# OFA-Sys/ONE-PEACE

Hardware: AMD Instinct MI355X
Metric: pretrain samples/s (tri-modal global batch) ONE-PEACE-4B (higher is better)
Workload: dtype bf16

## Files before the change

include/onepeace_hip.h:

```cpp
#ifndef ONEPEACE_HIP_H
#define ONEPEACE_HIP_H

#include <stdint.h>

#ifdef __cplusplus
extern "C" {
#endif

int op_abi_version(void);
const char* op_last_error(void);

int op_prof_enable(int on);
int op_prof_reserve(int events);
int op_prof_collect(double* ms, int64_t* count, double* work, int n_families);

int op_layernorm_fwd(const void* x, const void* w, const void* b, void* y, float* mean, float* rstd, int64_t rows,
                     int64_t cols, float eps, int act_gelu, int dtype, const int* x_rows, void* stream);
int64_t op_layernorm_bwd_workspace_bytes(int64_t rows, int64_t cols);
int op_layernorm_bwd(const void* dy, const void* x, const void* w, const void* b, const float* mean, const float* rstd,
                     const void* add, void* dx, void* dw, void* db, void* workspace, int64_t rows, int64_t cols,
                     int act_gelu, int accumulate, int dtype, const int* x_rows, void* stream);

int op_gemm_nt(const void* A, int64_t lda, const void* B0, const void* B1, const void* B2, int64_t ldb, int64_t n_seg,
               const void* bias0, const void* bias1, const void* bias2, void* C, int64_t ldc, void* h0, void* h1,
// ... 22 lines not shown
int op_gemm_tn_grouped(int64_t nprob, const void* const* A, const int64_t* lda, const void* const* B, const int64_t* ldb, void* const* C,
                       const int64_t* ldc, const int64_t* M, const int64_t* N, const int64_t* K, const int32_t* accumulate,
                       const void* const* W, const int64_t* ldw, float* const* rowdot, const void* const* rscale, void* counters,
                       int64_t tune, void* stream);
int op_gemm_tn_grouped_lists(int64_t nprob, const void* const* A, const int64_t* lda, const void* const* B, const int64_t* ldb, void* const* C,
                             const int64_t* ldc, const int64_t* M, const int64_t* N, const int64_t* K, const int32_t* accumulate,
                             const void* const* W, const int64_t* ldw, float* const* rowdot, const void* const* rscale,
                             const int32_t* const* ktiles, const int32_t* const* n_ktiles, void* counters, int64_t tune, void* stream);
int op_live_ktiles(int64_t nseg, const float* const* ps, const int64_t* row0, const int64_t* S, const int64_t* B, int64_t nprob,
                   const int64_t* prob_row0, const int64_t* prob_rows, int32_t* const* ktiles, int32_t* const* n_ktiles, void* stream);
int op_live_mwindows(int64_t nseg, const float* const* ps, const int64_t* ps_stride, const int64_t* row0, const int64_t* S, const int64_t* B,
                     const int64_t* wps, const int64_t* odd, const int64_t* seg_list, const int64_t* seg_prob, const int64_t* seg_base, int64_t nlist,
                     int32_t* const* windows,
                     int32_t* const* n_windows, const int64_t* max_windows, int64_t nout, void* const* out, const int64_t* out_ld,
                     const int64_t* out_cols, const int64_t* out_rows, void* stream);
int op_gemm_nt_grouped_windows(int64_t nprob, const void* const* A, const int64_t* M, int64_t lda, const void* const* B, int64_t ldb,
                               void* const* C, int64_t ldc, int64_t N, int64_t K, const int32_t* windows, const int32_t* n_windows,
                               int64_t max_windows, int64_t max_row_stride, int64_t tune, void* stream);
int op_live_mwindows_fwd(int64_t nseg, const float* const* ps, const int64_t* ps_stride, const int64_t* row0, const int64_t* S, const int64_t* B,
                         const int64_t* wps, const int64_t* odd, const int64_t* seg_list, const int64_t* seg_prob, const int64_t* seg_base,
                         int64_t nlist, int32_t* const* windows, int32_t* const* n_windows, const int64_t* max_windows, int64_t nout,
                         void* const* out, const int64_t* out_ld, const int64_t* out_cols, const int64_t* out_rows,
                         const void* const* out_src, const int64_t* out_src_ld, void* stream);
int op_gemm_nt_grouped_windows_fwd(int64_t nprob, const void* const* A, const int64_t* M, int64_t lda, const void* const* B, int64_t ldb,
                                   int64_t n_seg, const void* const* bias, void* const* C, int64_t ldc, const void* const* resid, int64_t ldr,
                                   const void* const* gamma, const float* const* rowscale, const int64_t* rows_per_sample, int64_t N,
                                   int64_t K, int epilogue, const int32_t* windows, const int32_t* n_windows, int64_t max_windows,
                                   int64_t max_row_stride, int64_t tune, void* stream);
int op_gemm_plan(int64_t M, int64_t N, int64_t K, int epilogue, int has_bias, int64_t workspace_bytes, int64_t tune, int* plan);

int op_quant_fp8_rows(const void* x, int64_t ldx, void* q, int64_t ldq, float* scale, int64_t rows, int64_t cols, void* stream);
int op_layernorm_fwd_q8(const void* x, const void* w, const void* b, void* y, float* mean, float* rstd, void* q8, float* q8_scale,
                        int64_t rows, int64_t cols, float eps, void* stream);
int op_ln_geglu_fwd_q8(const void* h0, const void* h1, int64_t ldh, const void* w, const void* b, void* y, float* mean, float* rstd, void* q8,
                       float* q8_scale, int64_t rows, int64_t cols, float eps, void* stream);
int op_gemm_nt_fp8(const void* A8, int64_t lda, const float* sa, const void* B0, const void* B1, int64_t ldb, const float* sb0,
                   const float* sb1, const void* bias, void* C, int64_t ldc, void* h0, void* h1, const void* resid, int64_t ldr,
                   const void* gamma, const float* rowscale, int64_t rows_per_sample, int64_t M, int64_t N, int64_t K, int epilogue,
                   int64_t tune, void* stream);

int op_attn_fwd(const void* q, const void* k, const void* v, int64_t ld, const void* bias, int64_t bias_batch_stride,
                const void* bias_frag, const void* key_pad, void* out, int64_t ldo, float* lse, int64_t lse_ld, int64_t B,
                int64_t S, int64_t Spad, int64_t heads, int64_t head_dim, float scale, int64_t tune, void* stream);
int64_t op_attn_bias_frag_elems(int64_t n_img, int64_t S);
int op_attn_bias_pack(const void* src, void* dst, int64_t n_img, int64_t S, int64_t Spad, void* stream);
int op_attn_bwd_delta(const void* dout, const void* out, int64_t ldo, float* delta, int64_t B, int64_t S, int64_t Spad,
                      int64_t heads, void* stream);
int64_t op_attn_bwd_dbias_slabs(int64_t B, int64_t S, int64_t heads, int64_t tune);
int op_attn_bwd(const void* q, const void* k, const void* v, int64_t ld, const void* dout, const void* out, int64_t ldo,
                const void* bias, const void* biasT, const void* bias_frag, int64_t bias_batch_stride, const void* key_pad,
                const float* lse, float* delta, void* dq,
                void* dk, void* dv, int64_t ldg, float* dbias, int64_t B, int64_t S, int64_t Spad, int64_t heads,
                int64_t head_dim, float scale, int64_t tune, void* stream);

int op_relpos_bias_build(const void* table, const int* bucket, int64_t bucket_ld, void* out, int64_t heads, int64_t S,
                         int64_t Spad, int transposed, void* stream);
int op_relpos_bias_bwd(const float* dbias, int64_t S, int64_t Spad, const int* pos, const int* seg, int64_t nseg, const int* bucket_seg,
                       int64_t num_rel, float* partial_ws, float* dtable, int64_t heads, void* stream);
int op_relpos_bias_build_ids(const void* table, const int* bucket, int64_t bucket_ld, const int* ids, void* out, int64_t B,
                             int64_t heads, int64_t K, int64_t Kpad, int transposed, void* stream);
int op_relpos_bias_fold_ids(const float* dbias, const int* ids, float* dense_ws, int64_t Sfull, int64_t B, int64_t heads, int64_t K,
                            int64_t Kpad, void* stream);

int op_transpose(const void* in, void* out, int64_t rows, int64_t cols, int64_t ld_in, int64_t ld_out, void* stream);
int op_transpose_scaled(const void* in, void* out, int64_t rows, int64_t cols, int64_t ld_in, int64_t ld_out, const void* scale,
                        void* stream);
int op_transpose_batched(const void* table, int64_t n, int64_t total_tiles, void* stream);
int64_t op_transpose_desc_bytes(void);
int64_t op_colsum_workspace_bytes(int64_t N);
int op_colsum_segments(const void* x, void* out0, void* out1, void* out2, void* workspace, int64_t M, int64_t n_seg,
                       int64_t seg_cols, int accumulate, void* stream);
int64_t op_resid_bwd_workspace_bytes(int64_t N);
int op_resid_bwd(const void* dout, const void* y, const void* gamma, const float* rowscale, int64_t rows_per_sample,
                 void* dbranch, void* dgamma, void* dbias, float* g0, void* workspace, int64_t M, int64_t N, int accumulate,
                 const int* dout_rows, void* stream);
int op_gamma_grad_finish(const float* rowdot, int64_t slots, const void* b0, const float* g00, const void* b1, const float* g01,
                         const void* b2, const float* g02, void* dgamma, int64_t N, int accumulate, void* stream);
int op_ln_geglu_bwd(const void* dy, const void* h0, const void* h1, const void* w, const float* mean, const float* rstd,
                    void* dh0, void* dh1, int64_t ldd, int64_t ldh, void* dw, void* db, void* workspace, int64_t rows,
                    int64_t cols, int accumulate, void* stream);
int op_ln_geglu_fwd(const void* h0, const void* h1, int64_t ldh, const void* w, const void* b, void* y, float* mean, float* rstd,
                    int64_t rows, int64_t cols, float eps, void* stream);
int op_colsum(const void* x, const void* y, const float* rowscale, int64_t rows_per_sample, const void* mul, void* out,
              void* workspace, int64_t M, int64_t N, int accumulate, int out_dtype, void* stream);
int op_geglu_bwd(const void* dg, const void* h0, const void* h1, void* dh0, void* dh1, int64_t numel, void* stream);
int op_scale_rows(const void* dout, const void* gamma, const float* rowscale, int64_t rows_per_sample, void* dbranch,
                  int64_t M, int64_t N, void* stream);

int op_l2norm_fwd(const void* x, void* y, float* inv_norm, int64_t rows, int64_t cols, float eps, int out_dtype, void* stream);
int op_l2norm_bwd(const void* dy, const void* y, const float* inv_norm, void* dx, int64_t rows, int64_t cols, int y_dtype,
                  void* stream);
int op_infonce_rows(float* sim, int64_t rows, int64_t n, int64_t ld, int64_t target0, float label_smoothing, float gscale,
                    float* row_loss, float* row_hit, float* row_dot, int write_grad, void* stream);

int op_adamw_step(void* p, const void* g, float* m, float* v, int64_t numel, float lr, float beta1, float beta2, float eps,
                  float weight_decay, int64_t step, float grad_scale, const float* grad_sqnorm, float clip_norm,
                  void* stream);
int op_adamw_step_groups(void* p, const void* g, float* m, float* v, int64_t numel, const int64_t* group_end8,
                         const float* group_lr_scale, const float* group_weight_decay, int64_t n_groups, float lr, float beta1,
                         float beta2, float eps, int64_t step, float grad_scale, const float* grad_sqnorm, float clip_norm,
                         void* stream);
int op_adamw_step_groups_master(void* p, float* master, const void* g, float* m, float* v, int64_t numel,
                                const int64_t* group_end8, const float* group_lr_scale, const float* group_weight_decay,
                                int64_t n_groups, float lr, float beta1, float beta2, float eps, int64_t step, float grad_scale,
                                const float* grad_sqnorm, float clip_norm, void* stream);
int op_ema_step(float* ema, const void* p, int64_t numel, float keep, float take, void* stream);
// ... 55 lines not shown
```

one-peace_amd/csrc/attention.hip:

```cpp
#include <type_traits>

#include "common.h"

namespace {

constexpr int HD = 64;
constexpr int BQ = 128;
constexpr int BKV = 64;
constexpr int VSTRIDE = 160;

struct AttnArgs {
  const bf16_t* q; const bf16_t* k; const bf16_t* v; int64_t ld;
  const bf16_t* bias;
  int64_t bias_bs;
  const uint8_t* key_pad;
  bf16_t* out; int64_t ldo;
  float* lse;
  int64_t lse_ld;
  int B, S, Spad, heads;
  float scale;
};

__device__ __forceinline__ bf16x8 pack8(const float* a, const float* b) {
  bf16x8 r;
#pragma unroll
  for (int i = 0; i < 4; ++i) { r[i] = (bf16_t)a[i]; r[4 + i] = (bf16_t)b[i]; }
  return r;
}

__device__ __forceinline__ s16x4 tr_read(const char* p) {
  return __builtin_amdgcn_ds_read_tr16_b64_v4i16((__attribute__((address_space(3))) s16x4*)(p));
}

__device__ __forceinline__ bf16x8 join_tr(s16x4 a, s16x4 b) {
  typedef __attribute__((ext_vector_type(8))) short s16x8;
  s16x8 r = {a[0], a[1], a[2], a[3], b[0], b[1], b[2], b[3]};
  return __builtin_bit_cast(bf16x8, r);
}

__device__ __forceinline__ int tr_off_swz(int rowblk, int db, int g, int t) {
  const int row = rowblk * 16 + g * 4 + (t >> 2);
  const int c = db * 2 + ((t >> 1) & 1);
  return row * 128 + ((c ^ (row & 7)) << 4) + (t & 1) * 8;
}

__device__ __forceinline__ void xcd_work_item(int& bx, int& by, int& bz) {
  const int nx = gridDim.x, ny = gridDim.y;
  const int total = nx * ny * (int)gridDim.z;
  int lin = blockIdx.x + nx * (blockIdx.y + ny * blockIdx.z);
  if ((total & 7) == 0) lin = (lin & 7) * (total >> 3) + (lin >> 3);
  bx = lin % nx;
  by = (lin / nx) % ny;
  bz = lin / (nx * ny);
}

template <bool HAS_BIAS, bool HAS_PAD>
__global__ __launch_bounds__(256, 2) void attn_fwd_kernel(AttnArgs p) {
  __shared__ __attribute__((aligned(16))) char smem[BKV * 128 + BKV * VSTRIDE];
  char* ldsK = smem;
  char* ldsV = smem + BKV * 128;
  const int tid = threadIdx.x, lane = tid & 63, wid = tid >> 6;
  const int g = lane >> 4, t = lane & 15;
  int bx, h, b;
  xcd_work_item(bx, h, b);
  const int q0 = bx * BQ + wid * 32;
  const bool wave_active = q0 < p.S;
  const int64_t row_base = (int64_t)b * p.S;

  bf16x8 qf[2][2];
#pragma unroll
  for (int qb = 0; qb < 2; ++qb) {
    const int qi = min(q0 + qb * 16 + t, p.S - 1);
    const bf16_t* qp = p.q + (row_base + qi) * p.ld + h * HD;
#pragma unroll
// ... 346 lines not shown
  };

  const int ntiles = (p.S + BKV - 1) / BKV;
  for (int kt = 0; kt < ntiles; ++kt) {
    const int k0 = kt * BKV;
    if (k0 + BKV <= p.S) tile(k0, std::true_type{});
    else tile(k0, std::false_type{});
  }

  float l = l_run;
  l += __shfl_xor(l, 16);
  l += __shfl_xor(l, 32);
  if (q0 + t >= p.S) continue;
  const float inv = 1.f / l;
  bf16_t* op = p.out + (row_base + q0 + t) * p.ldo + h * HD;
#pragma unroll
  for (int db = 0; db < 4; ++db) {
    bf16x4 o;
#pragma unroll
    for (int r = 0; r < 4; ++r) o[r] = (bf16_t)(ot[db][r] * inv);
    *reinterpret_cast<bf16x4*>(op + db * 16 + g * 4) = o;
  }
  if (g == 0 && p.lse) p.lse[((int64_t)b * p.heads + h) * p.lse_ld + q0 + t] = m2_run * (1.0f / LOG2E) + logf(l);
  }
}

constexpr int PERS_NW = 8;
constexpr int PERS_MAX_ROWS = 288;
constexpr int PERS_SCR = 68;
constexpr int PERS_PPT = 2;

__device__ __forceinline__ s16x4 tr_read_a(const char* p) {
  s16x4 r;
  asm volatile("ds_read_b64_tr_b16 %0, %1" : "=v"(r) : "v"((unsigned)(uintptr_t)((__attribute__((address_space(3))) const char*)p)));
  return r;
}
#define ATTN_WAIT_LGKM0()                         \
  do {                                            \
    __builtin_amdgcn_s_waitcnt(0xC07F);           \
    __builtin_amdgcn_sched_barrier(0);            \
  } while (0)

__device__ __forceinline__ void gload16_asm(bf16x8& d, const void* p) { asm volatile("global_load_dwordx4 %0, %1, off" : "=v"(d) : "v"(p)); }
__device__ __forceinline__ void gload4_asm(unsigned& d, const void* p) { asm volatile("global_load_dword %0, %1, off" : "=v"(d) : "v"(p)); }
template <int OFF>
__device__ __forceinline__ void gload16_s(bf16x8& d, const void* sbase, unsigned voff) {
  asm volatile("s_nop 4\n\tglobal_load_dwordx4 %0, %1, %2 offset:%3" : "=v"(d) : "v"(voff), "s"(sbase), "n"(OFF));
}
template <int OFF>
__device__ __forceinline__ void gload4_s(unsigned& d, const void* sbase, unsigned voff) {
  asm volatile("s_nop 4\n\tglobal_load_dword %0, %1, %2 offset:%3" : "=v"(d) : "v"(voff), "s"(sbase), "n"(OFF));
}

template <bool HAS_BIAS, bool HAS_PAD>
__global__ __launch_bounds__(PERS_NW * 64, 2) void attn_fwd_pers_kernel(AttnArgs p, const bf16_t* __restrict__ bias_frag, int rows_pad,
                                                                         int nitems) {
  extern __shared__ __attribute__((aligned(16))) char smem[];
  const int tid = threadIdx.x, lane = tid & 63;
  const int wid = __builtin_amdgcn_readfirstlane(tid >> 6);
  const int g = lane >> 4, t = lane & 15;
  const int KVB = 2 * rows_pad * 128;
  float* scratch = reinterpret_cast<float*>(smem + 2 * KVB);
  const int nqb = (p.S + 15) >> 4, nkp = (p.S + 31) >> 5;
  const bool has_left = nqb > 2 * PERS_NW;
  const int q0 = wid * 32;
  const int nact = min(2, max(0, nqb - 2 * wid));
  const int64_t per_head = (int64_t)nqb * nkp * FRAG_BLOCK;
  const int ntiles = (p.S + BKV - 1) / BKV;
  const float c1 = p.scale * LOG2E;

  bf16x8 sel_lo, sel_hi;
  {
    const bf16_t inv = (bf16_t)(1.0f / p.scale), zero = (bf16_t)0.f;
#pragma unroll
    for (int i = 0; i < 8; ++i) {
      sel_lo[i] = (g * 8 + i == t) ? inv : zero;
      sel_hi[i] = (g * 8 + i == 16 + t) ? inv : zero;
    }
  }
  int trsw[4];
#pragma unroll
  for (int db = 0; db < 4; ++db) trsw[db] = tr_off_swz(0, db, g, t);
  const int kswz[2] = {((0 * 4 + g) ^ (t & 7)) << 4, ((1 * 4 + g) ^ (t & 7)) << 4};

  const int ngrp = rows_pad >> 3;
  const int r_in = lane >> 3, slot = lane & 7;
  const int npiece = (2 * ngrp - wid + PERS_NW - 1) / PERS_NW;
  auto piece = [&](int it, int buf, int j) {
    const int b = it / p.heads, h = it - b * p.heads;
    const int grp = wid + j * PERS_NW;
    const bool isv = grp >= ngrp;
    const int gi = isv ? grp - ngrp : grp;
    const int r = gi * 8 + r_in;
    const int kr = min(r, p.S - 1);
    const bf16_t* src = (isv ? p.v : p.k) + ((int64_t)b * p.S + kr) * p.ld + h * HD + ((slot ^ (r & 7)) << 3);
    char* dst = smem + buf * KVB + (isv ? rows_pad * 128 : 0) + gi * 1024;
    __builtin_amdgcn_global_load_lds((const __attribute__((address_space(1))) void*)src,
                                     (__attribute__((address_space(3))) void*)dst, 16, 0, 0);
  };
  auto load_q = [&](int it, int qrow, bf16x8 (&q)[2]) {
    const int b = it / p.heads, h = it - b * p.heads;
    const bf16_t* qp = p.q + ((int64_t)b * p.S + qrow) * p.ld + h * HD;
#pragma unroll
    for (int kk = 0; kk < 2; ++kk) q[kk] = *reinterpret_cast<const bf16x8*>(qp + kk * 32 + g * 8);
  };
  const int qi_main[2] = {min(q0 + t, p.S - 1), min(q0 + 16 + t, p.S - 1)};

  bf16x8 bn[2][2];
  unsigned padn[4] = {0u, 0u, 0u, 0u};
  auto small_loads = [&](int it, int kt) {
    const int b = it / p.heads, h = it - b * p.heads;
    if constexpr (HAS_BIAS) {
      const bf16_t* fhead = bias_frag + ((p.bias_bs != 0 ? (int64_t)b * p.heads : 0) + h) * per_head + lane * 8;
#pragma unroll
      for (int qb = 0; qb < 2; ++qb) {
        const bf16_t* fb = fhead + (int64_t)min(2 * wid + qb, nqb - 1) * nkp * FRAG_BLOCK;
#pragma unroll
        for (int m = 0; m < 2; ++m) gload16_asm(bn[qb][m], fb + min(2 * kt + m, nkp - 1) * FRAG_BLOCK);
      }
    }
    if constexpr (HAS_PAD) {
      const uint8_t* pr = p.key_pad + (int64_t)b * p.Spad + g * 4 + kt * BKV;
#pragma unroll
      for (int kb = 0; kb < 4; ++kb) gload4_asm(padn[kb], pr + kb * 16);
    }
  };

  constexpr int NSMALL = (HAS_BIAS ? 4 : 0) + (HAS_PAD ? 4 : 0);
  bf16x8 qn[2][2], ql[2], bfl[2];
  unsigned padl[2][2] = {{0u, 0u}, {0u, 0u}};
  auto late_loads = [&](int it_next, int it) {
    {
      const int b = it_next / p.heads, h = it_next - b * p.heads;
#pragma unroll
      for (int qb = 0; qb < 2; ++qb) {
        const bf16_t* qp = p.q + ((int64_t)b * p.S + qi_main[qb]) * p.ld + h * HD;
#pragma unroll
        for (int kk = 0; kk < 2; ++kk) gload16_asm(qn[qb][kk], qp + kk * 32 + g * 8);
      }
    }
    if (has_left) {
      const int b = it / p.heads, h = it - b * p.heads;
      const bf16_t* qp = p.q + ((int64_t)b * p.S + p.S - 1) * p.ld + h * HD;
#pragma unroll
      for (int kk = 0; kk < 2; ++kk) gload16_asm(ql[kk], qp + kk * 32 + g * 8);
      if constexpr (HAS_BIAS) {
        const bf16_t* fleft = bias_frag + ((p.bias_bs != 0 ? (int64_t)b * p.heads : 0) + h) * per_head + lane * 8 + (int64_t)(nqb - 1) * nkp * FRAG_BLOCK;
        gload16_asm(bfl[0], fleft + wid * FRAG_BLOCK);
        gload16_asm(bfl[1], fleft + min(PERS_NW, nkp - 1) * FRAG_BLOCK);
      }
      if constexpr (HAS_PAD) {
        const uint8_t* pr = p.key_pad + (int64_t)b * p.Spad + g * 4;
#pragma unroll
        for (int j = 0; j < 2; ++j) {
          gload4_asm(padl[0][j], pr + (2 * wid + j) * 16);
          gload4_asm(padl[1][j], pr + min((2 * PERS_NW + j) * 16, p.Spad - 16));
        }
      }
    }
  };

  int item = blockIdx.x;
  const int step = gridDim.x;
  if (item < nitems) {
    for (int j = 0; j < npiece; ++j) piece(item, 0, j);
    load_q(item, qi_main[0], qn[0]);
    load_q(item, qi_main[1], qn[1]);
    small_loads(item, 0);
  }
  int buf = 0, prev_item = -1;
  auto wait_all = [&]() {
    asm volatile("s_waitcnt vmcnt(0)" : "+v"(qn[0][0]), "+v"(qn[0][1]), "+v"(qn[1][0]), "+v"(qn[1][1]), "+v"(bn[0][0]), "+v"(bn[0][1]), "+v"(bn[1][0]), "+v"(bn[1][1]),
                 "+v"(padn[0]), "+v"(padn[1]), "+v"(padn[2]), "+v"(padn[3]) : : "memory");
  };
  wait_all();

  auto merge_left = [&](int it, int sb) {
    const float* sc = scratch + sb * (PERS_NW * PERS_SCR);
    float M = -INFINITY;
#pragma unroll
    for (int w = 0; w < PERS_NW; ++w) M = fmaxf(M, sc[w * PERS_SCR + 64]);
    float L = 0.f, o = 0.f;
#pragma unroll
    for (int w = 0; w < PERS_NW; ++w) {
      const float f = __builtin_amdgcn_exp2f(sc[w * PERS_SCR + 64] - M);
      L = __builtin_fmaf(sc[w * PERS_SCR + 65], f, L);
      o = __builtin_fmaf(sc[w * PERS_SCR + lane], f, o);
    }
    const int b = it / p.heads, h = it - b * p.heads;
    const int qrow = p.S - 1;
    p.out[((int64_t)b * p.S + qrow) * p.ldo + h * HD + lane] = (bf16_t)(o / L);
    if (lane == 0 && p.lse) p.lse[((int64_t)b * p.heads + h) * p.lse_ld + qrow] = M * (1.0f / LOG2E) + logf(L);
  };

  for (; item < nitems; item += step, buf ^= 1) {
    const int b = item / p.heads, h = item - b * p.heads;
    const int64_t row_base = (int64_t)b * p.S;
    __syncthreads();
    bf16x8 qf[2][2] = {{qn[0][0], qn[0][1]}, {qn[1][0], qn[1][1]}};
    const bool more = item + step < nitems;
    const int nxt = more ? item + step : item;
    if (has_left && prev_item >= 0 && wid == ((prev_item / step) & (PERS_NW - 1))) merge_left(prev_item, buf ^ 1);
    prev_item = item;

    const char* ldsK = smem + buf * KVB;
    const char* ldsV = ldsK + rows_pad * 128;

    f32x4 ot[2][4];
    float m2_run[2] = {-INFINITY, -INFINITY}, l_run[2] = {0.f, 0.f};
#pragma unroll
    for (int qb = 0; qb < 2; ++qb)
#pragma unroll
      for (int db = 0; db < 4; ++db) ot[qb][db] = (f32x4){0.f, 0.f, 0.f, 0.f};

    auto tile = [&](const int kt, auto full_c) {
      constexpr bool FULL = decltype(full_c)::value;
      const int k0 = kt * BKV;
      const int nkb = FULL ? 4 : ((p.S - k0 + 15) >> 4);
      bf16x8 bf[2][2];
      unsigned padw[4] = {0u, 0u, 0u, 0u};
      if constexpr (HAS_BIAS) {
#pragma unroll
        for (int qb = 0; qb < 2; ++qb)
#pragma unroll
          for (int m = 0; m < 2; ++m) bf[qb][m] = bn[qb][m];
      }
      if constexpr (HAS_PAD) {
#pragma unroll
        for (int kb = 0; kb < 4; ++kb) padw[kb] = padn[kb];
      }
      __builtin_amdgcn_sched_barrier(0);
      if constexpr (FULL) {
        small_loads(item, kt + 1);
      } else {
        late_loads(nxt, item);
        small_loads(nxt, 0);
      }
      __builtin_amdgcn_sched_barrier(0);
#pragma unroll
      for (int jj = 0; jj < PERS_PPT; ++jj) piece(nxt, buf ^ 1, min(kt * PERS_PPT + jj, npiece - 1));
      __builtin_amdgcn_sched_barrier(0);
      if (nact == 0) return;

      const char* kt_ = ldsK + k0 * 128;
      const char* vt = ldsV + k0 * 128;
      f32x4 st[2][4];
#pragma unroll
      for (int qb = 0; qb < 2; ++qb)
#pragma unroll
        for (int kb = 0; kb < 4; ++kb) st[qb][kb] = (f32x4){0.f, 0.f, 0.f, 0.f};
#pragma unroll
      for (int kb = 0; kb < 4; ++kb) {
        if (!FULL && kb >= nkb) break;
#pragma unroll
        for (int kk = 0; kk < 2; ++kk) {
          const bf16x8 kf = *reinterpret_cast<const bf16x8*>(kt_ + (kb * 16 + t) * 128 + kswz[kk]);
#pragma unroll
          for (int qb = 0; qb < 2; ++qb) st[qb][kb] = __builtin_amdgcn_mfma_f32_16x16x32_bf16(kf, qf[qb][kk], st[qb][kb], 0, 0, 0);
        }
        if constexpr (HAS_BIAS) {
#pragma unroll
          for (int qb = 0; qb < 2; ++qb)
            st[qb][kb] = __builtin_amdgcn_mfma_f32_16x16x32_bf16(bf[qb][kb >> 1], (kb & 1) ? sel_hi : sel_lo, st[qb][kb], 0, 0, 0);
        }
      }
      s16x4 va0[4], va1[4];
#pragma unroll
      for (int db = 0; db < 4; ++db) {
        va0[db] = tr_read_a(vt + trsw[db]);
        va1[db] = tr_read_a(vt + trsw[db] + 2048);
      }
      bf16x8 pf[2][2];
#pragma unroll
      for (int qb = 0; qb < 2; ++qb) {
        float mx = -INFINITY;
#pragma unroll
        for (int kb = 0; kb < 4; ++kb) {
          if (!FULL && kb >= nkb) break;
          const int key = k0 + kb * 16 + g * 4;
#pragma unroll
          for (int r = 0; r < 4; ++r) {
            if constexpr (!FULL || HAS_PAD) {
              bool masked = false;
              if constexpr (!FULL) masked = key + r >= p.S;
              if constexpr (HAS_PAD) masked = masked || ((padw[kb] >> (8 * r)) & 0xffu);
              st[qb][kb][r] = masked ? -INFINITY : st[qb][kb][r];
            }
            mx = fmaxf(mx, st[qb][kb][r]);
// ... 110 lines not shown
        float psum = 0.f;
#pragma unroll
        for (int j = 0; j < 2; ++j)
#pragma unroll
          for (int r = 0; r < 4; ++r) {
            pv[j][r] = __builtin_amdgcn_exp2f(__builtin_fmaf(s4[j][r], c1, -m2_use));
            psum += pv[j][r];
          }
        lsum = lsum * alpha + psum;
        const bf16x8 pf = pack8(pv[0], pv[1]);
        s16x4 v0[4], v1[4];
#pragma unroll
        for (int db = 0; db < 4; ++db) {
          v0[db] = tr_read_a(ldsV + trsw[db] + (2 * kp) * 2048);
          v1[db] = tr_read_a(ldsV + trsw[db] + (2 * kp + 1) * 2048);
        }
        ATTN_WAIT_LGKM0();
#pragma unroll
        for (int db = 0; db < 4; ++db) {
#pragma unroll
          for (int r = 0; r < 4; ++r) ol[db][r] *= alpha;
          ol[db] = __builtin_amdgcn_mfma_f32_16x16x32_bf16(join_tr(v0[db], v1[db]), pf, ol[db], 0, 0, 0);
        }
      }
      lsum += __shfl_xor(lsum, 16);
      lsum += __shfl_xor(lsum, 32);
      float* sc = scratch + (buf * PERS_NW + wid) * PERS_SCR;
      if (t == 0) {
#pragma unroll
        for (int db = 0; db < 4; ++db) *reinterpret_cast<f32x4*>(sc + db * 16 + g * 4) = ol[db];
        if (g == 0) { sc[64] = m2; sc[65] = lsum; }
      }
    }
#pragma unroll
    for (int qb = 0; qb < 2; ++qb) {
      float l = l_run[qb];
      l += __shfl_xor(l, 16);
      l += __shfl_xor(l, 32);
      const int qrow = q0 + qb * 16 + t;
      if (qb < nact && qrow < p.S) {
        const float inv = 1.f / l;
        bf16_t* op = p.out + (row_base + qrow) * p.ldo + h * HD;
#pragma unroll
        for (int db = 0; db < 4; ++db) {
          bf16x4 o;
#pragma unroll
          for (int r = 0; r < 4; ++r) o[r] = (bf16_t)(ot[qb][db][r] * inv);
          *reinterpret_cast<bf16x4*>(op + db * 16 + g * 4) = o;
        }
        if (g == 0 && p.lse) p.lse[((int64_t)b * p.heads + h) * p.lse_ld + qrow] = m2_run[qb] * (1.0f / LOG2E) + logf(l);
      }
    }
    wait_all();
  }
  if (has_left && prev_item >= 0) {
    __syncthreads();
    if (wid == 0) merge_left(prev_item, buf ^ 1);
  }
}

__global__ __launch_bounds__(256) void bias_pack_kernel(const bf16_t* __restrict__ src, bf16_t* __restrict__ dst, int S, int Spad,
                                                        int nqb, int nkp, int64_t total) {
  const int64_t idx = (int64_t)blockIdx.x * 256 + threadIdx.x;
  if (idx >= total) return;
  const int lane = (int)(idx & 63);
  int64_t blk = idx >> 6;
  const int kp = (int)(blk % nkp);
  blk /= nkp;
  const int qb = (int)(blk % nqb);
  const int64_t img = blk / nqb;
  const int g = lane >> 4, t = lane & 15;
  const int key = kp * 32 + (g >> 1) * 16 + t;
  const int qbase = qb * 16 + (g & 1) * 8;
  bf16x8 v;
#pragma unroll
  for (int i = 0; i < 8; ++i) {
    const int q = qbase + i;
    v[i] = (q < S && key < S) ? src[(img * S + q) * Spad + key] : (bf16_t)0.f;
  }
  *reinterpret_cast<bf16x8*>(dst + idx * 8) = v;
}

struct AttnBwdArgs {
  const bf16_t* q; const bf16_t* k; const bf16_t* v; int64_t ld;
  const bf16_t* dout; int64_t ldo;
  const bf16_t* bias;
  const bf16_t* biasT;
  const bf16_t* bias_frag;
  int64_t bias_bs;
  const uint8_t* key_pad;
  const float* lse;
  const float* delta;
  const bf16_t* out;
  float* delta_w;
  bf16_t* dq; bf16_t* dk; bf16_t* dv; int64_t ldg;
  float* dbias;
  int B, S, Spad, heads, bchunk;
  float scale;
  int lone_keys;
};

__global__ __launch_bounds__(256) void attn_delta_kernel(const bf16_t* __restrict__ dout, const bf16_t* __restrict__ out,
                                                         int64_t ldo, float* __restrict__ delta, int B, int S, int Spad,
                                                         int heads) {
  const int64_t gid = (int64_t)blockIdx.x * 256 + threadIdx.x;
  const int per_row = heads * 8;
// ... 620 lines not shown
              ds[0][kb][r] = __builtin_amdgcn_exp2f(__builtin_fmaf(st[kb][r], c1, nl2)) * (ds[0][kb][r] - dl);
        }
      } else {
        ds_tile<1, true, (NT < 6)>(p, b, h, k0, q0w, g, t, qf, of, lse, del, kfrag, vfrag, biasfrag, prefetch, ds);
      }
#pragma unroll
      for (int c = 0; c < NT; ++c) {
        if (kt == c) {
#pragma unroll
          for (int kb = 0; kb < 4; ++kb)
            if (c < NT - 1 || kb < LASTB) acc[c][kb] += ds[0][kb];
        }
      }
#pragma unroll
      for (int m = 0; m < 2; ++m) {
        if (k0 + m * 32 >= p.S) break;
        float a0[4], a1[4];
#pragma unroll
        for (int r = 0; r < 4; ++r) { a0[r] = ds[0][2 * m][r]; a1[r] = ds[0][2 * m + 1][r]; }
        const bf16x8 dsf = pack8(a0, a1);
#pragma unroll
        for (int db = 0; db < 4; ++db) {
          const bf16x8 kT = join_tr(tr_read(ldsK + trsw[db] + (2 * m) * 2048), tr_read(ldsK + trsw[db] + (2 * m + 1) * 2048));
          dqT[db] = __builtin_amdgcn_mfma_f32_16x16x32_bf16(kT, dsf, dqT[db], 0, 0, 0);
        }
      }
    }
    if (wave_active && q0w + t < p.S) {
      bf16_t* qp = p.dq + ((int64_t)b * p.S + q0w + t) * p.ldg + h * HD;
#pragma unroll
      for (int db = 0; db < 4; ++db) {
        bf16x4 a;
#pragma unroll
        for (int r = 0; r < 4; ++r) a[r] = (bf16_t)(dqT[db][r] * p.scale);
        *reinterpret_cast<bf16x4*>(qp + db * 16 + g * 4) = a;
      }
    }
  }
  if (!wave_active || q0w + t >= p.S) return;
  float* drow = p.dbias + (((int64_t)chunk * p.heads + h) * p.S + q0w + t) * p.Spad + g * 4;
#pragma unroll
  for (int kt = 0; kt < NT; ++kt) {
    f32x4 cur[4];
#pragma unroll
    for (int kb = 0; kb < 4; ++kb)
      if ((kt < NT - 1 || kb < LASTB) && kt * BKV + kb * 16 < p.Spad) cur[kb] = *reinterpret_cast<const f32x4*>(drow + kt * BKV + kb * 16);
#pragma unroll
    for (int kb = 0; kb < 4; ++kb)
      if ((kt < NT - 1 || kb < LASTB) && kt * BKV + kb * 16 < p.Spad)
        *reinterpret_cast<f32x4*>(drow + kt * BKV + kb * 16) = cur[kb] + acc[kt][kb];
  }
}

template <bool HAS_BIAS, bool HAS_PAD, int NT, int LASTB, bool LEFT>
__device__ __forceinline__ void attn_bwd_dq_pers_body(const AttnBwdArgs& p, char* smem, int rows_pad, int nqh, int qhalf0) {
  const int tid = threadIdx.x, lane = tid & 63;
  const int wid = __builtin_amdgcn_readfirstlane(tid >> 6);
  const int g = lane >> 4, t = lane & 15;
  const int KVB = 2 * rows_pad * 128;
  float* scratch = reinterpret_cast<float*>(smem + 2 * KVB);
  const int nqb = (p.S + 15) >> 4, nkp = (p.S + 31) >> 5;
  const int qhalf = qhalf0, h = (blockIdx.x / nqh) % p.heads, chunk = blockIdx.x / (nqh * p.heads);
  const int b_begin = chunk * p.bchunk, b_end = min(p.B, b_begin + p.bchunk);
  if (b_begin >= b_end) return;
  const int qblk = qhalf * PERS_NW + wid;
  const bool active = qblk < min(nqb, 2 * PERS_NW);
  constexpr bool has_left = LEFT;
  const int q0w = min(qblk, nqb - 1) * 16;
  const int qi = min(q0w + t, p.S - 1);
  const float c1 = p.scale * LOG2E;
  const int64_t per_head = (int64_t)nqb * nkp * FRAG_BLOCK;

  bf16x8 sel_lo, sel_hi;
  {
    const bf16_t inv = (bf16_t)(1.0f / p.scale), zero = (bf16_t)0.f;
#pragma unroll
    for (int i = 0; i < 8; ++i) {
      sel_lo[i] = (g * 8 + i == t) ? inv : zero;
      sel_hi[i] = (g * 8 + i == 16 + t) ? inv : zero;
    }
  }
  int trsw[4];
#pragma unroll
  for (int db = 0; db < 4; ++db) trsw[db] = tr_off_swz(0, db, g, t);
  const int kswz[2] = {((0 * 4 + g) ^ (t & 7)) << 4, ((1 * 4 + g) ^ (t & 7)) << 4};

  const int ngrp = rows_pad >> 3;
  const int r_in = lane >> 3, slot = lane & 7;
  const int npiece = (2 * ngrp - wid + PERS_NW - 1) / PERS_NW;
  auto piece = [&](int b, int buf, int j) {
    const int grp = wid + j * PERS_NW;
    const bool isv = grp >= ngrp;
    const int gi = isv ? grp - ngrp : grp;
    int rl = r_in;
    asm volatile("" : "+v"(rl));
    const int r = gi * 8 + rl;
    const int kr = min(r, p.S - 1);
    const unsigned voff = (unsigned)((kr * (int)p.ld + ((slot ^ (r & 7)) << 3)) * 2);
    const char* sbase = (const char*)((isv ? p.v : p.k) + (int64_t)b * p.S * p.ld + h * HD);
    char* dst = smem + buf * KVB + (isv ? rows_pad * 128 : 0) + gi * 1024;
    __builtin_amdgcn_global_load_lds((const __attribute__((address_space(1))) void*)(sbase + voff),
                                     (__attribute__((address_space(3))) void*)dst, 16, 0, 0);
  };

  constexpr int NSMALL = (HAS_BIAS ? 2 : 0) + (HAS_PAD ? 4 : 0);
  constexpr int BPPT = 3;
  auto ppt_of = [](int kt) { return kt < 3 ? BPPT : 0; };
  const bf16_t* fwave = HAS_BIAS ? p.bias_frag + (int64_t)h * per_head + (int64_t)(q0w >> 4) * nkp * FRAG_BLOCK : nullptr;
  const bf16_t* fleft = HAS_BIAS ? p.bias_frag + (int64_t)h * per_head + (int64_t)(nqb - 1) * nkp * FRAG_BLOCK : nullptr;
  const unsigned vo_frag = lane * 16, vo_pad = g * 4;
  const unsigned vo_q = (unsigned)(((int64_t)qi * p.ld + h * HD + g * 8) * 2), vo_o = (unsigned)(((int64_t)qi * p.ldo + h * HD + g * 8) * 2);
  const unsigned vo_ql = (unsigned)(((int64_t)(p.S - 1) * p.ld + h * HD + g * 8) * 2), vo_ol = (unsigned)(((int64_t)(p.S - 1) * p.ldo + h * HD + g * 8) * 2);
  const unsigned vo_lse = qi * 4, vo_lsel = (p.S - 1) * 4;
  bf16x8 bn[2];
  unsigned padn[4] = {0u, 0u, 0u, 0u};
  auto small_loads = [&](int b, int kt) {
    if constexpr (HAS_BIAS) {
// ... 3 lines not shown
    if constexpr (HAS_PAD) {
      const uint8_t* pr = p.key_pad + (int64_t)b * p.Spad + kt * BKV;
      gload4_s<0>(padn[0], pr, vo_pad);
      gload4_s<16>(padn[1], pr, vo_pad);
      gload4_s<32>(padn[2], pr, vo_pad);
      gload4_s<48>(padn[3], pr, vo_pad);
    }
  };
  bf16x8 qn[2], don[2], oon[2], ql[2], dol[2], ool[2], bfl[2];
  float lsen, lsel;
  unsigned padl[2][2] = {{0u, 0u}, {0u, 0u}};
  auto query_loads = [&](int b, unsigned voq, unsigned voo, unsigned vol, bf16x8 (&q)[2], bf16x8 (&d)[2], bf16x8 (&o)[2], float& l) {
    const bf16_t* sq = p.q + (int64_t)b * p.S * p.ld;
    const bf16_t* sd = p.dout + (int64_t)b * p.S * p.ldo;
    const bf16_t* so = p.out + (int64_t)b * p.S * p.ldo;
    gload16_s<0>(q[0], sq, voq);
    gload16_s<64>(q[1], sq, voq);
    gload16_s<0>(d[0], sd, voo);
    gload16_s<64>(d[1], sd, voo);
    gload16_s<0>(o[0], so, voo);
    gload16_s<64>(o[1], so, voo);
    unsigned lw;
    gload4_s<0>(lw, p.lse + ((int64_t)b * p.heads + h) * p.Spad, vol);
    l = __builtin_bit_cast(float, lw);
  };
  auto late_loads = [&](int b_next, int b) {
    (void)b_next;
    if (has_left) {
      query_loads(b, vo_ql, vo_ol, vo_lsel, ql, dol, ool, lsel);
      if constexpr (HAS_BIAS) {
        gload16_s<0>(bfl[0], fleft + wid * FRAG_BLOCK, vo_frag);
        gload16_s<0>(bfl[1], fleft + min(PERS_NW, nkp - 1) * FRAG_BLOCK, vo_frag);
      }
      if constexpr (HAS_PAD) {
        const uint8_t* pr = p.key_pad + (int64_t)b * p.Spad;
        gload4_s<0>(padl[0][0], pr + 2 * wid * 16, vo_pad);
        gload4_s<16>(padl[0][1], pr + 2 * wid * 16, vo_pad);
        gload4_s<0>(padl[1][0], pr + min(2 * PERS_NW * 16, p.Spad - 32), vo_pad);
        gload4_s<16>(padl[1][1], pr + min(2 * PERS_NW * 16, p.Spad - 32), vo_pad);
      }
    }
  };

  f32x4 acc[NT][4], accl[2][2];
#pragma unroll
  for (int kt = 0; kt < NT; ++kt)
#pragma unroll
    for (int kb = 0; kb < 4; ++kb) acc[kt][kb] = (f32x4){0.f, 0.f, 0.f, 0.f};
#pragma unroll
  for (int i = 0; i < 2; ++i)
#pragma unroll
    for (int j = 0; j < 2; ++j) accl[i][j] = (f32x4){0.f, 0.f, 0.f, 0.f};

  for (int j = 0; j < npiece; ++j) piece(b_begin, 0, j);
  query_loads(b_begin, vo_q, vo_o, vo_lse, qn, don, oon, lsen);
  small_loads(b_begin, 0);
  int buf = 0, prev_b = -1;
  auto merge_left = [&](int b, int sb) {
    const float* sc = scratch + sb * (PERS_NW * 64);
    float o = 0.f;
#pragma unroll
    for (int w = 0; w < PERS_NW; ++w) o += sc[w * 64 + lane];
    p.dq[((int64_t)b * p.S + p.S - 1) * p.ldg + h * HD + lane] = (bf16_t)(o * p.scale);
  };

  auto wait_all = [&]() {
    asm volatile("s_waitcnt vmcnt(0)" : "+v"(qn[0]), "+v"(qn[1]), "+v"(don[0]), "+v"(don[1]), "+v"(oon[0]), "+v"(oon[1]), "+v"(lsen), "+v"(bn[0]), "+v"(bn[1]),
                 "+v"(padn[0]), "+v"(padn[1]), "+v"(padn[2]), "+v"(padn[3]) : : "memory");
  };
  wait_all();
  for (int b = b_begin; b < b_end; ++b, buf ^= 1) {
    __syncthreads();
    const bf16x8 qf[2] = {qn[0], qn[1]}, dof[2] = {don[0], don[1]};
    const float dl = delta_from_frags(dof, oon);
    const float nl2 = -lsen * LOG2E;
    if (active && g == 0 && q0w + t < p.S) p.delta_w[((int64_t)b * p.heads + h) * p.Spad + q0w + t] = dl;
    const int nxt = b + 1 < b_end ? b + 1 : b;
    if (has_left && prev_b >= 0 && wid == (prev_b & (PERS_NW - 1))) merge_left(prev_b, buf ^ 1);
    prev_b = b;
    const char* ldsK = smem + buf * KVB;
    const char* ldsV = ldsK + rows_pad * 128;
    f32x4 dqT[4];
#pragma unroll
    for (int db = 0; db < 4; ++db) dqT[db] = (f32x4){0.f, 0.f, 0.f, 0.f};

    auto tile = [&](const int kt, auto last_c) {
      constexpr bool LAST = decltype(last_c)::value;
      const int k0 = kt * BKV;
      if (kt > 0) {
        if (ppt_of(kt - 1) > 0) {
          if constexpr (HAS_BIAS && HAS_PAD)
            asm volatile("s_waitcnt vmcnt(%6)" : "+v"(bn[0]), "+v"(bn[1]), "+v"(padn[0]), "+v"(padn[1]), "+v"(padn[2]), "+v"(padn[3]) : "n"(BPPT));
          else if constexpr (HAS_BIAS)
            asm volatile("s_waitcnt vmcnt(%2)" : "+v"(bn[0]), "+v"(bn[1]) : "n"(BPPT));
          else if constexpr (HAS_PAD)
            asm volatile("s_waitcnt vmcnt(%4)" : "+v"(padn[0]), "+v"(padn[1]), "+v"(padn[2]), "+v"(padn[3]) : "n"(BPPT));
        } else {
          if constexpr (HAS_BIAS && HAS_PAD)
            asm volatile("s_waitcnt vmcnt(0)" : "+v"(bn[0]), "+v"(bn[1]), "+v"(padn[0]), "+v"(padn[1]), "+v"(padn[2]), "+v"(padn[3]));
          else if constexpr (HAS_BIAS)
            asm volatile("s_waitcnt vmcnt(0)" : "+v"(bn[0]), "+v"(bn[1]));
          else if constexpr (HAS_PAD)
            asm volatile("s_waitcnt vmcnt(0)" : "+v"(padn[0]), "+v"(padn[1]), "+v"(padn[2]), "+v"(padn[3]));
        }
      }
      bf16x8 bf[2];
      unsigned padw[4] = {0u, 0u, 0u, 0u};
      if constexpr (HAS_BIAS) { bf[0] = bn[0]; bf[1] = bn[1]; }
      if constexpr (HAS_PAD) {
#pragma unroll
        for (int kb = 0; kb < 4; ++kb) padw[kb] = padn[kb];
      }
      __builtin_amdgcn_sched_barrier(0);
      if constexpr (!LAST) {
        if constexpr (!LEFT) {
          if (kt == NT - 2) query_loads(nxt, vo_q, vo_o, vo_lse, qn, don, oon, lsen);
        }
        small_loads(b, kt + 1);
      } else {
        late_loads(nxt, b);
        small_loads(nxt, 0);
      }
      __builtin_amdgcn_sched_barrier(0);
#pragma unroll
      for (int jj = 0; jj < BPPT; ++jj)
        if (ppt_of(kt) > 0) piece(nxt, buf ^ 1, min(kt * BPPT + jj, npiece - 1));
      __builtin_amdgcn_sched_barrier(0);
      const char* kt_ = ldsK + k0 * 128;
      const char* vt = ldsV + k0 * 128;
      constexpr int NKB = LAST ? LASTB : 4;
// ... 79 lines not shown
      f32x4 dql[4];
#pragma unroll
      for (int db = 0; db < 4; ++db) dql[db] = (f32x4){0.f, 0.f, 0.f, 0.f};
#pragma unroll
      for (int pc = 0; pc < 2; ++pc) {
        if (pc == 1 && wid != 0) break;
        const int kp = pc == 0 ? wid : PERS_NW;
        f32x4 s4[2], d4[2];
#pragma unroll
        for (int j = 0; j < 2; ++j) {
          s4[j] = (f32x4){0.f, 0.f, 0.f, 0.f};
          d4[j] = (f32x4){0.f, 0.f, 0.f, 0.f};
#pragma unroll
          for (int kk = 0; kk < 2; ++kk) {
            const bf16x8 kf = *reinterpret_cast<const bf16x8*>(ldsK + ((2 * kp + j) * 16 + t) * 128 + kswz[kk]);
            const bf16x8 vf = *reinterpret_cast<const bf16x8*>(ldsV + ((2 * kp + j) * 16 + t) * 128 + kswz[kk]);
            s4[j] = __builtin_amdgcn_mfma_f32_16x16x32_bf16(kf, ql[kk], s4[j], 0, 0, 0);
            d4[j] = __builtin_amdgcn_mfma_f32_16x16x32_bf16(vf, dol[kk], d4[j], 0, 0, 0);
          }
          if constexpr (HAS_BIAS) s4[j] = __builtin_amdgcn_mfma_f32_16x16x32_bf16(bfl[pc], j ? sel_hi : sel_lo, s4[j], 0, 0, 0);
        }
        float a0[4], a1[4];
#pragma unroll
        for (int j = 0; j < 2; ++j)
#pragma unroll
          for (int r = 0; r < 4; ++r) {
            bool dead = (2 * kp + j) * 16 + g * 4 + r >= p.S;
            if constexpr (HAS_PAD) dead = dead || ((padl[pc][j] >> (8 * r)) & 0xffu);
            const float x = dead ? -INFINITY : __builtin_fmaf(s4[j][r], c1, nl2l);
            const float v = __builtin_amdgcn_exp2f(x) * (d4[j][r] - dll);
            d4[j][r] = v;
            (j ? a1 : a0)[r] = v;
          }
        if constexpr (HAS_BIAS) { accl[pc][0] += d4[0]; accl[pc][1] += d4[1]; }
        const bf16x8 dsf = pack8(a0, a1);
        s16x4 k0r[4], k1r[4];
#pragma unroll
        for (int db = 0; db < 4; ++db) {
          k0r[db] = tr_read_a(ldsK + trsw[db] + (2 * kp) * 2048);
          k1r[db] = tr_read_a(ldsK + trsw[db] + (2 * kp + 1) * 2048);
        }
        ATTN_WAIT_LGKM0();
#pragma unroll
        for (int db = 0; db < 4; ++db) dql[db] = __builtin_amdgcn_mfma_f32_16x16x32_bf16(join_tr(k0r[db], k1r[db]), dsf, dql[db], 0, 0, 0);
      }
      float* sc = scratch + (buf * PERS_NW + wid) * 64;
      if (t == 0) {
#pragma unroll
        for (int db = 0; db < 4; ++db) *reinterpret_cast<f32x4*>(sc + db * 16 + g * 4) = dql[db];
      }
    }

    wait_all();
  }
  if (has_left && prev_b >= 0) {
    __syncthreads();
    if (wid == 0) merge_left(prev_b, buf ^ 1);
  }
  if constexpr (HAS_BIAS) {
    if (p.dbias == nullptr) return;
    if (active && q0w + t < p.S) {
      float* drow = p.dbias + (((int64_t)chunk * p.heads + h) * p.S + q0w + t) * p.Spad + g * 4;
#pragma unroll
      for (int kt = 0; kt < NT; ++kt) {
        f32x4 cur[4];
#pragma unroll
        for (int kb = 0; kb < 4; ++kb)
          if ((kt < NT - 1 || kb < LASTB) && kt * BKV + kb * 16 < p.Spad) cur[kb] = *reinterpret_cast<const f32x4*>(drow + kt * BKV + kb * 16);
#pragma unroll
        for (int kb = 0; kb < 4; ++kb)
          if ((kt < NT - 1 || kb < LASTB) && kt * BKV + kb * 16 < p.Spad)
            *reinterpret_cast<f32x4*>(drow + kt * BKV + kb * 16) = cur[kb] + acc[kt][kb];
      }
    }
    if (has_left && t == 0) {
      float* drow = p.dbias + (((int64_t)chunk * p.heads + h) * p.S + p.S - 1) * p.Spad + g * 4;
#pragma unroll
      for (int pc = 0; pc < 2; ++pc) {
        if (pc == 1 && wid != 0) break;
        const int kp = pc == 0 ? wid : PERS_NW;
#pragma unroll
        for (int j = 0; j < 2; ++j) {
          const int key0 = (2 * kp + j) * 16;
          if (key0 < p.Spad) {
            float* d = drow + key0;
            *reinterpret_cast<f32x4*>(d) = *reinterpret_cast<const f32x4*>(d) + accl[pc][j];
          }
        }
      }
    }
  }
}

template <bool HAS_BIAS, bool HAS_PAD, int NT, int LASTB>
__global__ __launch_bounds__(PERS_NW * 64, 2) void attn_bwd_dq_pers_kernel(AttnBwdArgs p, int rows_pad, int nqh) {
  extern __shared__ __attribute__((aligned(16))) char smem[];
  const int qhalf = blockIdx.x % nqh;
  const bool lone = ((p.S + 15) >> 4) > 2 * PERS_NW && qhalf == nqh - 1;
  if constexpr (NT == 5) {
    if (lone) {
      attn_bwd_dq_pers_body<HAS_BIAS, HAS_PAD, NT, LASTB, true>(p, smem, rows_pad, nqh, qhalf);
      return;
    }
  }
  attn_bwd_dq_pers_body<HAS_BIAS, HAS_PAD, NT, LASTB, false>(p, smem, rows_pad, nqh, qhalf);
}

constexpr int PERS_SCRL = 136;

template <int OFF>
__device__ __forceinline__ void gload1_s(unsigned& d, const void* sbase, unsigned voff) {
  asm volatile("s_nop 4\n\tglobal_load_ubyte %0, %1, %2 offset:%3" : "=v"(d) : "v"(voff), "s"(sbase), "n"(OFF));
}

__device__ __forceinline__ u32x4 attn_raw_rsrc(const void* base, int nbytes) {
  const uint64_t a = (uint64_t)base;
  return (u32x4){(unsigned)__builtin_amdgcn_readfirstlane((int)(unsigned)a), (unsigned)__builtin_amdgcn_readfirstlane((int)(unsigned)(a >> 32)) & 0xffffu,
                 (unsigned)__builtin_amdgcn_readfirstlane(nbytes), 0x00020000u};
}
__device__ __forceinline__ void bstore8(const bf16x4& data, const u32x4& rsrc, unsigned voff) {
  asm volatile("s_nop 4\n\tbuffer_store_dwordx2 %0, %1, %2, 0 offen\n\ts_nop 1" ::"v"(data), "v"(voff), "s"(rsrc) : "memory");
}

template <bool HAS_BIAS, bool HAS_PAD, int NT, bool LONE>
__global__ __launch_bounds__(PERS_NW * 64, 2) void attn_bwd_dkdv_pers_kernel(AttnBwdArgs p, int rows_pad, int nitems) {
  extern __shared__ __attribute__((aligned(16))) char smem[];
  const int tid = threadIdx.x, lane = tid & 63;
  const int wid = __builtin_amdgcn_readfirstlane(tid >> 6);
  const int g = lane >> 4, t = lane & 15;
  const int QBY = rows_pad * 128;
  const int BUFB = 2 * QBY + 6144;
  float* scratch = reinterpret_cast<float*>(smem + 2 * BUFB);
  const int kbase = wid * 32;
  const bool wave_active = kbase < min(p.S, 256);
  const float c1 = p.scale * LOG2E;

  bf16x8 sel_lo, sel_hi;
  {
    const bf16_t inv = (bf16_t)(1.0f / p.scale), zero = (bf16_t)0.f;
#pragma unroll
    for (int i = 0; i < 8; ++i) {
      sel_lo[i] = (g * 8 + i == t) ? inv : zero;
      sel_hi[i] = (g * 8 + i == 16 + t) ? inv : zero;
    }
  }
  int trsw[4];
#pragma unroll
  for (int db = 0; db < 4; ++db) trsw[db] = tr_off_swz(0, db, g, t);
  const int kswz[2] = {((0 * 4 + g) ^ (t & 7)) << 4, ((1 * 4 + g) ^ (t & 7)) << 4};

  const int ngrp = rows_pad >> 3;
  const int NG = 2 * ngrp + (LONE ? 6 : 4);
  const int r_in = lane >> 3, slot = lane & 7;
  const int npiece = (NG - wid + PERS_NW - 1) / PERS_NW;
  auto piece = [&](int it, int buf, int j) {
    const int b = it / p.heads, h = it - b * p.heads;
    const int grp = wid + j * PERS_NW;
    int rl = r_in;
    asm volatile("" : "+v"(rl));
    const char* sbase;
    unsigned voff;
    int dst_off;
    if (grp < 2 * ngrp) {
      const bool isd = grp >= ngrp;
      const int gi = isd ? grp - ngrp : grp;
      const int r = gi * 8 + rl;
      const int qr = min(r, p.S - 1);
      const int ldx = isd ? (int)p.ldo : (int)p.ld;
      voff = (unsigned)((qr * ldx + ((slot ^ (r & 7)) << 3)) * 2);
      sbase = isd ? (const char*)(p.dout + (int64_t)b * p.S * p.ldo + h * HD) : (const char*)(p.q + (int64_t)b * p.S * p.ld + h * HD);
      dst_off = (isd ? QBY : 0) + gi * 1024;
    } else {
      const int e = grp - 2 * ngrp;
      if (e < 4) {
        voff = (unsigned)min((e & 1) * 1024 + (rl * 8 + slot) * 16, p.Spad * 4 - 16);
        sbase = (const char*)((e < 2 ? p.lse : p.delta) + ((int64_t)b * p.heads + h) * p.Spad);
      } else {
        voff = (unsigned)(((p.S - 1) * (int)p.ld + slot * 8) * 2);
        sbase = (const char*)((e == 4 ? p.k : p.v) + (int64_t)b * p.S * p.ld + h * HD);
// ... 5 lines not shown
  };

  const int key_kb[2] = {min(kbase + t, p.S - 1), min(kbase + 16 + t, p.S - 1)};
  const unsigned vo_k[2] = {(unsigned)((key_kb[0] * (int)p.ld + g * 8) * 2), (unsigned)((key_kb[1] * (int)p.ld + g * 8) * 2)};
  bf16x8 kf[2][2], vf[2][2], kn[LONE ? 1 : 2][2], vn[LONE ? 1 : 2][2];
  unsigned kdn[2] = {0u, 0u}, kdl = 0u;
  auto kv_loads = [&](int it, bf16x8 (&kd)[2][2], bf16x8 (&vd)[2][2]) {
    const int b = it / p.heads, h = it - b * p.heads;
    const bf16_t* sk = p.k + (int64_t)b * p.S * p.ld + h * HD;
    const bf16_t* sv = p.v + (int64_t)b * p.S * p.ld + h * HD;
#pragma unroll
    for (int kb = 0; kb < 2; ++kb) {
      gload16_s<0>(kd[kb][0], sk, vo_k[kb]);
      gload16_s<64>(kd[kb][1], sk, vo_k[kb]);
      gload16_s<0>(vd[kb][0], sv, vo_k[kb]);
      gload16_s<64>(vd[kb][1], sv, vo_k[kb]);
    }
    if constexpr (HAS_PAD) {
      const uint8_t* pr = p.key_pad + (int64_t)b * p.Spad;
      gload1_s<0>(kdn[0], pr, (unsigned)key_kb[0]);
      gload1_s<0>(kdn[1], pr, (unsigned)key_kb[1]);
      if constexpr (LONE) gload1_s<0>(kdl, pr, (unsigned)(p.S - 1));
    }
  };
  constexpr int NKV = 8 + (HAS_PAD ? (LONE ? 3 : 2) : 0);
  const unsigned vo_b[2] = {(unsigned)((key_kb[0] * p.Spad + g * 8) * 2), (unsigned)((key_kb[1] * p.Spad + g * 8) * 2)};
  const unsigned vo_bl = (unsigned)(((p.S - 1) * p.Spad + g * 8) * 2);
  bf16x8 bn[2][2], bfl[2];
  auto bias_loads = [&](int it, auto qt_c, auto m_c) {
    constexpr int QT = decltype(qt_c)::value, M = decltype(m_c)::value;
    if constexpr (HAS_BIAS) {
      const int h = it % p.heads;
      const bf16_t* sb = p.biasT + (int64_t)h * p.S * p.Spad;
      gload16_s<(QT * 64 + M * 32) * 2>(bn[M][0], sb, vo_b[0]);
      gload16_s<(QT * 64 + M * 32) * 2>(bn[M][1], sb, vo_b[1]);
    }
  };
  constexpr int NBH = HAS_BIAS ? 2 : 0;
  auto lone_bias_loads = [&](int it) {
    if constexpr (HAS_BIAS && LONE) {
      const int h = it % p.heads;
      const bf16_t* sb = p.biasT + (int64_t)h * p.S * p.Spad;
      gload16_s<0>(bfl[0], sb + wid * 32, vo_bl);
      gload16_s<512>(bfl[1], sb, vo_bl);
    }
  };
  constexpr int NLB = (HAS_BIAS && LONE) ? 2 : 0;
  constexpr int BPPT = NT == 5 ? 3 : 4;

  int item = blockIdx.x;
  const int step = gridDim.x;
  using I0 = std::integral_constant<int, 0>;
  using I1 = std::integral_constant<int, 1>;
  if (item < nitems) {
    for (int j = 0; j < npiece; ++j) piece(item, 0, j);
    if constexpr (LONE) kv_loads(item, kf, vf);
    else kv_loads(item, kn, vn);
    bias_loads(item, I0{}, I0{});
    bias_loads(item, I0{}, I1{});
  }
#define DKDV_WAIT_LOADS(NST)                                                                                                                  \
  do {                                                                                                                                     \
    if constexpr (LONE)                                                                                                                    \
      asm volatile("s_waitcnt vmcnt(%15)" : "+v"(kf[0][0]), "+v"(kf[0][1]), "+v"(kf[1][0]), "+v"(kf[1][1]), "+v"(vf[0][0]), "+v"(vf[0][1]),   \
                   "+v"(vf[1][0]), "+v"(vf[1][1]), "+v"(bn[0][0]), "+v"(bn[0][1]), "+v"(bn[1][0]), "+v"(bn[1][1]), "+v"(kdn[0]), "+v"(kdn[1]), \
                   "+v"(kdl) : "n"(NST) : "memory");                                                                                      \
    else                                                                                                                                   \
      asm volatile("s_waitcnt vmcnt(%15)" : "+v"(kn[0][0]), "+v"(kn[0][1]), "+v"(kn[1][0]), "+v"(kn[1][1]), "+v"(vn[0][0]), "+v"(vn[0][1]),   \
                   "+v"(vn[1][0]), "+v"(vn[1][1]), "+v"(bn[0][0]), "+v"(bn[0][1]), "+v"(bn[1][0]), "+v"(bn[1][1]), "+v"(kdn[0]), "+v"(kdn[1]), \
                   "+v"(kdl) : "n"(NST) : "memory");                                                                                      \
  } while (0)
  DKDV_WAIT_LOADS(0);
  int buf = 0, prev_item = -1;
  auto merge_lone = [&](int it, int sb) {
    const float* sc = scratch + sb * (PERS_NW * PERS_SCRL);
    float dv = 0.f, dk = 0.f;
#pragma unroll
    for (int w = 0; w < PERS_NW; ++w) { dv += sc[w * PERS_SCRL + lane]; dk += sc[w * PERS_SCRL + 64 + lane]; }
    const bool dead = sc[128] != 0.f;
    const int b = it / p.heads, h = it - b * p.heads;
    const int64_t row = ((int64_t)b * p.S + p.S - 1) * p.ldg + h * HD + lane;
    p.dv[row] = dead ? (bf16_t)0.f : (bf16_t)dv;
    p.dk[row] = dead ? (bf16_t)0.f : (bf16_t)(dk * p.scale);
  };

  for (; item < nitems; item += step, buf ^= 1) {
    const int b = item / p.heads, h = item - b * p.heads;
    asm volatile("s_waitcnt lgkmcnt(0)" ::: "memory");
    __builtin_amdgcn_s_barrier();
    asm volatile("" ::: "memory");
    if constexpr (!LONE) {
#pragma unroll
      for (int kb = 0; kb < 2; ++kb)
#pragma unroll
        for (int kk = 0; kk < 2; ++kk) { kf[kb][kk] = kn[kb][kk]; vf[kb][kk] = vn[kb][kk]; }
    }
    const bool kdead[2] = {HAS_PAD && kdn[0] != 0u, HAS_PAD && kdn[1] != 0u};
    const bool ldead = HAS_PAD && LONE && kdl != 0u;
    const int nxt = item + step < nitems ? item + step : item;
    if (LONE && prev_item >= 0 && wid == ((prev_item / step) & (PERS_NW - 1))) merge_lone(prev_item, buf ^ 1);
    prev_item = item;
    const char* ldsQ = smem + buf * BUFB;
    const char* ldsO = ldsQ + QBY;
    const float* ldsL = reinterpret_cast<const float*>(ldsQ + 2 * QBY);
    const float* ldsD = ldsL + 512;

    f32x4 dvT[2][4], dkT[2][4];
#pragma unroll
    for (int kb = 0; kb < 2; ++kb)
#pragma unroll
      for (int db = 0; db < 4; ++db) { dvT[kb][db] = (f32x4){0.f, 0.f, 0.f, 0.f}; dkT[kb][db] = (f32x4){0.f, 0.f, 0.f, 0.f}; }

    auto half = [&](const int q0h, auto nkb_c, const bf16x8 (&kx)[2][2], const bf16x8 (&vx)[2][2], const bf16x8 (&bx)[2],
                    f32x4 (&dvx)[2][4], f32x4 (&dkx)[2][4]) {
      constexpr int NKB = decltype(nkb_c)::value;
      f32x4 s[2][NKB], dp[2][NKB];
#pragma unroll
      for (int j = 0; j < 2; ++j)
#pragma unroll
        for (int kb = 0; kb < NKB; ++kb) { s[j][kb] = (f32x4){0.f, 0.f, 0.f, 0.f}; dp[j][kb] = (f32x4){0.f, 0.f, 0.f, 0.f}; }
      const bool second = q0h + 16 < p.S;
#pragma unroll
      for (int j = 0; j < 2; ++j) {
        if (j == 1 && !second) continue;
#pragma unroll
        for (int kk = 0; kk < 2; ++kk) {
          const int off = (q0h + j * 16 + t) * 128 + kswz[kk];
          const bf16x8 qfr = *reinterpret_cast<const bf16x8*>(ldsQ + off);
          const bf16x8 ofr = *reinterpret_cast<const bf16x8*>(ldsO + off);
#pragma unroll
          for (int kb = 0; kb < NKB; ++kb) {
            s[j][kb] = __builtin_amdgcn_mfma_f32_16x16x32_bf16(qfr, kx[kb][kk], s[j][kb], 0, 0, 0);
            dp[j][kb] = __builtin_amdgcn_mfma_f32_16x16x32_bf16(ofr, vx[kb][kk], dp[j][kb], 0, 0, 0);
          }
        }
        if constexpr (HAS_BIAS) {
#pragma unroll
          for (int kb = 0; kb < NKB; ++kb) s[j][kb] = __builtin_amdgcn_mfma_f32_16x16x32_bf16(j ? sel_hi : sel_lo, bx[kb], s[j][kb], 0, 0, 0);
        }
      }
      const s16x4 zero4 = {0, 0, 0, 0};
      s16x4 o0[2], o1[2], q0r[2], q1r[2];
      auto tr_request = [&](int dh) {
#pragma unroll
        for (int i = 0; i < 2; ++i) {
          const int db = 2 * dh + i;
          o0[i] = tr_read_a(ldsO + q0h * 128 + trsw[db]);
          q0r[i] = tr_read_a(ldsQ + q0h * 128 + trsw[db]);
          o1[i] = zero4;
          q1r[i] = zero4;
          if (second) {
            o1[i] = tr_read_a(ldsO + q0h * 128 + trsw[db] + 2048);
            q1r[i] = tr_read_a(ldsQ + q0h * 128 + trsw[db] + 2048);
          }
// ... 19 lines not shown
#pragma unroll
      for (int j = 0; j < 2; ++j) {
        if (j == 1 && !second) continue;
#pragma unroll
        for (int kb = 0; kb < NKB; ++kb) {
#pragma unroll
          for (int r = 0; r < 4; ++r) {
            const float pr = __builtin_amdgcn_exp2f(__builtin_fmaf(s[j][kb][r], c1, -l2[j][r]));
            s[j][kb][r] = pr;
            dp[j][kb][r] = pr * (dp[j][kb][r] - dl[j][r]);
          }
        }
      }
      bf16x8 pfr[NKB], dsf[NKB];
#pragma unroll
      for (int kb = 0; kb < NKB; ++kb) {
        float a0[4], a1[4], b0[4], b1[4];
#pragma unroll
        for (int r = 0; r < 4; ++r) {
          a0[r] = s[0][kb][r]; a1[r] = s[1][kb][r];
          b0[r] = dp[0][kb][r]; b1[r] = dp[1][kb][r];
        }
        pfr[kb] = pack8(a0, a1);
        dsf[kb] = pack8(b0, b1);
      }
#pragma unroll
      for (int dh = 0; dh < 2; ++dh) {
        if (dh == 1) tr_request(1);
        ATTN_WAIT_LGKM0();
#pragma unroll
        for (int i = 0; i < 2; ++i) {
          const int db = 2 * dh + i;
          const bf16x8 oT = join_tr(o0[i], o1[i]), qT = join_tr(q0r[i], q1r[i]);
#pragma unroll
          for (int kb = 0; kb < NKB; ++kb) {
            dvx[kb][db] = __builtin_amdgcn_mfma_f32_16x16x32_bf16(oT, pfr[kb], dvx[kb][db], 0, 0, 0);
            dkx[kb][db] = __builtin_amdgcn_mfma_f32_16x16x32_bf16(qT, dsf[kb], dkx[kb][db], 0, 0, 0);
          }
        }
      }
    };

    auto tile = [&](auto qt_c) {
      constexpr int QT = decltype(qt_c)::value;
      constexpr bool LAST = QT == NT - 1;
      using QN = std::integral_constant<int, LAST ? 0 : QT + 1>;
      if constexpr (!LAST) {
#pragma unroll
        for (int jj = 0; jj < BPPT; ++jj) piece(nxt, buf ^ 1, min(QT * BPPT + jj, npiece - 1));
      }
      __builtin_amdgcn_sched_barrier(0);
      if (wave_active) half(QT * 64, std::integral_constant<int, 2>{}, kf, vf, bn[0], dvT, dkT);
      __builtin_amdgcn_sched_barrier(0);
      if constexpr (!LAST) bias_loads(item, QN{}, I0{});
      if constexpr (HAS_BIAS && QT > 0) {
        if constexpr (!LAST) asm volatile("s_waitcnt vmcnt(%2)" : "+v"(bn[1][0]), "+v"(bn[1][1]) : "n"(BPPT + NBH));
        else asm volatile("s_waitcnt vmcnt(0)" : "+v"(bn[1][0]), "+v"(bn[1][1]));
      }
      __builtin_amdgcn_sched_barrier(0);
      if (wave_active && QT * 64 + 32 < p.S) half(QT * 64 + 32, std::integral_constant<int, 2>{}, kf, vf, bn[1], dvT, dkT);
      __builtin_amdgcn_sched_barrier(0);
      if constexpr (!LAST) {
        bias_loads(item, QN{}, I1{});
        if constexpr (HAS_BIAS) asm volatile("s_waitcnt vmcnt(%2)" : "+v"(bn[0][0]), "+v"(bn[0][1]) : "n"(NBH));
      } else {
        lone_bias_loads(item);
        bias_loads(nxt, I0{}, I0{});
        bias_loads(nxt, I0{}, I1{});
        if constexpr (!LONE) kv_loads(nxt, kn, vn);
      }
    };
    tile(std::integral_constant<int, 0>{});
    tile(std::integral_constant<int, 1>{});
    tile(std::integral_constant<int, 2>{});
    tile(std::integral_constant<int, 3>{});
    if constexpr (NT == 5) tile(std::integral_constant<int, 4>{});

    if constexpr (LONE) {
      kv_loads(nxt, kf, vf);
      if constexpr (NLB > 0) asm volatile("s_waitcnt vmcnt(%2)" : "+v"(bfl[0]), "+v"(bfl[1]) : "n"(NKV + 2 * NBH));
      const char* ldsLK = ldsQ + 2 * QBY + 4096;
      bf16x8 kl[2][2], vl[2][2];
#pragma unroll
      for (int kk = 0; kk < 2; ++kk) {
        kl[0][kk] = *reinterpret_cast<const bf16x8*>(ldsLK + (kk * 4 + g) * 16);
        vl[0][kk] = *reinterpret_cast<const bf16x8*>(ldsLK + 1024 + (kk * 4 + g) * 16);
        kl[1][kk] = kl[0][kk];
        vl[1][kk] = vl[0][kk];
      }
      f32x4 dvl[2][4], dkl[2][4];
#pragma unroll
      for (int db = 0; db < 4; ++db) { dvl[0][db] = (f32x4){0.f, 0.f, 0.f, 0.f}; dkl[0][db] = (f32x4){0.f, 0.f, 0.f, 0.f}; }
      const bf16x8 bl0[2] = {bfl[0], bfl[0]}, bl1[2] = {bfl[1], bfl[1]};
      half(wid * 32, std::integral_constant<int, 1>{}, kl, vl, bl0, dvl, dkl);
      if (wid == 0) half(256, std::integral_constant<int, 1>{}, kl, vl, bl1, dvl, dkl);
      float* sc = scratch + (buf * PERS_NW + wid) * PERS_SCRL;
      if (t == 0) {
#pragma unroll
        for (int db = 0; db < 4; ++db) {
          *reinterpret_cast<f32x4*>(sc + db * 16 + g * 4) = dvl[0][db];
          *reinterpret_cast<f32x4*>(sc + 64 + db * 16 + g * 4) = dkl[0][db];
        }
      }
      if (wid == 0 && lane == 0) sc[128] = ldead ? 1.f : 0.f;
    }

    {
      const int nrec = ((min(p.S, 256) - 1) * (int)p.ldg + HD) * 2;
      const u32x4 rk = attn_raw_rsrc(p.dk + (int64_t)b * p.S * p.ldg + h * HD, nrec);
      const u32x4 rv = attn_raw_rsrc(p.dv + (int64_t)b * p.S * p.ldg + h * HD, nrec);
#pragma unroll
      for (int kb = 0; kb < 2; ++kb) {
        const unsigned voff = (unsigned)(((kbase + kb * 16 + t) * (int)p.ldg + g * 4) * 2);
#pragma unroll
        for (int db = 0; db < 4; ++db) {
          bf16x4 a, c;
#pragma unroll
          for (int r = 0; r < 4; ++r) {
            a[r] = kdead[kb] ? (bf16_t)0.f : (bf16_t)(dkT[kb][db][r] * p.scale);
            c[r] = kdead[kb] ? (bf16_t)0.f : (bf16_t)dvT[kb][db][r];
          }
          bstore8(a, rk, voff + db * 32);
          bstore8(c, rv, voff + db * 32);
        }
      }
      DKDV_WAIT_LOADS(16);
    }
  }
  if (LONE && prev_item >= 0) {
    __syncthreads();
    if (wid == 0) merge_lone(prev_item, buf ^ 1);
  }
}

#undef DKDV_WAIT_LOADS

__global__ __launch_bounds__(256, 2) void attn_bwd_dbias_kernel(AttnBwdArgs p) {
  __shared__ __attribute__((aligned(16))) char smem[2 * 64 * 128];
  char* ldsK = smem;
  char* ldsV = smem + 64 * 128;
  const int tid = threadIdx.x, lane = tid & 63, wid = tid >> 6;
  const int g = lane >> 4, t = lane & 15;
  const int h = blockIdx.z % p.heads, chunk = blockIdx.z / p.heads;
  const int q0w = blockIdx.x * BQ + wid * 32;
  const int k0 = blockIdx.y * BKV;
  const bool wave_active = q0w < p.S;
  f32x4 acc[2][4];
  bf16x4 breg[2][4];
#pragma unroll
  for (int qb = 0; qb < 2; ++qb) {
    const int qi = min(q0w + qb * 16 + t, p.S - 1);
#pragma unroll
    for (int kb = 0; kb < 4; ++kb) {
      acc[qb][kb] = (f32x4){0.f, 0.f, 0.f, 0.f};
      if (p.bias)
        breg[qb][kb] = *reinterpret_cast<const bf16x4*>(p.bias + (int64_t)(chunk * p.bchunk) * p.bias_bs + ((int64_t)h * p.S + qi) * p.Spad +
                                                        k0 + kb * 16 + g * 4);
    }
  }
  u32x4 rk[2], rv[2];
  int st_row[2], st_c[2];
#pragma unroll
  for (int i = 0; i < 2; ++i) { const int c2 = tid + 256 * i; st_row[i] = c2 >> 3; st_c[i] = c2 & 7; }
  auto load_tile = [&](int b) {
#pragma unroll
    for (int i = 0; i < 2; ++i) {
      const int kr = min(k0 + st_row[i], p.S - 1);
      const int64_t off = ((int64_t)b * p.S + kr) * p.ld + h * HD + st_c[i] * 8;
      rk[i] = *reinterpret_cast<const u32x4*>(p.k + off);
      rv[i] = *reinterpret_cast<const u32x4*>(p.v + off);
    }
  };
  auto write_tile = [&]() {
#pragma unroll
    for (int i = 0; i < 2; ++i) {
      const int off = st_row[i] * 128 + ((st_c[i] ^ (st_row[i] & 7)) << 4);
      *reinterpret_cast<u32x4*>(ldsK + off) = rk[i];
      *reinterpret_cast<u32x4*>(ldsV + off) = rv[i];
    }
  };
// ... 80 lines not shown
  if (forced > 0) return ceil_div(B, ceil_div(B, min((int64_t)forced, B)));
  if (round2_rule) {
    const int64_t base2 = (int64_t)ceil_div(S, 64) * heads;
    int chunks = (int)((768 + base2 - 1) / base2);
    if (chunks < 1) chunks = 1;
    if (chunks > B) chunks = (int)B;
    return ceil_div(B, ceil_div(B, chunks));
  }
  const int cus = op_num_cus();
  const int64_t base = (int64_t)ceil_div(S, 64) * heads, slots = 2 * (int64_t)cus;
  int best = 1;
  double best_cost = 1e30;
  for (int c = 1; c <= 32 && c <= B; ++c) {
    const int bchunk = ceil_div(B, c), n = ceil_div(B, bchunk);
    if (n != c) continue;
    const double cost = (double)ceil_div(base * n, slots) * bchunk + 0.05 * n;
    if (cost < best_cost - 1e-9) { best_cost = cost; best = c; }
  }
  return best;
}

inline int sep_bchunk(int64_t B, int64_t S, int64_t heads) {
  const int64_t base = (int64_t)ceil_div(S, BQ) * ceil_div(S, BKV) * heads;
  int chunks = (int)((1024 + base - 1) / base);
  if (chunks < 1) chunks = 1;
  if (chunks > B) chunks = (int)B;
  return ceil_div(B, chunks);
}

inline int pers_bwd_chunks(int64_t B, int64_t S, int64_t heads) {
  const int nqh = ceil_div(min((int64_t)ceil_div(S, 16), (int64_t)2 * PERS_NW), PERS_NW);
  int c = (int)(op_num_cus() / (heads * nqh));
  if (c < 1) c = 1;
  if (c > B) c = (int)B;
  return ceil_div(B, ceil_div(B, c));
}
inline bool pers_bwd_shape(int64_t S) { return S > 192 && S <= 257; }

inline int dkdv_pers_rows(int64_t S) { return (int)((S + 15) / 16) * 16; }
inline size_t dkdv_pers_lds(int64_t S) { return (size_t)2 * (2 * dkdv_pers_rows(S) * 128 + 6144) + 2 * PERS_NW * PERS_SCRL * 4; }

}

extern "C" int op_prof_begin(int family, double work, void* stream);
extern "C" void op_prof_end(int slot, void* stream);

static int attn_launched(int rc, int slot, void* stream) {
  op_prof_end(slot, stream);
  if (rc != OP_OK) return rc;
  OP_LAUNCH_CHECK();
  return OP_OK;
}

extern "C" {

int64_t op_attn_bwd_dbias_slabs(int64_t B, int64_t S, int64_t heads, int64_t tune) {
  if ((tune & BWD_SEPARATE_DBIAS) || ceil_div(S, BKV) > 6) return ceil_div(B, sep_bchunk(B, S, heads));
  const int64_t n = dbias_chunks(B, S, heads, true, (tune & BWD_ROUND2_CHUNKS) != 0, (int)((tune >> BWD_CHUNKS_SHIFT) & BWD_CHUNKS_MASK));
  if (!(tune & BWD_NO_PERS_DQ) && pers_bwd_shape(S)) return max(n, (int64_t)pers_bwd_chunks(B, S, heads));
  return n;
}

int op_attn_fwd(const void* q, const void* k, const void* v, int64_t ld, const void* bias, int64_t bias_batch_stride,
                const void* bias_frag, const void* key_pad, void* out, int64_t ldo, float* lse, int64_t lse_ld, int64_t B,
                int64_t S, int64_t Spad, int64_t heads, int64_t head_dim, float scale, int64_t tune, void* stream) {
  OP_CHECK_ARG(q && k && v && out, "attn_fwd: null pointer");
  OP_CHECK_ARG(head_dim == HD, "attn_fwd: head_dim %lld unsupported (only 64)", (long long)head_dim);
  OP_CHECK_ARG(B > 0 && S > 0 && heads > 0 && ld % 8 == 0 && ldo % 4 == 0, "attn_fwd: bad sizes");
  OP_CHECK_ARG((!bias && !key_pad) || (Spad >= ((S + 63) / 64) * 64 && Spad % 8 == 0),
               "attn_fwd: Spad must be >= S rounded up to 64");
  AttnArgs a;
  a.q = (const bf16_t*)q; a.k = (const bf16_t*)k; a.v = (const bf16_t*)v; a.ld = ld;
  a.bias = (const bf16_t*)bias; a.bias_bs = bias ? bias_batch_stride : 0; a.key_pad = (const uint8_t*)key_pad;
  a.out = (bf16_t*)out; a.ldo = ldo; a.lse = lse; a.lse_ld = lse_ld > 0 ? lse_ld : S;
  a.B = (int)B; a.S = (int)S; a.Spad = (int)Spad; a.heads = (int)heads; a.scale = scale;
  dim3 grid(ceil_div(S, BQ), (unsigned)heads, (unsigned)B);
  const int slot = op_prof_begin(1, 4.0 * (double)B * (double)heads * (double)S * (double)S * HD, stream);
  hipStream_t s = (hipStream_t)stream;
  const bool inv_exact = (float)(bf16_t)(1.0f / scale) * scale == 1.0f;
  const bf16_t* fr = (const bf16_t*)bias_frag;
  if (!(tune & FWD_STREAMING) && !(tune & FWD_NO_PERS) && S > 192 && S <= 257 && (!bias || (bias_frag && inv_exact))) {
    const int rows_pad = ceil_div(S, 32) * 32;
    const size_t sh = (size_t)4 * rows_pad * 128 + 2 * PERS_NW * PERS_SCR * 4;
    const int nitems = (int)(B * heads);
    const int nwg = min(nitems, op_num_cus());
    return attn_launched(with_bias_pad(bias, key_pad, [&](auto hb, auto hp) {
      constexpr auto kern = attn_fwd_pers_kernel<decltype(hb)::value, decltype(hp)::value>;
      OP_ENSURE_LDS(kern, 4 * PERS_MAX_ROWS * 128 + 2 * PERS_NW * PERS_SCR * 4, "attn_fwd");
      hipLaunchKernelGGL(kern, dim3(nwg), dim3(PERS_NW * 64), sh, s, a, fr, rows_pad, nitems);
      return OP_OK;
    }), slot, stream);
  }
  if (!(tune & FWD_STREAMING) && S <= RES_MAX_S && (!bias || (bias_frag && inv_exact))) {
    const int nqb = ceil_div(S, 16);
    const int nwg = ceil_div(nqb, RES_MAX_NW);
    const int qb_per_wg = ceil_div(nqb, nwg);
    int nwaves = qb_per_wg;
    const int forced_waves = (int)((tune >> FWD_WAVES_SHIFT) & FWD_WAVES_MASK);
    if (forced_waves) nwaves = min(qb_per_wg, forced_waves);
    else if (qb_per_wg == 9) nwaves = 8;
    const int rows_pad = ceil_div(S, 32) * 32;
    const size_t sh = (size_t)2 * rows_pad * 128;
    const dim3 rgrid(nwg, (unsigned)heads, (unsigned)B);
    const int abl = (int)((tune >> FWD_ABLATE_SHIFT) & FWD_ABLATE_MASK);
    return attn_launched(with_bias_pad(bias, key_pad, [&](auto hb, auto hp) {
      constexpr auto kern = attn_fwd_res_kernel<decltype(hb)::value, decltype(hp)::value>;
      OP_ENSURE_LDS(kern, 2 * RES_MAX_S * 128, "attn_fwd");
      hipLaunchKernelGGL(kern, rgrid, dim3(nwaves * 64), sh, s, a, fr, rows_pad, qb_per_wg, abl);
      return OP_OK;
    }), slot, stream);
  }
  return attn_launched(with_bias_pad(bias, key_pad, [&](auto hb, auto hp) {
    hipLaunchKernelGGL((attn_fwd_kernel<decltype(hb)::value, decltype(hp)::value>), grid, dim3(256), 0, s, a);
    return OP_OK;
  }), slot, stream);
}


int64_t op_attn_bias_frag_elems(int64_t n_img, int64_t S) {
  return n_img * (int64_t)ceil_div(S, 16) * ceil_div(S, 32) * FRAG_BLOCK;
}

int op_attn_bias_pack(const void* src, void* dst, int64_t n_img, int64_t S, int64_t Spad, void* stream) {
  OP_CHECK_ARG(src && dst && n_img > 0 && S > 0 && Spad >= S, "attn_bias_pack: bad args");
  const int nqb = ceil_div(S, 16), nkp = ceil_div(S, 32);
  const int64_t total = n_img * nqb * nkp * 64;
  hipLaunchKernelGGL(bias_pack_kernel, dim3(ceil_div(total, 256)), dim3(256), 0, (hipStream_t)stream, (const bf16_t*)src,
                     (bf16_t*)dst, (int)S, (int)Spad, nqb, nkp, total);
  OP_LAUNCH_CHECK();
  return OP_OK;
}

int op_attn_bwd_delta(const void* dout, const void* out, int64_t ldo, float* delta, int64_t B, int64_t S, int64_t Spad,
                      int64_t heads, void* stream) {
  OP_CHECK_ARG(dout && out && delta && ldo % 8 == 0, "attn_bwd_delta: bad args");
  const int64_t threads = B * S * heads * 8;
  hipLaunchKernelGGL(attn_delta_kernel, dim3(ceil_div(threads, 256)), dim3(256), 0, (hipStream_t)stream, (const bf16_t*)dout,
                     (const bf16_t*)out, ldo, delta, (int)B, (int)S, (int)Spad, (int)heads);
  OP_LAUNCH_CHECK();
  return OP_OK;
}

int op_attn_bwd(const void* q, const void* k, const void* v, int64_t ld, const void* dout, const void* out, int64_t ldo, const void* bias,
                const void* biasT, const void* bias_frag, int64_t bias_batch_stride, const void* key_pad, const float* lse,
                float* delta, void* dq,
                void* dk, void* dv, int64_t ldg, float* dbias, int64_t B, int64_t S, int64_t Spad, int64_t heads,
                int64_t head_dim, float scale, int64_t tune, void* stream) {
  const bool merge_dbias = !(tune & BWD_SEPARATE_DBIAS);
  OP_CHECK_ARG(q && k && v && dout && lse && delta && dq && dk && dv, "attn_bwd: null pointer");
  OP_CHECK_ARG(head_dim == HD, "attn_bwd: head_dim %lld unsupported (only 64)", (long long)head_dim);
  OP_CHECK_ARG(B > 0 && S > 0 && heads > 0, "attn_bwd: bad sizes");
  OP_CHECK_ARG(Spad >= ((S + 127) / 128) * 128 && Spad % 8 == 0, "attn_bwd: Spad must be >= S rounded up to 128");
  OP_CHECK_ARG((bias == nullptr) == (biasT == nullptr), "attn_bwd: bias and biasT must be given together");
  OP_CHECK_ARG(!dbias || bias, "attn_bwd: dbias without a bias");
  OP_CHECK_ARG(ld % 8 == 0 && ldo % 8 == 0 && ldg % 4 == 0, "attn_bwd: bad leading dims");
  AttnBwdArgs a;
  a.q = (const bf16_t*)q; a.k = (const bf16_t*)k; a.v = (const bf16_t*)v; a.ld = ld;
  a.dout = (const bf16_t*)dout; a.ldo = ldo; a.bias = (const bf16_t*)bias; a.biasT = (const bf16_t*)biasT;
  a.bias_frag = bias ? (const bf16_t*)bias_frag : nullptr;
  a.bias_bs = bias ? bias_batch_stride : 0;
  a.key_pad = (const uint8_t*)key_pad; a.lse = lse; a.delta = delta; a.out = (const bf16_t*)out; a.delta_w = delta;
  a.dq = (bf16_t*)dq; a.dk = (bf16_t*)dk; a.dv = (bf16_t*)dv; a.ldg = ldg; a.dbias = dbias;
  a.B = (int)B; a.S = (int)S; a.Spad = (int)Spad; a.heads = (int)heads; a.scale = scale;
  a.lone_keys = !(tune & BWD_NO_LONE_KEYS);
  a.bchunk = sep_bchunk(B, S, heads);
  hipStream_t s = (hipStream_t)stream;
  const double fl = 4.0 * (double)B * (double)heads * (double)S * (double)S * HD;
  const int bchunk_dkdv = a.bchunk;
  auto launch_dkdv = [&]() {
    AttnBwdArgs d = a;
    d.bchunk = bchunk_dkdv;
    const int sl = op_prof_begin(2, 2.0 * fl, stream);
    const int kb = ((tune >> BWD_DKDV_KEYS_SHIFT) & BWD_DKDV_KEYS_MASK) == 2 ? 1 : 2;
    return attn_launched(op_with_bool(bias != nullptr, [&](auto hb) {
      return op_with_int<1, 2>(kb, [&](auto kbc) {
        constexpr int KB = decltype(kbc)::value;
        hipLaunchKernelGGL((attn_bwd_dkdv_kernel<decltype(hb)::value, KB>), dim3(ceil_div(S, 64 * KB), (unsigned)heads, (unsigned)B), dim3(256),
                           0, s, d);
        return OP_OK;
      });
    }), sl, stream);
  };
  if (!out) {
    const int rc = launch_dkdv();
    if (rc != OP_OK) return rc;
  }
  const int nt = ceil_div(S, BKV);
  if (merge_dbias && !(tune & BWD_NO_PERS_DQ) && out && pers_bwd_shape(S) && a.bias_bs == 0 &&
      (!bias || (a.bias_frag != nullptr && (float)(bf16_t)(1.0f / scale) * scale == 1.0f))) {
    const int nqb = ceil_div(S, 16);
    const int nqh = ceil_div(min(nqb, 2 * PERS_NW), PERS_NW);
    const int chunks = pers_bwd_chunks(B, S, heads);
    a.bchunk = ceil_div(B, chunks);
    const int rows_pad = S > 256 ? PERS_MAX_ROWS : 256;
    const size_t sh = (size_t)4 * rows_pad * 128 + 2 * PERS_NW * 64 * 4;
    const int nwg = chunks * (int)heads * nqh;
    AttnBwdArgs d = a;
    if (!bias) d.dbias = nullptr;
    const int slot = op_prof_begin(2, 1.5 * fl, stream);
    int rc = attn_launched(with_bias_pad(bias, key_pad, [&](auto hb, auto hp) {
      return op_with_bool(S > 256, [&](auto lone) {
        constexpr bool LONE = decltype(lone)::value;
        constexpr auto kern = attn_bwd_dq_pers_kernel<decltype(hb)::value, decltype(hp)::value, LONE ? 5 : 4, LONE ? 1 : 4>;
        OP_ENSURE_LDS(kern, 4 * PERS_MAX_ROWS * 128 + 2 * PERS_NW * 64 * 4, "attn_bwd");
        hipLaunchKernelGGL(kern, dim3(nwg), dim3(PERS_NW * 64), sh, s, d, rows_pad, nqh);
        return OP_OK;
      });
    }), slot, stream);
    if (rc != OP_OK) return rc;
    a.bchunk = bchunk_dkdv;
    if ((tune & BWD_NO_PERS_DKDV) || (bias && !biasT) || (S == 256 && !(tune & BWD_PERS_DKDV_256))) return launch_dkdv();
    const int dk_rows = dkdv_pers_rows(S), nitems = a.B * a.heads, dk_nwg = min(nitems, op_num_cus());
    const int dk_slot = op_prof_begin(2, 2.0 * fl, stream);
    return attn_launched(with_bias_pad(bias, key_pad, [&](auto hb, auto hp) {
      return op_with_bool(S > 256, [&](auto lone) {
        constexpr bool LONE = decltype(lone)::value;
        constexpr auto kern = attn_bwd_dkdv_pers_kernel<decltype(hb)::value, decltype(hp)::value, LONE ? 5 : 4, LONE>;
        OP_ENSURE_LDS(kern, (int)dkdv_pers_lds(LONE ? 257 : 256), "attn_bwd");
        hipLaunchKernelGGL(kern, dim3(dk_nwg), dim3(PERS_NW * 64), dkdv_pers_lds(S), s, a, dk_rows, nitems);
        return OP_OK;
      });
    }), dk_slot, stream);
  }
  if (dbias && nt <= 6 && merge_dbias) {
    const int chunks = a.bias_bs != 0 ? (int)B : dbias_chunks(B, S, heads, true, (tune & BWD_ROUND2_CHUNKS) != 0,
                                                              (int)((tune >> BWD_CHUNKS_SHIFT) & BWD_CHUNKS_MASK));
    a.bchunk = ceil_div(B, chunks);
    const dim3 grid(ceil_div(S, 64), (unsigned)heads, (unsigned)chunks);
    const bool one_block = ceil_div(S - (nt - 1) * BKV, 16) == 1;
    const bool frag = a.bias_frag != nullptr && (float)(bf16_t)(1.0f / scale) * scale == 1.0f && (nt <= 4 || (nt == 5 && one_block));
    const int slot = op_prof_begin(2, 1.5 * fl, stream);
    const int rc = attn_launched(op_with_int<1, 2, 3, 4, 5, 6>(nt, [&](auto n) {
      return op_with_bool(frag, [&](auto fr) {
        return op_with_bool(one_block, [&](auto ob) {
          hipLaunchKernelGGL((attn_bwd_dq_dbias_kernel<decltype(n)::value, decltype(fr)::value, decltype(ob)::value ? 1 : 4>), grid, dim3(256),
                             0, s, a);
          return OP_OK;
        });
      });
    }), slot, stream);
    return rc != OP_OK || !out ? rc : launch_dkdv();
  }
  const int slot = op_prof_begin(2, 1.5 * fl, stream);
  int rc = attn_launched(op_with_bool(bias != nullptr, [&](auto hb) {
    hipLaunchKernelGGL(attn_bwd_dq_kernel<decltype(hb)::value>, dim3(ceil_div(S, BQ), (unsigned)heads, (unsigned)B), dim3(256), 0, s, a);
    return OP_OK;
  }), slot, stream);
  if (rc == OP_OK && out) rc = launch_dkdv();
  if (rc != OP_OK) return rc;
  if (dbias) {
    if (a.bias_bs != 0) a.bchunk = 1;
    const int chunks = ceil_div(B, a.bchunk);
    hipLaunchKernelGGL(attn_bwd_dbias_kernel, dim3(ceil_div(S, BQ), ceil_div(S, BKV), (unsigned)(heads * chunks)), dim3(256), 0,
                       s, a);
    OP_LAUNCH_CHECK();
  }
  return OP_OK;
}

}
```

one-peace_amd/csrc/elementwise.hip:

```cpp
#include "common.h"
#include <string.h>

namespace {

constexpr int CS_MAX_PARTS = 256;

__device__ __forceinline__ void transpose_tile(int bx, int by, const bf16_t* __restrict__ in, bf16_t* __restrict__ out,
                                                        int rows, int cols, int64_t ld_in, int64_t ld_out,
                                                        const bf16_t* __restrict__ scale = nullptr) {
  __shared__ bf16_t tile[64][64 + 2];
  const int r0 = by * 64, c0 = bx * 64;
  const int tx = threadIdx.x & 15, ty = threadIdx.x >> 4;
#pragma unroll
  for (int k = 0; k < 4; ++k) {
    const int r = r0 + ty + k * 16, c = c0 + tx * 4;
    if (r < rows) {
      const float sc = scale ? (float)scale[r] : 1.f;
      if (c + 3 < cols && (ld_in & 3) == 0) {
        bf16x4 v = *reinterpret_cast<const bf16x4*>(in + (int64_t)r * ld_in + c);
#pragma unroll
        for (int j = 0; j < 4; ++j) tile[ty + k * 16][tx * 4 + j] = scale ? (bf16_t)(sc * (float)v[j]) : v[j];
      } else {
        for (int j = 0; j < 4; ++j)
          if (c + j < cols) tile[ty + k * 16][tx * 4 + j] = scale ? (bf16_t)(sc * (float)in[(int64_t)r * ld_in + c + j]) : in[(int64_t)r * ld_in + c + j];
// ... 704 lines not shown
            if (lane == 0) wave_n[wid] = __popcll(m);
            __syncthreads();
            int before = base;
#pragma unroll
            for (int w = 0; w < 4; ++w) {
              if (w < wid) before += wave_n[w] * per;
              base += wave_n[w] * per;
            }
            if (live) {
              const int64_t first = a.seg[i].row0 - a.seg[i].base[k] + (int64_t)u * (a.seg[i].wps > 0 ? a.seg[i].S : 256);
              int* dst = a.lists[l].list + 2 * (before + __popcll(m & ((1ull << lane) - 1ull)) * per);
              for (int w = 0; w < per; ++w) {
                dst[2 * w] = (a.seg[i].prob[k] << 28) | (int)(first + w * 256);
                dst[2 * w + 1] = (256 << 16) | 1;
              }
            }
            __syncthreads();
          }
          if (a.seg[i].odd) {
            const int nw = (a.seg[i].B + 255) / 256;
            if (tid < nw) {
              int* dst = a.lists[l].list + 2 * (base + tid);
              dst[0] = (a.seg[i].prob[k] << 28) | (int)(a.seg[i].row0 - a.seg[i].base[k] + (int64_t)tid * 256 * a.seg[i].S + a.seg[i].S - 1);
              dst[1] = (min(256, a.seg[i].B - tid * 256) << 16) | a.seg[i].S;
            }
            base += nw;
          }
        }
      }
      if (tid == 0) *a.lists[l].count = base;
    }
    return;
  }
  int i = 0;
#pragma unroll
  for (int j = 1; j < MW_MAX_SEG; ++j)
    if (j < a.nseg && (int)blockIdx.x >= a.seg[j].unit0) i = j;
  const int u = (int)blockIdx.x - a.seg[i].unit0;
  const int64_t seg_rows = (int64_t)a.seg[i].S * a.seg[i].B;
  const int64_t ubeg = (int64_t)u * (a.seg[i].wps > 0 ? a.seg[i].S : 256);
  const int64_t uend = min(ubeg + (a.seg[i].wps > 0 ? a.seg[i].S : 256), seg_rows);
  const int64_t r0 = ubeg + (int64_t)blockIdx.y * MW_PIECE, r1 = min(r0 + MW_PIECE, uend);
  if (r0 >= r1 || mw_unit_live(a.seg[i], u)) return;
  const int nrows = (int)(r1 - r0);
  for (int o = 0; o < a.nout; ++o) {
    const int c8 = a.out[o].cols >> 3;
    bf16_t* base = a.out[o].ptr + (a.seg[i].row0 + r0) * a.out[o].ld;
    const bf16_t* src = a.out[o].src;
    if (src) src += (a.seg[i].row0 + r0) * a.out[o].lds;
    for (int r = wid; r < nrows; r += 4)
      for (int c = lane; c < c8; c += 64)
        *reinterpret_cast<uint4*>(base + (int64_t)r * a.out[o].ld + c * 8) =
            src ? *reinterpret_cast<const uint4*>(src + (int64_t)r * a.out[o].lds + c * 8) : make_uint4(0u, 0u, 0u, 0u);
  }
}

}

extern "C" {

int op_transpose_scaled(const void* in, void* out, int64_t rows, int64_t cols, int64_t ld_in, int64_t ld_out, const void* scale,
                        void* stream) {
  OP_CHECK_ARG(in && out && rows >= 0 && cols >= 0, "transpose: bad args");
  if (rows == 0 || cols == 0) return OP_OK;
  dim3 grid(ceil_div(cols, 64), ceil_div(rows, 64));
  hipLaunchKernelGGL(transpose_kernel, grid, dim3(256), 0, (hipStream_t)stream, (const bf16_t*)in, (bf16_t*)out, (int)rows,
                     (int)cols, ld_in, ld_out, (const bf16_t*)scale);
  OP_LAUNCH_CHECK();
  return OP_OK;
}
int op_transpose(const void* in, void* out, int64_t rows, int64_t cols, int64_t ld_in, int64_t ld_out, void* stream) {
  return op_transpose_scaled(in, out, rows, cols, ld_in, ld_out, nullptr, stream);
}

int op_transpose_batched(const void* table, int64_t n, int64_t total_tiles, void* stream) {
  OP_CHECK_ARG(table && n > 0 && total_tiles > 0, "transpose_batched: bad args");
  hipLaunchKernelGGL(transpose_batched_kernel, dim3((unsigned)total_tiles), dim3(256), 0, (hipStream_t)stream,
                     (const TransposeDesc*)table, (int)n);
  OP_LAUNCH_CHECK();
  return OP_OK;
}
int64_t op_transpose_desc_bytes(void) { return (int64_t)sizeof(TransposeDesc); }

int64_t op_colsum_workspace_bytes(int64_t N) { return (int64_t)CS_MAX_PARTS * N * (int64_t)sizeof(float); }

int op_colsum(const void* x, const void* y, const float* rowscale, int64_t rows_per_sample, const void* mul, void* out,
              void* workspace, int64_t M, int64_t N, int accumulate, int out_dtype, void* stream) {
  OP_CHECK_ARG(x && out && workspace, "colsum: null pointer");
  OP_CHECK_ARG(N > 0 && N % 8 == 0, "colsum: N must be a multiple of 8");
  hipStream_t s = (hipStream_t)stream;
  int parts = (int)((M + 63) / 64);
  if (parts > CS_MAX_PARTS) parts = CS_MAX_PARTS;
  if (parts < 1) parts = 1;
  dim3 grid(ceil_div(N, 512), parts);
  hipLaunchKernelGGL(colsum_partial_kernel, grid, dim3(256), 0, s, (const bf16_t*)x, (const bf16_t*)y, rowscale,
                     (int)(rows_per_sample > 0 ? rows_per_sample : 1), (float*)workspace, M, (int)N, N);
  OP_LAUNCH_CHECK();
  if (out_dtype == OP_DT_BF16)
    hipLaunchKernelGGL((partials_reduce_kernel<bf16_t>), dim3(ceil_div(N, 32)), dim3(256), 0, s, (const float*)workspace, parts,
                       N, (int)N, (const bf16_t*)mul, (bf16_t*)out, accumulate);
  else
    hipLaunchKernelGGL((partials_reduce_kernel<float>), dim3(ceil_div(N, 32)), dim3(256), 0, s, (const float*)workspace, parts,
                       N, (int)N, (const bf16_t*)mul, (float*)out, accumulate);
  OP_LAUNCH_CHECK();
  return OP_OK;
}
// ... 370 lines not shown
    if ((sg.wps > 0 ? S[i] : 256) > unit_rows) unit_rows = sg.wps > 0 ? S[i] : 256;
    for (int k = 0; k < 2; ++k) {
      const int64_t l = seg_list[i * 2 + k];
      sg.list[k] = (int)l;
      if (l < 0) { sg.list[k] = -1; continue; }
      OP_CHECK_ARG(l < nlist && seg_prob[i * 2 + k] >= 0 && seg_prob[i * 2 + k] <= 2 && seg_base[i * 2 + k] >= 0 &&
                   seg_base[i * 2 + k] <= row0[i] && row0[i] - seg_base[i * 2 + k] + S[i] * B[i] + 256 * wps[i] < ((int64_t)1 << 28),
                   "live_mwindows: segment %d: bad list reference %d", i, k);
      sg.prob[k] = (int)seg_prob[i * 2 + k]; sg.base[k] = seg_base[i * 2 + k];
      need[l] += (int64_t)sg.units * (sg.wps > 0 ? sg.wps : 1) + (sg.odd ? (sg.B + 255) / 256 : 0);
    }
  }
  a.nunits = units;
  for (int l = 0; l < (int)nlist; ++l) {
    OP_CHECK_ARG(windows[l] && n_windows[l] && max_windows[l] >= need[l], "live_mwindows: list %d: null, or room for %lld entries (%lld needed)", l,
                 (long long)max_windows[l], (long long)need[l]);
    a.lists[l].list = windows[l]; a.lists[l].count = n_windows[l];
  }
  for (int o = 0; o < (int)nout; ++o) {
    OP_CHECK_ARG(out[o] && ((uintptr_t)out[o] & 15) == 0 && out_cols[o] >= 8 && out_cols[o] % 8 == 0 && out_ld[o] % 8 == 0 && out_ld[o] >= out_cols[o] && out_rows[o] >= last_row &&
                 out_cols[o] < ((int64_t)1 << 31), "live_mwindows: output %d: null or not 16-byte aligned, cols / ld %% 8, or fewer than %lld rows", o, (long long)last_row);
    a.out[o].ptr = (bf16_t*)out[o]; a.out[o].ld = out_ld[o]; a.out[o].cols = (int)out_cols[o];
    if (out_src && out_src[o]) {
      OP_CHECK_ARG(out_src_ld && ((uintptr_t)out_src[o] & 15) == 0 && out_src_ld[o] % 8 == 0 && out_src_ld[o] >= out_cols[o] && out_src[o] != out[o],
                   "live_mwindows: source of output %d: not 16-byte aligned, ld %% 8 or ld < cols, or the output itself", o);
      a.out[o].src = (const bf16_t*)out_src[o]; a.out[o].lds = out_src_ld[o];
    }
  }
  hipLaunchKernelGGL(live_mwindows_kernel, dim3(units + (int)nlist, (int)((unit_rows + MW_PIECE - 1) / MW_PIECE)), dim3(256), 0, (hipStream_t)stream, a);
  OP_LAUNCH_CHECK();
  return OP_OK;
}

int op_live_mwindows(int64_t nseg, const float* const* ps, const int64_t* ps_stride, const int64_t* row0, const int64_t* S, const int64_t* B,
                     const int64_t* wps, const int64_t* odd, const int64_t* seg_list, const int64_t* seg_prob, const int64_t* seg_base, int64_t nlist,
                     int32_t* const* windows,
                     int32_t* const* n_windows, const int64_t* max_windows, int64_t nout, void* const* out, const int64_t* out_ld,
                     const int64_t* out_cols, const int64_t* out_rows, void* stream) {
  return live_mwindows_impl(nseg, ps, ps_stride, row0, S, B, wps, odd, seg_list, seg_prob, seg_base, nlist, windows, n_windows, max_windows, nout,
                            out, out_ld, out_cols, out_rows, nullptr, nullptr, stream);
}

int op_live_mwindows_fwd(int64_t nseg, const float* const* ps, const int64_t* ps_stride, const int64_t* row0, const int64_t* S, const int64_t* B,
                         const int64_t* wps, const int64_t* odd, const int64_t* seg_list, const int64_t* seg_prob, const int64_t* seg_base,
                         int64_t nlist, int32_t* const* windows, int32_t* const* n_windows, const int64_t* max_windows, int64_t nout,
                         void* const* out, const int64_t* out_ld, const int64_t* out_cols, const int64_t* out_rows,
                         const void* const* out_src, const int64_t* out_src_ld, void* stream) {
  OP_CHECK_ARG(nout >= 1 && out_src && out_src_ld, "live_mwindows_fwd: outputs with their source array (entries may be null)");
  return live_mwindows_impl(nseg, ps, ps_stride, row0, S, B, wps, odd, seg_list, seg_prob, seg_base, nlist, windows, n_windows, max_windows, nout,
                            out, out_ld, out_cols, out_rows, out_src, out_src_ld, stream);
}

}
```

one-peace_amd/hip.py:

```python
import ctypes
import os
from ctypes import c_double, c_float, c_int, c_int64, c_void_p

import torch

_HERE = os.path.dirname(os.path.abspath(__file__))
LIB_PATH = os.environ.get("ONEPEACE_HIP_LIB") or os.path.join(_HERE, "lib", "libonepeace_hip.so")
_lib = None

DT_BF16, DT_F32 = 0, 1
EPI_BIAS, EPI_F32, EPI_GEGLU, EPI_RESID = 0, 1, 2, 3
PROF_GEMM, PROF_ATTN = 0, 1
ATTN_RESIDENT_MAX_S = 320

P = c_void_p
I64 = c_int64

SIGNATURES = {
    "op_abi_version": (c_int, []),
    "op_last_error": (ctypes.c_char_p, []),
    "op_prof_enable": (c_int, [c_int]),
    "op_prof_reserve": (c_int, [c_int]),
    "op_prof_collect": (c_int, [P, P, P, c_int]),
    "op_layernorm_fwd": (c_int, [P, P, P, P, P, P, I64, I64, c_float, c_int, c_int, P, P]),
# ... 5 lines not shown
                           c_int, P, I64, I64, P, I64, P]),
    "op_gemm_nt_grouped": (c_int, [I64, P, P, I64, P, I64, P, P, I64, P, P, P, I64, P, P, P, I64, I64, c_int, I64, P, I64, P]),
    "op_gemm_tn": (c_int, [P, I64, P, I64, P, I64, I64, I64, I64, c_int, P, I64, I64, P]),
    "op_gemm_tn_grouped_counter_bytes": (I64, []),
    "op_gemm_tn_grouped_plan": (I64, [I64, P, P, P, I64, I64, P, I64]),
    "op_gemm_tn_grouped": (c_int, [I64, P, P, P, P, P, P, P, P, P, P, P, P, P, P, P, I64, P]),
    "op_gemm_tn_grouped_lists": (c_int, [I64, P, P, P, P, P, P, P, P, P, P, P, P, P, P, P, P, P, I64, P]),
    "op_live_ktiles": (c_int, [I64, P, P, P, P, I64, P, P, P, P, P]),
    "op_live_mwindows": (c_int, [I64, P, P, P, P, P, P, P, P, P, P, I64, P, P, P, I64, P, P, P, P, P]),
    "op_gemm_nt_grouped_windows": (c_int, [I64, P, P, I64, P, I64, P, I64, I64, I64, P, P, I64, I64, I64, P]),
    "op_live_mwindows_fwd": (c_int, [I64, P, P, P, P, P, P, P, P, P, P, I64, P, P, P, I64, P, P, P, P, P, P, P]),
    "op_gemm_nt_grouped_windows_fwd": (c_int, [I64, P, P, I64, P, I64, I64, P, P, I64, P, I64, P, P, P, I64, I64, c_int, P, P, I64, I64,
                                               I64, P]),
    "op_gemm_nt_batched": (c_int, [P, I64, I64, P, I64, I64, P, I64, P, I64, I64, I64, I64, I64, I64, P]),
    "op_audio_conv1_ln_gelu_fwd": (c_int, [P, I64, P, P, P, P, P, P, P, I64, I64, c_float, P]),
    "op_audio_conv1_ln_gelu_bwd_workspace_bytes": (I64, [I64]),
    "op_audio_conv1_ln_gelu_bwd": (c_int, [P, P, I64, P, P, P, P, P, P, P, P, P, P, P, I64, I64, c_int, P]),
    "op_transpose": (c_int, [P, P, I64, I64, I64, I64, P]),
    "op_transpose_scaled": (c_int, [P, P, I64, I64, I64, I64, P, P]),
    "op_transpose_batched": (c_int, [P, I64, I64, P]),
    "op_transpose_desc_bytes": (I64, []),
    "op_colsum_workspace_bytes": (I64, [I64]),
    "op_colsum_segments": (c_int, [P, P, P, P, P, I64, I64, I64, c_int, P]),
    "op_resid_bwd_workspace_bytes": (I64, [I64]),
    "op_resid_bwd": (c_int, [P, P, P, P, I64, P, P, P, P, P, I64, I64, c_int, P, P]),
    "op_gamma_grad_finish": (c_int, [P, I64, P, P, P, P, P, P, P, I64, c_int, P]),
    "op_ln_geglu_bwd": (c_int, [P, P, P, P, P, P, P, P, I64, I64, P, P, P, I64, I64, c_int, P]),
    "op_ln_geglu_fwd": (c_int, [P, P, I64, P, P, P, P, P, I64, I64, c_float, P]),
    "op_colsum": (c_int, [P, P, P, I64, P, P, P, I64, I64, c_int, c_int, P]),
    "op_geglu_bwd": (c_int, [P, P, P, P, P, I64, P]),
    "op_scale_rows": (c_int, [P, P, P, I64, P, I64, I64, P]),
    "op_l2norm_fwd": (c_int, [P, P, P, I64, I64, c_float, c_int, P]),
    "op_l2norm_bwd": (c_int, [P, P, P, P, I64, I64, c_int, P]),
    "op_infonce_rows": (c_int, [P, I64, I64, I64, I64, c_float, c_float, P, P, P, c_int, P]),
    "op_adamw_step": (c_int, [P, P, P, P, I64, c_float, c_float, c_float, c_float, c_float, I64, c_float, P, c_float, P]),
    "op_adamw_step_groups": (c_int, [P, P, P, P, I64, P, P, P, I64, c_float, c_float, c_float, c_float, I64, c_float, P, c_float, P]),
    "op_adamw_step_groups_master": (c_int, [P, P, P, P, P, I64, P, P, P, I64, c_float, c_float, c_float, c_float, I64, c_float, P,
                                           c_float, P]),
    "op_ema_step": (c_int, [P, P, I64, c_float, c_float, P]),
    "op_adamw_step_groups_ema": (c_int, [P, P, P, P, P, P, I64, P, P, P, I64, c_float, c_float, c_float, c_float, I64, c_float, P,
                                        c_float, c_float, c_float, P]),
    "op_adamw_step_shard": (c_int, [P, P, I64, I64, I64, P, P, P, P, P, P, P, I64, c_float, c_float, c_float, c_float, I64, c_float, P,
                                   c_float, c_float, c_float, P]),
    "op_sqnorm": (c_int, [P, I64, P, P, P]),
    "op_relpos_bias_build": (c_int, [P, P, I64, P, I64, I64, I64, c_int, P]),
    "op_relpos_bias_bwd": (c_int, [P, I64, I64, P, P, I64, P, I64, P, P, I64, P]),
    "op_relpos_bias_build_ids": (c_int, [P, P, I64, P, P, I64, I64, I64, I64, c_int, P]),
    "op_relpos_bias_fold_ids": (c_int, [P, P, P, I64, I64, I64, I64, I64, P]),
    "op_attn_fwd": (c_int, [P, P, P, I64, P, I64, P, P, P, I64, P, I64, I64, I64, I64, I64, I64, c_float, I64, P]),
    "op_attn_bias_frag_elems": (I64, [I64, I64]),
    "op_attn_bias_pack": (c_int, [P, P, I64, I64, I64, P]),
    "op_attn_bwd_delta": (c_int, [P, P, I64, P, I64, I64, I64, I64, P]),
    "op_attn_bwd": (c_int, [P, P, P, I64, P, P, I64, P, P, P, I64, P, P, P, P, P, P, I64, P, I64, I64, I64, I64, I64, c_float, I64, P]),
    "op_quant_fp8_rows": (c_int, [P, I64, P, I64, P, I64, I64, P]),
    "op_layernorm_fwd_q8": (c_int, [P, P, P, P, P, P, P, P, I64, I64, c_float, P]),
    "op_ln_geglu_fwd_q8": (c_int, [P, P, I64, P, P, P, P, P, P, P, I64, I64, c_float, P]),
    "op_gemm_nt_fp8": (c_int, [P, I64, P, P, P, I64, P, P, P, P, I64, P, P, P, I64, P, P, I64, I64, I64, I64, c_int, I64, P]),
    "op_rows_gather": (c_int, [P, P, P, I64, P, P, P, P, P, P, P, I64, I64, P]),
    "op_rows_merge": (c_int, [P, P, P, P, I64, P, P, P, P, P, P, P, I64, I64, P]),
    "op_rows_map": (c_int, [P, P, I64, P, P, P, P, P, P, P, I64, P]),
    "op_sim_topk_splits": (I64, [I64, I64, I64]),
    "op_sim_topk_workspace_bytes": (I64, [I64, I64, I64, I64]),
    "op_sim_topk": (c_int, [P, I64, P, I64, I64, I64, I64, I64, P, P, P, I64, I64, P]),
    "op_image_resize_normalize": (c_int, [P, I64, P, P, I64, P, I64, I64, P, P, P, c_int, P, I64, P]),
    "op_audio_normalize_pad": (c_int, [P, I64, P, P, I64, I64, I64, P, I64, c_int, P, I64, P]),
    "op_audio_resample": (c_int, [P, I64, P, P, I64, P, I64, P, I64, P]),
    "op_average_precision_workspace_bytes": (I64, [I64, I64]),
    "op_average_precision": (c_int, [P, I64, P, I64, I64, I64, P, P, P, I64, P]),
    "op_row_loss": (c_int, [P, c_int, I64, P, c_int, I64, I64, I64, c_int, c_float, c_float, c_float, P, P, P, P, P]),
    "op_box_loss": (c_int, [P, c_int, P, I64, c_float, P, P, P]),
    "op_attn_pool_fwd": (c_int, [P, P, I64, I64, P, P, I64, P, P, I64, I64, I64, I64, P]),
    "op_attn_pool_bwd": (c_int, [P, P, P, I64, I64, P, P, P, P, I64, I64, P, I64, I64, I64, I64, P]),
}


PROBE_SIGNATURES = {
    "op_last_error": (ctypes.c_char_p, []),
    "op_probe_mfma16": (c_int, [P, P, P, c_int, P]),
    "op_probe_mfma32": (c_int, [P, P, P, c_int, P]),
    "op_probe_tr16": (c_int, [P, P, P, c_int, P]),
    "op_probe_glds": (c_int, [P, P, c_int, P, P]),
    "op_probe_mfma_f8": (c_int, [P, P, P, P, P, c_int, P]),
    "op_probe_mfma_rate": (c_int, [P, P, P, c_int, c_int, P]),
    "op_probe_lds_atomic": (c_int, [P, P, c_int, c_int, c_int, P]),
    "op_probe_occupy": (c_int, [P, ctypes.c_longlong, c_int, ctypes.c_longlong, P, P]),
}


class Tuning:

    def __init__(self):
        self.reset()

    def reset(self):
        self.tile_mode = 0
        self.fullline = 2
        self.tail_rows = 1
        self.gm = 0
        self.force_splits = 0
        self.glds = 1
        self.sched = int(os.environ.get("ONEPEACE_TUNE_SCHED", "0"))
        self.fp8_small = 0
        self.merge_dbias = 1
        self.resident = 1
        self.attn_waves = 0
        self.attn_pers = 1
# ... 809 lines not shown
    t = torch.arange(nseg, device=dev)
    r = torch.searchsorted(bucket_seg[1:], t, right=True)
    rc = r.clamp(max=num_rel - 1)
    seg = torch.full((nseg + 1,), S * S, dtype=torch.int64, device=dev)
    seg[:nseg] = torch.where(r < num_rel, pair_off[rc] + (t - bucket_seg[rc]) * PAIR_SEG, S * S)
    res = (order.to(torch.int32), seg.to(torch.int32), bucket_seg.to(torch.int32), nseg)
    bucket_i32._op_pairs = (key, res)
    return res


def relpos_bias_bwd(dbias_f32, bucket_i32, num_rel, S, Spad):
    heads = dbias_f32.shape[0]
    pos, seg, bucket_seg, nseg = relpos_pairs(bucket_i32, S, num_rel)
    dtable = torch.empty(num_rel, heads, dtype=torch.float32, device=dbias_f32.device)
    partial = torch.empty(nseg, heads, dtype=torch.float32, device=dbias_f32.device)
    _check(lib().op_relpos_bias_bwd(ptr(dbias_f32), S, Spad, ptr(pos), ptr(seg), nseg, ptr(bucket_seg), num_rel, ptr(partial), ptr(dtable),
                                    heads, stream()), "op_relpos_bias_bwd")
    return dtable


def relpos_bias_build_ids(table, bucket_i32, ids_i32, Kpad, transposed=False):
    B, K = ids_i32.shape
    heads = table.shape[1]
    out = torch.empty(B, heads, K, Kpad, dtype=torch.bfloat16, device=table.device)
    _check(lib().op_relpos_bias_build_ids(ptr(table), ptr(bucket_i32), bucket_i32.stride(0), ptr(ids_i32), ptr(out), B, heads, K, Kpad,
                                          int(transposed), stream()), "op_relpos_bias_build_ids")
    return out


def relpos_bias_bwd_ids(dbias_f32, bucket_i32, ids_i32, num_rel):
    B, heads, K, Kpad = dbias_f32.shape
    Sfull = bucket_i32.shape[0]
    dense = torch.zeros(heads, Sfull, Sfull, dtype=torch.float32, device=dbias_f32.device)
    _check(lib().op_relpos_bias_fold_ids(ptr(dbias_f32), ptr(ids_i32), ptr(dense), Sfull, B, heads, K, Kpad, stream()),
           "op_relpos_bias_fold_ids")
    return relpos_bias_bwd(dense, bucket_i32, num_rel, Sfull, Sfull)


def attn_spad(S):
    return ((S + 127) // 128) * 128


def _bias_bstride(bias):
    return bias.stride(0) if bias is not None and bias.dim() == 4 else 0


def attn_bias_pack(image, S):
    n_img = image.numel() // (image.shape[-2] * image.shape[-1])
    out = torch.empty(lib().op_attn_bias_frag_elems(n_img, S), dtype=torch.bfloat16, device=image.device)
    _check(lib().op_attn_bias_pack(ptr(image), ptr(out), n_img, S, image.shape[-1], stream()), "op_attn_bias_pack")
    return out


def attn_fwd(q, k, v, ld, B, S, heads, scale, bias=None, key_pad=None, Spad=0, out=None, want_lse=True, bias_frag=None):
    dev = q.device
    H = heads * 64
    Spad = Spad or attn_spad(S)
    if out is None:
        out = torch.empty(B * S, H, dtype=torch.bfloat16, device=dev)
    lse = torch.empty(B, heads, Spad, dtype=torch.float32, device=dev) if want_lse else None
    _check(lib().op_attn_fwd(ptr(q), ptr(k), ptr(v), ld, ptr(bias), _bias_bstride(bias), ptr(bias_frag), ptr(key_pad), ptr(out), out.stride(0),
                             ptr(lse), Spad, B, S, Spad, heads, 64, scale, TUNE.attn_fwd(), stream()), "op_attn_fwd")
    return out, lse


def attn_bwd(q, k, v, ld, dout, out, lse, B, S, heads, scale, bias=None, biasT=None, key_pad=None, Spad=0, dqkv=None,
             want_dbias=False, bias_frag=None):
    dev = q.device
    H = heads * 64
    Spad = Spad or attn_spad(S)
    delta = torch.empty(B, heads, Spad, dtype=torch.float32, device=dev)
    assert out.stride(0) == dout.stride(0)
    if dqkv is None:
        dqkv = torch.empty(B * S, 3 * H, dtype=torch.bfloat16, device=dev)
    per_sample = bias is not None and bias.dim() == 4
    dbias = attn_dbias_buffer(B, S, heads, Spad, dev, per_sample) if want_dbias else None
    dq, dk, dv = dqkv[:, :H], dqkv[:, H:2 * H], dqkv[:, 2 * H:]
    attn_bwd_launch(q, k, v, ld, dout, bias, biasT, key_pad, lse, delta, dq, dk, dv, dqkv.stride(0), dbias, B, S, Spad, heads, scale,
                    bias_frag, out=out)
    if dbias is None:
        return dqkv, None
    return dqkv, (dbias if per_sample else dbias.sum(0))


def attn_bwd_launch(q, k, v, ld, dout, bias, biasT, key_pad, lse, delta, dq, dk, dv, ldg, dbias, B, S, Spad, heads, scale,
                    bias_frag=None, out=None):
    _check(lib().op_attn_bwd(ptr(q), ptr(k), ptr(v), ld, ptr(dout), ptr(out), dout.stride(0), ptr(bias), ptr(biasT), ptr(bias_frag),
                             _bias_bstride(bias),
                             ptr(key_pad), ptr(lse), ptr(delta), ptr(dq), ptr(dk), ptr(dv), ldg, ptr(dbias), B, S, Spad, heads,
                             64, scale, TUNE.attn_bwd(), stream()), "op_attn_bwd")


def attn_dbias_buffer(B, S, heads, Spad, device, per_sample=False):
    slabs = B if per_sample else lib().op_attn_bwd_dbias_slabs(B, S, heads, TUNE.attn_bwd())
    return torch.zeros(slabs, heads, S, Spad, dtype=torch.float32, device=device)


class profile_kernels:

    def __enter__(self):
        lib().op_prof_enable(1)
        return self

    def __exit__(self, *exc):
        lib().op_prof_enable(0)

    @staticmethod
    def collect(n=4):
        ms = (c_double * n)()
        cnt = (c_int64 * n)()
        work = (c_double * n)()
        lib().op_prof_collect(ms, cnt, work, n)
        return [dict(ms=ms[i], count=cnt[i], work=work[i]) for i in range(n)]


class KeptRows:

    def __init__(self, segs, lists, base, full_rows, scale, pad=256):
        n = len(segs)
        assert 1 <= n <= 4
        self.lists, self.full_rows, self.scale, self.nseg = lists, int(full_rows), float(scale), n
        self.S = [int(s[1]) for s in segs]
        self.n_samples = [int(s[2]) for s in segs]
        self.n_kept = [len(s[3]) for s in segs]
        self.src_row0 = [int(s[0]) for s in segs]
        self.dst_rows = [-(-(k * S) // pad) * pad for k, S in zip(self.n_kept, self.S)]
        self.dst_row0, self.off_kept, self.off_inv = [], [], []
        r, o = 0, int(base)
        for k, ns, dr in zip(self.n_kept, self.n_samples, self.dst_rows):
            self.dst_row0.append(r)
            self.off_kept.append(o)
            self.off_inv.append(o + k)
            r, o = r + dr, o + k + ns
        self.total, self.list_end = r, o
        arr = lambda v: (c_int64 * n)(*v)
        self._c = tuple(arr(v) for v in (self.src_row0, self.dst_row0, self.S, self.n_kept, self.dst_rows, self.n_samples))
        self._c_kept, self._c_inv = arr(self.off_kept), arr(self.off_inv)

    def kept_list(self, i):
        return self.lists[self.off_kept[i]:self.off_kept[i] + self.n_kept[i]]

    def rowmap(self):
        m = getattr(self, "_rowmap", None)
# ... 305 lines not shown
```

one-peace_amd/ops.py:

```python
import math
import os
import weakref

import torch
import torch.nn.functional as F

from . import hip

_wt_cache = {}
_cache_epoch = 0


_refresh_plan = None


def invalidate_weight_cache():
    global _cache_epoch
    _cache_epoch += 1


def refresh_weight_cache():
    global _cache_epoch, _refresh_plan
    _cache_epoch += 1
    if not FP8_FFN and (_fp8_cache or _fp8_derived_cache):
# ... 218 lines not shown
    key = (M, N, K, ws, hip.TUNE.gemm())
    if key not in _dense_dgrad_plans:
        _, splits, _, tail = hip.gemm_plan(M, N, K, hip.EPI_BIAS, False, ws)
        _dense_dgrad_plans[key] = splits == 1 and (tail == 0 or hip.gemm_plan(tail, N, K, hip.EPI_BIAS, False, ws)[1] == 1)
    return _dense_dgrad_plans[key]


def _dgrad_windows(segs, lists, outs, dense):
    if not SKIP_ZERO_DGRAD or all(q[0] is None for q in segs) or len(segs) > 4 or len(lists) > 4 or len(outs) > 4:
        return None
    if any(N % 256 != 0 or K % 64 != 0 or K < 128 or not _dense_dgrad_sums_k_in_one_piece(M, N, K, outs[0].device) for M, N, K in dense):
        return None
    if any(ps is not None and (ps.dtype != torch.float32 or not ps.is_contiguous() or ps.numel() <= (B - 1) * st) for ps, _, _, B, st in segs):
        return None
    if any(o.dtype != torch.bfloat16 or o.stride(0) % 8 != 0 or o.shape[1] % 8 != 0 for o in outs):
        return None
    return hip.live_mwindows(segs, lists, outs)


def _dgrad_listed(As, Ws, outs, windows, segs):
    return hip.gemm_nt_windows(As, Ws, outs, windows, max([sg.S for sg in segs if hip.mwindow_rule(sg.S)[1]] or [1]))


SKIP_ZERO_FWD = os.environ.get("ONEPEACE_SKIP_ZERO_FWD", "1") != "0"
_dense_fwd_plans = {}


def _dense_fwd_sums_k_in_one_piece(M, N, K, epilogue, has_bias, device):
    scratch = hip.splitk_scratch(M, N, K, epilogue, device)
    ws = scratch.numel() if scratch is not None else 0
    key = (M, N, K, epilogue, has_bias, ws, hip.TUNE.gemm())
    if key not in _dense_fwd_plans:
        _, splits, _, tail = hip.gemm_plan(M, N, K, epilogue, has_bias, ws)
        _dense_fwd_plans[key] = splits == 1 and (tail == 0 or hip.gemm_plan(tail, N, K, epilogue, has_bias, ws)[1] == 1)
    return _dense_fwd_plans[key]


def _fwd_windows_apply(segs, nlists, nouts, dense, device, flags=True):
    if not SKIP_ZERO_FWD or not flags or all(q[0] is None for q in segs) or len(segs) > 4 or nlists > 4 or nouts > 4:
        return False
    if any(ps is not None and (ps.dtype != torch.float32 or not ps.is_contiguous() or ps.numel() <= (B - 1) * st) for ps, _, _, B, st in segs):
        return False
    if any(S * B >= 1 << 27 or row0 + S * B + 256 * 64 >= 1 << 28 for _, row0, S, B, _ in segs):
        return False
    mrs = max([q[2] for q in segs if hip.mwindow_rule(q[2])[1]] or [1])
    for M, N, K, epi, has_bias in dense:
        if N % 256 != 0 or K % 64 != 0 or K < 128 or M * max(N, K) >= 1 << 30 or mrs * max(N, K) >= 1 << 23:
            return False
        if not _dense_fwd_sums_k_in_one_piece(M, N, K, epi, has_bias, device):
            return False
    return True


class _WgradQueue:

    def __init__(self):
        self.items, self.done, self.after, self.armed, self.epoch = [], [], [], False, 0
        self.lists = []

    def reset(self):
        self.items, self.done, self.after, self.armed = [], [], [], False
        self.lists = []
        self.epoch += 1

    @staticmethod
    def _span(out):
        lo = out.data_ptr()
        return lo, lo + ((out.shape[0] - 1) * out.stride(0) + out.shape[1]) * out.element_size()

    def add(self, dy, x, out, params, side=None, after=None, ktiles=None):
        lo, hi = self._span(out)
        for it in self.items:
            l2, h2 = self._span(it[2])
            if lo < h2 and l2 < hi:
                self.flush()
                break
        self.items.append((dy, x, out, True, side))
        self.lists.append(ktiles)
        self.done.extend(params)
        if after is not None:
            self.after.append(after)
        if not self.armed:
            self.armed = True
            epoch = self.epoch
            torch.autograd.Variable._execution_engine.queue_callback(lambda: self._end_of_backward(epoch))
        if len(self.items) >= hip.TN_GROUP_MAX:
            self.flush()

    def _end_of_backward(self, epoch):
        if epoch != self.epoch:
            return
        self.armed = False
        self.flush()

    def flush(self):
        items, done, after, lists = self.items, self.done, self.after, self.lists
        self.items, self.done, self.after, self.lists = [], [], [], []
        if items:
            kw = {"ktiles": lists} if any(k is not None for k in lists) else {}
            if len(items) == 1 or not hip.gemm_tn_grouped(items, **kw):
                for dy, x, out, _, side in items:
                    if side is None:
                        hip.gemm_tn(dy, x, out, True)
                    else:
                        prod = hip.gemm_tn(dy, x, None, False)
                        W, rowdot, gamma = side
# ... 430 lines not shown
class StreamSeg:
    __slots__ = ("name", "B", "S", "row0", "bias", "key_pad", "pad")

    def __init__(self, name, B, S, row0, bias=None, key_pad=None, pad=0):
        self.name, self.B, self.S, self.row0, self.bias, self.key_pad, self.pad = name, B, S, row0, bias, key_pad, pad

    @property
    def tokens(self):
        return self.B * self.S

    @property
    def rows(self):
        return self.B * self.S + self.pad

    @property
    def end(self):
        return self.row0 + self.B * self.S + self.pad

    def frag(self, limit):
        return self.bias.frag if self.bias is not None and self.S <= limit else None


def _attn_forward(x2, P, segs, heads, scale, rowscale, rps, keep, want_y=True, xmap=None, out=None, listed=False):
    H = x2.shape[1]
    xln1, mean1, rstd1 = hip.layernorm_fwd(x2, P["ln1_w"], P["ln1_b"], want_stats=keep, x_rows=xmap)
    Nr = xln1.shape[0]
    full = _qkv_rows_that_fill_whole_rounds(Nr, 3 * H) if QKV_ROUND_SPLIT and H % 128 == 0 else Nr
    win, mrs, qkv, x_mid = None, 1, None, None
    if (listed and rowscale is not None and xmap is None and out is None and not (keep and want_y) and H % 256 == 0 and Nr % rps == 0
            and sum(sg.rows for sg in segs) == Nr and all(sg.S % rps == 0 and sg.row0 % rps == 0 for sg in segs)):
        wsegs = [(rowscale[sg.row0 // rps:], sg.row0, sg.S, sg.B, sg.S // rps) for sg in segs]
        dense = [(m, 3 * H, H, hip.EPI_BIAS, True) for m in ((full, Nr - full) if full < Nr else (Nr,))] + [(Nr, H, H, hip.EPI_RESID, True)]
        if _fwd_windows_apply(wsegs, 1, 2, dense, x2.device, flags=not any(sg.pad for sg in segs)):
            qkv = torch.empty(Nr, 3 * H, dtype=x2.dtype, device=x2.device)
            x_mid = torch.empty_like(x2)
            win = hip.live_mwindows_fwd(wsegs, [[(i, 0, 0) for i in range(len(segs))]], [qkv, x_mid], [None, x2])[0]
            mrs = max([sg.S for sg in segs if hip.mwindow_rule(sg.S)[1]] or [1])
    if win is not None and hip.gemm_nt_windows_fwd([xln1], [[P["wq"], P["wk"], P["wv"]]], [[P["bq"], None, P["bv"]]], [qkv], win, H,
                                                   max_row_stride=mrs):
        pass
    elif H % 128 == 0:
        if full < Nr:
            qkv = torch.empty(Nr, 3 * H, dtype=x2.dtype, device=x2.device)
            for lo, hi in ((0, full), (full, Nr)):
                hip.gemm_nt(xln1[lo:hi], [P["wq"], P["wk"], P["wv"]], [P["bq"], None, P["bv"]], n_seg=H, N=3 * H, out=qkv[lo:hi])
        else:
            qkv = hip.gemm_nt(xln1, [P["wq"], P["wk"], P["wv"]], [P["bq"], None, P["bv"]], n_seg=H, N=3 * H)
    else:
        qkv = torch.empty(xln1.shape[0], 3 * H, dtype=x2.dtype, device=x2.device)
        for i, (w, b) in enumerate(((P["wq"], P["bq"]), (P["wk"], None), (P["wv"], P["bv"]))):
            hip.gemm_nt(xln1, [w], [b] if b is not None else None, out=qkv[:, i * H:(i + 1) * H], ldc=3 * H)
    attn = torch.empty_like(xln1)
    lses = []
    for sg in segs:
        r = slice(sg.row0, sg.end)
        _, lse = hip.attn_fwd(qkv[r, :H], qkv[r, H:2 * H], qkv[r, 2 * H:], 3 * H, sg.B, sg.S, heads, scale,
                              sg.bias.image.detach() if sg.bias is not None else None, sg.key_pad, hip.attn_spad(sg.S), out=attn[r],
                              want_lse=keep, bias_frag=sg.frag(hip.ATTN_RESIDENT_MAX_S))
        lses.append(lse)
        if sg.pad:
            attn[sg.end - sg.pad:sg.end].zero_()
    if P["aln_w"] is not None:
        aln, mean_a, rstd_a = hip.layernorm_fwd(attn, P["aln_w"], P["aln_b"], want_stats=keep)
    else:
        aln, mean_a, rstd_a = attn, None, None
    y1 = torch.empty_like(xln1) if keep and want_y else None
    if win is None or not hip.gemm_nt_windows_fwd([aln], [[P["wo"]]], [[P["bo"]]], [x_mid], win, H, epilogue=hip.EPI_RESID, resids=[x2],
                                                  gammas=[P["g1"]], rowscales=[rowscale], rows_per_sample=[rps], max_row_stride=mrs):
        x_mid = hip.gemm_nt(aln, [P["wo"]], [P["bo"]], epilogue=hip.EPI_RESID, resid=x2, gamma=P["g1"], rowscale=rowscale,
                            rows_per_sample=rps, h0=y1, out=out, resid_rows=xmap)
    if not keep:
        return x_mid, None
    acts = dict(xln1=xln1, mean1=mean1, rstd1=rstd1, qkv=qkv, attn=attn, aln=aln, mean_a=mean_a, rstd_a=rstd_a, y1=y1)
    for i, lse in enumerate(lses):
        acts["lse%d" % i] = lse
    return x_mid, acts


QKV_ROUND_SPLIT = os.environ.get("ONEPEACE_QKV_ROUND_SPLIT", "1") != "0"
SKIP_ROW_TABLES = os.environ.get("ONEPEACE_SKIP_ROW_TABLES", "1") != "0"


def _row_tables(kept):
    return kept is not None and SKIP_ROW_TABLES and not FP8_FFN


def _qkv_rows_that_fill_whole_rounds(rows, n_out, cus=256, max_tail=512):
    tn, tm = (n_out + 255) // 256, (rows + 255) // 256
    rounds = -(-tm * tn // cus)
    tm_main = (rounds - 1) * cus // tn
    full = tm_main * 256
    return full if 0 < rows - full <= max_tail and tm_main > 0 else rows


GEGLU_SPLIT = os.environ.get("ONEPEACE_GEGLU_SPLIT", "1") != "0"
SEPARATE_DELTA = os.environ.get("ONEPEACE_SEPARATE_DELTA", "0") == "1"


def _geglu_split(Fd, fln_w):
    return GEGLU_SPLIT and fln_w is not None and Fd % 256 == 0


def _register_direct(ctx, names, params, needs):
    ctx.direct = tuple((n, q) for n, q, ng in zip(names, params, needs) if ng and q is not None and _direct_grad(q))
    for _, q in ctx.direct:
        q._op_pending = getattr(q, "_op_pending", 0) + 1


def _targets(direct, *names):
    if all(n in direct for n in names):
        return [direct[n].grad for n in names], True
    return [None] * len(names), False


def _finish(direct, G, names, values, accumulated):
    for n, v in zip(names, values):
        if accumulated:
            _direct_grad_done(direct[n])
        else:
            G[n] = v


def _return_grads(names, params, G, direct):
    out = []
    for n, q in zip(names, params):
        g = G.get(n) if q is not None else None
        if g is not None and n in direct:
            direct[n].grad.add_(g.view_as(direct[n].grad))
# ... 152 lines not shown
        kt1 = None
        whole = rowscale is not None and kept is None and N % rps == 0 and not any(sg.pad for sg in segs) and sum(sg.rows for sg in segs) == N
        if whole:
            kt1 = _live_ktiles([(rowscale, 0, rps, N // rps)], [(0, N)], dx_mid.device)[0]
        if ctx.dg_fused:
            g0 = torch.empty(H, dtype=torch.float32, device=dx_mid.device)
            dy1 = _resid_backward(dx_mid, None, P["g1"], rowscale, rps, "g1", "bo", direct, G, needs, g0=g0, rows=xmap)
            rowdot, (rd_wo,) = _rowdot_slots(dx_mid.device, [P["wo"]])
            weight_grad("wo", dy1, A["aln"], side=(P["wo"], rd_wo, P["g1"]),
                        after=_gamma_finish_hook(rowdot, direct["g1"], [(P["bo"], g0)] if P["bo"] is not None else [], True), ktiles=kt1)
            wo_t = _transposed(P["wo"], scale=P["g1"])
        else:
            dy1 = _resid_backward(dx_mid, A["y1"], P["g1"], rowscale, rps, "g1", "bo", direct, G, needs, rows=xmap)
            if needs["wo"]:
                weight_grad("wo", dy1, A["aln"], ktiles=kt1)
            wo_t = None
        upstream = ("ln1_w", "ln1_b", "wq", "bq", "wk", "wv", "bv", "aln_w", "aln_b")
        dx = None
        if need_x or any(want_dbias) or any(needs[n] for n in upstream):
            need_dxln1 = need_x or needs["ln1_w"] or needs["ln1_b"]
            win1, daln, dxln1 = None, None, None
            if whole and all(sg.S % rps == 0 and sg.row0 % rps == 0 for sg in segs):
                daln = torch.empty(N, H, dtype=dy1.dtype, device=dy1.device)
                dxln1 = torch.empty_like(daln) if need_dxln1 else None
                win1 = _dgrad_windows([(rowscale[sg.row0 // rps:], sg.row0, sg.S, sg.B, sg.S // rps) for sg in segs],
                                      [[(i, 0, 0) for i in range(nseg)]], [daln] + ([dxln1] if need_dxln1 else []),
                                      [(N, H, H)] + ([(N, H, 3 * H)] if need_dxln1 else []))
            wo_in = wo_t if wo_t is not None else _transposed(P["wo"])
            if win1 is None or not _dgrad_listed([dy1], [wo_in], [daln], win1[0], segs):
                daln = hip.gemm_nt(dy1, [wo_in])
            if P["aln_w"] is not None:
                want = needs["aln_w"] or needs["aln_b"]
                (tw, tb), acc = _targets(direct, "aln_w", "aln_b") if want else ((None, None), False)
                dattn, dw_, db_ = hip.layernorm_bwd(daln, A["attn"], P["aln_w"], P["aln_b"], A["mean_a"], A["rstd_a"], dw=tw, db=tb,
                                                    accumulate=acc, need_wgrad=want)
                if want:
                    _finish(direct, G, ("aln_w", "aln_b"), (dw_, db_), acc)
            else:
                dattn = daln
            qkv_names = ("wq", "wk", "wv")
            order = _adjacent_grads(direct, qkv_names) if all(needs[n] for n in qkv_names) and H % 8 == 0 else None
            cols = tuple(order) if order else qkv_names
            slot = {n: i for i, n in enumerate(cols)}
            qkv = A["qkv"]
            dqkv = torch.empty_like(qkv)
            for i, sg in enumerate(segs):
                r = slice(sg.row0, sg.end)
                if sg.pad:
                    dqkv[sg.end - sg.pad:sg.end].zero_()
                dparts = {n: dqkv[r, slot[n] * H:(slot[n] + 1) * H] for n in qkv_names}
                _attn_backward(qkv[r], dattn[r], A["attn"][r], A["lse%d" % i], sg.B, sg.S, heads, scale,
                               sg.bias.image.detach() if sg.bias is not None else None, sg.bias.imageT if sg.bias is not None else None,
                               sg.key_pad, sg.bias.grad_accumulator(sg.B) if want_dbias[i] else None, sg.frag(384),
                               dparts["wq"], dparts["wk"], dparts["wv"])
            bias_of = {"wq": "bq", "wv": "bv"}
            bnames = tuple(bias_of[n] for n in cols if n in bias_of and needs[bias_of[n]])
            if bnames:
                tgt, acc = _targets(direct, *bnames)
                if H % 8 == 0:
                    outs = [None, None, None]
                    for n, t_ in zip(bnames, tgt):
                        outs[slot["wq" if n == "bq" else "wv"]] = t_ if acc else torch.empty(H, dtype=dqkv.dtype, device=dqkv.device)
                    hip.colsum_segments(dqkv, H, outs, accumulate=acc)
                    _finish(direct, G, bnames, tuple(outs[slot["wq" if n == "bq" else "wv"]] for n in bnames), acc)
                else:
                    sums = hip.colsum(dqkv)
                    for n in bnames:
                        i = slot["wq" if n == "bq" else "wv"]
                        G[n] = sums[i * H:(i + 1) * H]
            if order:
                wgrad_into(dqkv, A["xln1"], _span(direct, order), [direct[n] for n in order], ktiles=kt1)
            elif any(n in direct for n in qkv_names) or not all(needs[n] for n in qkv_names):
                for n in qkv_names:
                    if needs[n]:
                        weight_grad(n, dqkv[:, slot[n] * H:(slot[n] + 1) * H], A["xln1"], ktiles=kt1)
            else:
                dW = wgrad(dqkv, A["xln1"])
                G["wq"], G["wk"], G["wv"] = dW[:H], dW[H:2 * H], dW[2 * H:]
            if need_dxln1:
                wqkv_t = _transposed(tuple(P[n] for n in cols))
                if win1 is None or not _dgrad_listed([dqkv], [wqkv_t], [dxln1], win1[0], segs):
                    dxln1 = hip.gemm_nt(dqkv, [wqkv_t])
                want = needs["ln1_w"] or needs["ln1_b"]
                (tw, tb), acc = _targets(direct, "ln1_w", "ln1_b") if want else ((None, None), False)
                dx, dw_, db_ = hip.layernorm_bwd(dxln1, x2, P["ln1_w"], P["ln1_b"], A["mean1"], A["rstd1"], add=dx_mid, dw=tw, db=tb,
                                                 accumulate=acc, need_wgrad=want, dx=torch.empty_like(dx_full) if mapped else None,
                                                 x_rows=xmap)
                if want:
                    _finish(direct, G, ("ln1_w", "ln1_b"), (dw_, db_), acc)
        if dx is None and need_x:
            dx = dx_full
        elif dx is not None and mapped:
            hip.rows_merge(dx_full, None, kept, out=dx)
        elif dx is not None and kept is not None:
            dx = hip.rows_merge(dx_full, dx, kept)
        flush_wgrads()
        grads = _return_grads(ATTN_PARAMS, params, G, direct)
        dimgs = []
        for sg, w in zip(segs, want_dbias):
            if w and not getattr(sg.bias, "_grad_routed", False):
                sg.bias._grad_routed = True
                img = sg.bias.image
                dimgs.append(torch.zeros((), dtype=img.dtype, device=img.device).expand(img.shape))
            else:
                dimgs.append(None)
        return (dx, None, None, None, None, None, None, *dimgs, *grads)

# ... 252 lines not shown
        if need_dxln2:
            if dxln2 is None:
                dxln2 = torch.empty(N, H, dtype=dt, device=dev)
            rs = [slice(sg.row0, sg.end) for sg in segs]
            wts = [_transposed(tuple(P[n] for n in cols)) for cols in colsets]
            if fp8b:
                for r, wt in zip(rs, wts):
                    hip.gemm_nt_fp8(*hip.quant_fp8_rows(dh[r]), *[[x] for x in _fp8_derived(wt)], out=dxln2[r])
            elif wins is not None and _dgrad_listed([dh[r] for r in rs], wts, [dxln2[r] for r in rs], wins[nseg], segs):
                pass
            elif nseg == 1 or hip.gemm_nt_grouped([dh[r] for r in rs], wts, outs=[dxln2[r] for r in rs]) is None:
                for r, wt in zip(rs, wts):
                    hip.gemm_nt(dh[r], [wt], out=dxln2[r])
            want = needs["ln2_w"] or needs["ln2_b"]
            (tw, tb), acc = _targets(direct, "ln2_w", "ln2_b") if want else ((None, None), False)
            dx, dw_, db_ = hip.layernorm_bwd(dxln2, x2, P["ln2_w"], P["ln2_b"], A["mean2"], A["rstd2"], add=dout, dw=tw, db=tb,
                                             accumulate=acc, need_wgrad=want, dx=torch.empty_like(dout_full) if mapped else None, x_rows=xmap)
            if want:
                _finish(direct, G, ("ln2_w", "ln2_b"), (dw_, db_), acc)
        if dx is None and need_x:
            dx = dout_full
        elif dx is not None and mapped:
            hip.rows_merge(dout_full, None, kept, out=dx)
        elif dx is not None and kept is not None:
            dx = hip.rows_merge(dout_full, dx, kept)
        grads = _return_grads(names, params, G, direct)
        return (dx, None, None, None, None, *grads)


def ffn_branch_multi(x2, segs, pss, shared, own, save_acts=True, kept=None):
    flat = list(shared)
    for o in own:
        flat += list(o)
    return FfnBranchMultiFn.apply(x2, segs, tuple(pss), _save_flags(save_acts), kept, *flat)


_SCALE_ROWS = {}


def kept_segments(kept, segs, device):
    out = []
    for i, sg in enumerate(segs):
        key_pad = sg.key_pad.index_select(0, kept.kept_list(i)) if sg.key_pad is not None else None
        out.append(StreamSeg(sg.name, kept.n_kept[i], sg.S, kept.dst_row0[i], sg.bias, key_pad, pad=kept.dst_rows[i] - kept.n_kept[i] * sg.S))
    key = (device, kept.scale)
    vec = _SCALE_ROWS.get(key)
    if vec is None or vec.numel() < kept.total + 8:
        if len(_SCALE_ROWS) > 256:
            _SCALE_ROWS.clear()
        vec = _SCALE_ROWS[key] = torch.full((max(kept.full_rows, kept.total) + 8,), kept.scale, dtype=torch.float32, device=device)
    return out, vec


def _attn_backward(qkv, dattn, attn, lse, B, S, heads, scale, bias_img, biasT, key_pad, dbias_acc, bias_frag, dq, dk, dv):
    H = heads * 64
    dev = qkv.device
    Spad = hip.attn_spad(S)
    delta = torch.empty(B, heads, Spad, dtype=torch.float32, device=dev)
    if attn.stride(0) != dattn.stride(0) or SEPARATE_DELTA:
        hip._check(hip.lib().op_attn_bwd_delta(hip.ptr(dattn), hip.ptr(attn), dattn.stride(0), hip.ptr(delta), B, S, Spad, heads,
                                               hip.stream()), "op_attn_bwd_delta")
        attn = None
    hip.attn_bwd_launch(qkv[:, :H], qkv[:, H:2 * H], qkv[:, 2 * H:], 3 * H, dattn, bias_img, biasT, key_pad, lse, delta, dq, dk,
                        dv, dq.stride(0), dbias_acc, B, S, Spad, heads, scale, bias_frag, out=attn)


def attn_branch(x, bias, key_pad, ps, heads, params, save_acts=False):
    B, S, H = x.shape
    seg = StreamSeg("x", B, S, 0, bias, key_pad)
    out = AttnBranchFn.apply(x.reshape(B * S, H), [seg], ps, S, heads, _save_flags(save_acts), None, bias.image if bias is not None else None, *params)
    return out.view(B, S, H)


def attn_branch_multi(x2, segs, ps_rows, heads, params, save_acts=False, kept=None):
    return AttnBranchFn.apply(x2, segs, ps_rows, 1, heads, _save_flags(save_acts), kept,
                              *[sg.bias.image if sg.bias is not None else None for sg in segs], *params)


def _save_flags(save_acts):
    return int(bool(save_acts)) | (2 if torch.is_grad_enabled() else 0) | (4 if RECOMPUTE_CHEAP and save_acts else 0)


def ffn_branch(x, ps, params, save_acts=False):
    B, S, H = x.shape
    P = dict(zip(FFN_PARAMS, params))
    out = ffn_branch_multi(x.reshape(B * S, H), [StreamSeg("x", B, S, 0)], [ps], [P[n] for n in FFN_SHARED], [[P[n] for n in FFN_OWN]],
                           save_acts)
    return out.view(B, S, H)


class L2NormalizeFn(torch.autograd.Function):

    @staticmethod
    def forward(ctx, x):
        y, inv = hip.l2norm_fwd(x.contiguous())
        ctx.save_for_backward(y, inv)
        return y

    @staticmethod
    def backward(ctx, dy):
        y, inv = ctx.saved_tensors
        return hip.l2norm_bwd(dy.contiguous(), y, inv)


def l2_normalize(x):
    return L2NormalizeFn.apply(x)


class InfoNCEFn(torch.autograd.Function):

    @staticmethod
    def forward(ctx, a_local, b_local, a_all, b_all, scale, rank, label_smoothing):
        b = a_local.shape[0]
        t0 = rank * b
        scale_f = scale.detach().float().reshape(1)
        sims, rows = [], []
        for loc, allv in ((a_local, b_all), (b_local, a_all)):
# ... 225 lines not shown
```

Before: 205.7.

## Skip attention work for samples with zero path-scale (dropped) in fwd/bwd

Adds kept-sample lists built on device from the per-sample drop-path scale, and kept-aware variants of the persistent attention forward, dQ and dK/dV kernels. These iterate only over live samples and zero the output or gradients of dropped ones. The aim is to avoid computing attention for samples whose branch output is multiplied by zero under stochastic depth. It adds a device list-building kernel, extra scalar indirection in the kernels, and route conditions (S range, scale exactness) that limit where it applies.

```diff
diff --git a/include/onepeace_hip.h b/include/onepeace_hip.h
--- a/include/onepeace_hip.h
+++ b/include/onepeace_hip.h
@@ -98,6 +98,20 @@
                 const float* lse, float* delta, void* dq,
                 void* dk, void* dv, int64_t ldg, float* dbias, int64_t B, int64_t S, int64_t Spad, int64_t heads,
                 int64_t head_dim, float scale, int64_t tune, void* stream);
+int op_live_samples(int64_t nseg, const float* const* ps, const int64_t* ps_stride, const int64_t* row0, const int64_t* S, const int64_t* B,
+                    int32_t* const* kept, int32_t* const* pos, int64_t nout, void* const* out, const int64_t* out_ld, const int64_t* out_cols,
+                    const int64_t* out_rows, void* stream);
+int op_live_samples_fill(int64_t nseg, const int64_t* row0, const int64_t* S, const int64_t* B, int32_t* const* pos, int64_t nout,
+                         void* const* out, const int64_t* out_ld, const int64_t* out_cols, const int64_t* out_rows, void* stream);
+int op_attn_fwd_kept(const void* q, const void* k, const void* v, int64_t ld, const void* bias, int64_t bias_batch_stride,
+                     const void* bias_frag, const void* key_pad, void* out, int64_t ldo, float* lse, int64_t lse_ld, int64_t B,
+                     int64_t S, int64_t Spad, int64_t heads, int64_t head_dim, float scale, int64_t tune, const int* kept, const int* pos,
+                     void* stream);
+int op_attn_bwd_kept(const void* q, const void* k, const void* v, int64_t ld, const void* dout, const void* out, int64_t ldo,
+                     const void* bias, const void* biasT, const void* bias_frag, int64_t bias_batch_stride, const void* key_pad,
+                     const float* lse, float* delta, void* dq, void* dk, void* dv, int64_t ldg, float* dbias, int64_t B, int64_t S,
+                     int64_t Spad, int64_t heads, int64_t head_dim, float scale, int64_t tune, const int* kept, const int* pos,
+                     void* stream);
 
 int op_relpos_bias_build(const void* table, const int* bucket, int64_t bucket_ld, void* out, int64_t heads, int64_t S,
                          int64_t Spad, int transposed, void* stream);
diff --git a/one-peace_amd/csrc/attention.hip b/one-peace_amd/csrc/attention.hip
--- a/one-peace_amd/csrc/attention.hip
+++ b/one-peace_amd/csrc/attention.hip
@@ -20,6 +20,22 @@
   int B, S, Spad, heads;
   float scale;
 };
+
+__device__ __forceinline__ int kept_sample(const int* __restrict__ kept, int i, int B) {
+  int b = __builtin_amdgcn_readfirstlane(kept[i]);
+  asm volatile("" : "+s"(b));
+  return min(max(b, 0), B - 1);
+}
+__device__ __forceinline__ int kept_below(const int* __restrict__ pos, int b, int B) {
+  int n = __builtin_amdgcn_readfirstlane(pos[b]);
+  asm volatile("" : "+s"(n));
+  return min(max(n, 0), B);
+}
+__device__ __forceinline__ int kept_count(const int* __restrict__ pos, int B) { return kept_below(pos, B, B); }
+__device__ __forceinline__ int kept_item(const int* __restrict__ kept, int it, int heads, int B) {
+  const int i = it / heads;
+  return kept_sample(kept, i, B) * heads + (it - i * heads);
+}
 
 __device__ __forceinline__ bf16x8 pack8(const float* a, const float* b) {
   bf16x8 r;
@@ -472,11 +488,22 @@
   asm volatile("s_nop 4\n\tglobal_load_dword %0, %1, %2 offset:%3" : "=v"(d) : "v"(voff), "s"(sbase), "n"(OFF));
 }
 
-template <bool HAS_BIAS, bool HAS_PAD>
+template <bool HAS_BIAS, bool HAS_PAD, bool KEPT = false>
 __global__ __launch_bounds__(PERS_NW * 64, 2) void attn_fwd_pers_kernel(AttnArgs p, const bf16_t* __restrict__ bias_frag, int rows_pad,
-                                                                         int nitems) {
+                                                                         int nitems, const int* __restrict__ kept,
+                                                                         const int* __restrict__ pos) {
   extern __shared__ __attribute__((aligned(16))) char smem[];
+  if constexpr (KEPT) nitems = min(nitems, kept_count(pos, p.B) * p.heads);
   const int tid = threadIdx.x, lane = tid & 63;
+  if constexpr (KEPT) {
+    const bf16x4 zero4 = {(bf16_t)0.f, (bf16_t)0.f, (bf16_t)0.f, (bf16_t)0.f};
+    for (int idx = blockIdx.x; idx < p.B * p.heads; idx += gridDim.x) {
+      const int b = idx / p.heads, h = idx - b * p.heads;
+      if (kept_below(pos, b + 1, p.B) != kept_below(pos, b, p.B)) continue;
+      bf16_t* op = p.out + (int64_t)b * p.S * p.ldo + h * HD + (tid & 15) * 4;
+      for (int r = tid >> 4; r < p.S; r += (PERS_NW * 64) >> 4) *reinterpret_cast<bf16x4*>(op + (int64_t)r * p.ldo) = zero4;
+    }
+  }
   const int wid = __builtin_amdgcn_readfirstlane(tid >> 6);
   const int g = lane >> 4, t = lane & 15;
   const int KVB = 2 * rows_pad * 128;
@@ -582,11 +609,13 @@
 
   int item = blockIdx.x;
   const int step = gridDim.x;
+  int xitem = item;
   if (item < nitems) {
-    for (int j = 0; j < npiece; ++j) piece(item, 0, j);
-    load_q(item, qi_main[0], qn[0]);
-    load_q(item, qi_main[1], qn[1]);
-    small_loads(item, 0);
+    if constexpr (KEPT) xitem = kept_item(kept, item, p.heads, p.B);
+    for (int j = 0; j < npiece; ++j) piece(KEPT ? xitem : item, 0, j);
+    load_q(KEPT ? xitem : item, qi_main[0], qn[0]);
+    load_q(KEPT ? xitem : item, qi_main[1], qn[1]);
+    small_loads(KEPT ? xitem : item, 0);
   }
   int buf = 0, prev_item = -1;
   auto wait_all = [&]() {
@@ -614,14 +643,15 @@
   };
 
   for (; item < nitems; item += step, buf ^= 1) {
-    const int b = item / p.heads, h = item - b * p.heads;
+    const int cur = KEPT ? xitem : item;
+    const int b = cur / p.heads, h = cur - b * p.heads;
     const int64_t row_base = (int64_t)b * p.S;
     __syncthreads();
     bf16x8 qf[2][2] = {{qn[0][0], qn[0][1]}, {qn[1][0], qn[1][1]}};
     const bool more = item + step < nitems;
-    const int nxt = more ? item + step : item;
+    const int nxt = KEPT ? (more ? kept_item(kept, item + step, p.heads, p.B) : xitem) : (more ? item + step : item);
     if (has_left && prev_item >= 0 && wid == ((prev_item / step) & (PERS_NW - 1))) merge_left(prev_item, buf ^ 1);
-    prev_item = item;
+    prev_item = cur;
 
     const char* ldsK = smem + buf * KVB;
     const char* ldsV = ldsK + rows_pad * 128;
@@ -651,9 +681,9 @@
       }
       __builtin_amdgcn_sched_barrier(0);
       if constexpr (FULL) {
-        small_loads(item, kt + 1);
+        small_loads(cur, kt + 1);
       } else {
-        late_loads(nxt, item);
+        late_loads(nxt, cur);
         small_loads(nxt, 0);
       }
       __builtin_amdgcn_sched_barrier(0);
@@ -870,6 +900,7 @@
       }
     }
     wait_all();
+    if constexpr (KEPT) xitem = nxt;
   }
   if (has_left && prev_item >= 0) {
     __syncthreads();
@@ -1596,8 +1627,9 @@
   }
 }
 
-template <bool HAS_BIAS, bool HAS_PAD, int NT, int LASTB, bool LEFT>
-__device__ __forceinline__ void attn_bwd_dq_pers_body(const AttnBwdArgs& p, char* smem, int rows_pad, int nqh, int qhalf0) {
+template <bool HAS_BIAS, bool HAS_PAD, int NT, int LASTB, bool LEFT, bool KEPT>
+__device__ __forceinline__ void attn_bwd_dq_pers_body(const AttnBwdArgs& p, char* smem, int rows_pad, int nqh, int qhalf0, const int* __restrict__ kept,
+                                                      const int* __restrict__ pos) {
   const int tid = threadIdx.x, lane = tid & 63;
   const int wid = __builtin_amdgcn_readfirstlane(tid >> 6);
   const int g = lane >> 4, t = lane & 15;
@@ -1607,6 +1639,21 @@
   const int qhalf = qhalf0, h = (blockIdx.x / nqh) % p.heads, chunk = blockIdx.x / (nqh * p.heads);
   const int b_begin = chunk * p.bchunk, b_end = min(p.B, b_begin + p.bchunk);
   if (b_begin >= b_end) return;
+  const int l_begin = KEPT ? kept_below(pos, b_begin, p.B) : b_begin, l_end = KEPT ? kept_below(pos, b_end, p.B) : b_end;
+  if constexpr (KEPT) {
+    const bf16x4 zero4 = {(bf16_t)0.f, (bf16_t)0.f, (bf16_t)0.f, (bf16_t)0.f};
+    const int r0 = qhalf * (PERS_NW * 16), r1 = qhalf == nqh - 1 ? p.S : min(p.S, r0 + PERS_NW * 16);
+    for (int b = b_begin; b < b_end; ++b) {
+      if (kept_below(pos, b + 1, p.B) != kept_below(pos, b, p.B)) continue;
+      const int64_t at = (int64_t)b * p.S * p.ldg + h * HD + (tid & 15) * 4;
+      for (int r = r0 + (tid >> 4); r < r1; r += (PERS_NW * 64) >> 4) {
+        *reinterpret_cast<bf16x4*>(p.dq + at + (int64_t)r * p.ldg) = zero4;
+        *reinterpret_cast<bf16x4*>(p.dk + at + (int64_t)r * p.ldg) = zero4;
+        *reinterpret_cast<bf16x4*>(p.dv + at + (int64_t)r * p.ldg) = zero4;
+      }
+    }
+    if (l_begin >= l_end) return;
+  }
   const int qblk = qhalf * PERS_NW + wid;
   const bool active = qblk < min(nqb, 2 * PERS_NW);
   constexpr bool has_left = LEFT;
@@ -1716,9 +1763,11 @@
 #pragma unroll
     for (int j = 0; j < 2; ++j) accl[i][j] = (f32x4){0.f, 0.f, 0.f, 0.f};
 
-  for (int j = 0; j < npiece; ++j) piece(b_begin, 0, j);
-  query_loads(b_begin, vo_q, vo_o, vo_lse, qn, don, oon, lsen);
-  small_loads(b_begin, 0);
+  int bcur = b_begin;
+  if constexpr (KEPT) bcur = kept_sample(kept, l_begin, p.B);
+  for (int j = 0; j < npiece; ++j) piece(KEPT ? bcur : b_begin, 0, j);
+  query_loads(KEPT ? bcur : b_begin, vo_q, vo_o, vo_lse, qn, don, oon, lsen);
+  small_loads(KEPT ? bcur : b_begin, 0);
   int buf = 0, prev_b = -1;
   auto merge_left = [&](int b, int sb) {
     const float* sc = scratch + sb * (PERS_NW * 64);
@@ -1733,13 +1782,14 @@
                  "+v"(padn[0]), "+v"(padn[1]), "+v"(padn[2]), "+v"(padn[3]) : : "memory");
   };
   wait_all();
-  for (int b = b_begin; b < b_end; ++b, buf ^= 1) {
+  for (int li = l_begin; li < l_end; ++li, buf ^= 1) {
+    const int b = KEPT ? bcur : li;
     __syncthreads();
     const bf16x8 qf[2] = {qn[0], qn[1]}, dof[2] = {don[0], don[1]};
     const float dl = delta_from_frags(dof, oon);
     const float nl2 = -lsen * LOG2E;
     if (active && g == 0 && q0w + t < p.S) p.delta_w[((int64_t)b * p.heads + h) * p.Spad + q0w + t] = dl;
-    const int nxt = b + 1 < b_end ? b + 1 : b;
+    const int nxt = KEPT ? (li + 1 < l_end ? kept_sample(kept, li + 1, p.B) : b) : (b + 1 < b_end ? b + 1 : b);
     if (has_left && prev_b >= 0 && wid == (prev_b & (PERS_NW - 1))) merge_left(prev_b, buf ^ 1);
     prev_b = b;
     const char* ldsK = smem + buf * KVB;
@@ -1925,6 +1975,7 @@
     }
 
     wait_all();
+    if constexpr (KEPT) bcur = nxt;
   }
   if (has_left && prev_b >= 0) {
     __syncthreads();
@@ -1965,18 +2016,19 @@
   }
 }
 
-template <bool HAS_BIAS, bool HAS_PAD, int NT, int LASTB>
-__global__ __launch_bounds__(PERS_NW * 64, 2) void attn_bwd_dq_pers_kernel(AttnBwdArgs p, int rows_pad, int nqh) {
+template <bool HAS_BIAS, bool HAS_PAD, int NT, int LASTB, bool KEPT = false>
+__global__ __launch_bounds__(PERS_NW * 64, 2) void attn_bwd_dq_pers_kernel(AttnBwdArgs p, int rows_pad, int nqh, const int* __restrict__ kept,
+                                                                            const int* __restrict__ pos) {
   extern __shared__ __attribute__((aligned(16))) char smem[];
   const int qhalf = blockIdx.x % nqh;
   const bool lone = ((p.S + 15) >> 4) > 2 * PERS_NW && qhalf == nqh - 1;
   if constexpr (NT == 5) {
     if (lone) {
-      attn_bwd_dq_pers_body<HAS_BIAS, HAS_PAD, NT, LASTB, true>(p, smem, rows_pad, nqh, qhalf);
+      attn_bwd_dq_pers_body<HAS_BIAS, HAS_PAD, NT, LASTB, true, KEPT>(p, smem, rows_pad, nqh, qhalf, kept, pos);
       return;
     }
   }
-  attn_bwd_dq_pers_body<HAS_BIAS, HAS_PAD, NT, LASTB, false>(p, smem, rows_pad, nqh, qhalf);
+  attn_bwd_dq_pers_body<HAS_BIAS, HAS_PAD, NT, LASTB, false, KEPT>(p, smem, rows_pad, nqh, qhalf, kept, pos);
 }
 
 constexpr int PERS_SCRL = 136;
@@ -1995,9 +2047,11 @@
   asm volatile("s_nop 4\n\tbuffer_store_dwordx2 %0, %1, %2, 0 offen\n\ts_nop 1" ::"v"(data), "v"(voff), "s"(rsrc) : "memory");
 }
 
-template <bool HAS_BIAS, bool HAS_PAD, int NT, bool LONE>
-__global__ __launch_bounds__(PERS_NW * 64, 2) void attn_bwd_dkdv_pers_kernel(AttnBwdArgs p, int rows_pad, int nitems) {
+template <bool HAS_BIAS, bool HAS_PAD, int NT, bool LONE, bool KEPT = false>
+__global__ __launch_bounds__(PERS_NW * 64, 2) void attn_bwd_dkdv_pers_kernel(AttnBwdArgs p, int rows_pad, int nitems, const int* __restrict__ kept,
+                                                                              const int* __restrict__ pos) {
   extern __shared__ __attribute__((aligned(16))) char smem[];
+  if constexpr (KEPT) nitems = min(nitems, kept_count(pos, p.B) * p.heads);
   const int tid = threadIdx.x, lane = tid & 63;
   const int wid = __builtin_amdgcn_readfirstlane(tid >> 6);
   const int g = lane >> 4, t = lane & 15;
@@ -2109,12 +2163,14 @@
   const int step = gridDim.x;
   using I0 = std::integral_constant<int, 0>;
   using I1 = std::integral_constant<int, 1>;
+  int xitem = item;
   if (item < nitems) {
-    for (int j = 0; j < npiece; ++j) piece(item, 0, j);
-    if constexpr (LONE) kv_loads(item, kf, vf);
-    else kv_loads(item, kn, vn);
-    bias_loads(item, I0{}, I0{});
-    bias_loads(item, I0{}, I1{});
+    if constexpr (KEPT) xitem = kept_item(kept, item, p.heads, p.B);
+    for (int j = 0; j < npiece; ++j) piece(KEPT ? xitem : item, 0, j);
+    if constexpr (LONE) kv_loads(KEPT ? xitem : item, kf, vf);
+    else kv_loads(KEPT ? xitem : item, kn, vn);
+    bias_loads(KEPT ? xitem : item, I0{}, I0{});
+    bias_loads(KEPT ? xitem : item, I0{}, I1{});
   }
 #define DKDV_WAIT_LOADS(NST)                                                                                                                  \
   do {                                                                                                                                     \
@@ -2142,7 +2198,8 @@
   };
 
   for (; item < nitems; item += step, buf ^= 1) {
-    const int b = item / p.heads, h = item - b * p.heads;
+    const int cur = KEPT ? xitem : item;
+    const int b = cur / p.heads, h = cur - b * p.heads;
     asm volatile("s_waitcnt lgkmcnt(0)" ::: "memory");
     __builtin_amdgcn_s_barrier();
     asm volatile("" ::: "memory");
@@ -2154,9 +2211,9 @@
     }
     const bool kdead[2] = {HAS_PAD && kdn[0] != 0u, HAS_PAD && kdn[1] != 0u};
     const bool ldead = HAS_PAD && LONE && kdl != 0u;
-    const int nxt = item + step < nitems ? item + step : item;
+    const int nxt = KEPT ? (item + step < nitems ? kept_item(kept, item + step, p.heads, p.B) : xitem) : (item + step < nitems ? item + step : item);
     if (LONE && prev_item >= 0 && wid == ((prev_item / step) & (PERS_NW - 1))) merge_lone(prev_item, buf ^ 1);
-    prev_item = item;
+    prev_item = cur;
     const char* ldsQ = smem + buf * BUFB;
     const char* ldsO = ldsQ + QBY;
     const float* ldsL = reinterpret_cast<const float*>(ldsQ + 2 * QBY);
@@ -2282,7 +2339,7 @@
       __builtin_amdgcn_sched_barrier(0);
       if (wave_active) half(QT * 64, std::integral_constant<int, 2>{}, kf, vf, bn[0], dvT, dkT);
       __builtin_amdgcn_sched_barrier(0);
-      if constexpr (!LAST) bias_loads(item, QN{}, I0{});
+      if constexpr (!LAST) bias_loads(cur, QN{}, I0{});
       if constexpr (HAS_BIAS && QT > 0) {
         if constexpr (!LAST) asm volatile("s_waitcnt vmcnt(%2)" : "+v"(bn[1][0]), "+v"(bn[1][1]) : "n"(BPPT + NBH));
         else asm volatile("s_waitcnt vmcnt(0)" : "+v"(bn[1][0]), "+v"(bn[1][1]));
@@ -2291,10 +2348,10 @@
       if (wave_active && QT * 64 + 32 < p.S) half(QT * 64 + 32, std::integral_constant<int, 2>{}, kf, vf, bn[1], dvT, dkT);
       __builtin_amdgcn_sched_barrier(0);
       if constexpr (!LAST) {
-        bias_loads(item, QN{}, I1{});
+        bias_loads(cur, QN{}, I1{});
         if constexpr (HAS_BIAS) asm volatile("s_waitcnt vmcnt(%2)" : "+v"(bn[0][0]), "+v"(bn[0][1]) : "n"(NBH));
       } else {
-        lone_bias_loads(item);
+        lone_bias_loads(cur);
         bias_loads(nxt, I0{}, I0{});
         bias_loads(nxt, I0{}, I1{});
         if constexpr (!LONE) kv_loads(nxt, kn, vn);
@@ -2356,6 +2413,7 @@
       }
       DKDV_WAIT_LOADS(16);
     }
+    if constexpr (KEPT) xitem = nxt;
   }
   if (LONE && prev_item >= 0) {
     __syncthreads();
@@ -2542,18 +2600,10 @@
   return OP_OK;
 }
 
-extern "C" {
-
-int64_t op_attn_bwd_dbias_slabs(int64_t B, int64_t S, int64_t heads, int64_t tune) {
-  if ((tune & BWD_SEPARATE_DBIAS) || ceil_div(S, BKV) > 6) return ceil_div(B, sep_bchunk(B, S, heads));
-  const int64_t n = dbias_chunks(B, S, heads, true, (tune & BWD_ROUND2_CHUNKS) != 0, (int)((tune >> BWD_CHUNKS_SHIFT) & BWD_CHUNKS_MASK));
-  if (!(tune & BWD_NO_PERS_DQ) && pers_bwd_shape(S)) return max(n, (int64_t)pers_bwd_chunks(B, S, heads));
-  return n;
-}
-
-int op_attn_fwd(const void* q, const void* k, const void* v, int64_t ld, const void* bias, int64_t bias_batch_stride,
-                const void* bias_frag, const void* key_pad, void* out, int64_t ldo, float* lse, int64_t lse_ld, int64_t B,
-                int64_t S, int64_t Spad, int64_t heads, int64_t head_dim, float scale, int64_t tune, void* stream) {
+static int attn_fwd_impl(const void* q, const void* k, const void* v, int64_t ld, const void* bias, int64_t bias_batch_stride,
+                         const void* bias_frag, const void* key_pad, void* out, int64_t ldo, float* lse, int64_t lse_ld, int64_t B,
+                         int64_t S, int64_t Spad, int64_t heads, int64_t head_dim, float scale, int64_t tune, const int* kept,
+                         const int* pos, void* stream) {
   OP_CHECK_ARG(q && k && v && out, "attn_fwd: null pointer");
   OP_CHECK_ARG(head_dim == HD, "attn_fwd: head_dim %lld unsupported (only 64)", (long long)head_dim);
   OP_CHECK_ARG(B > 0 && S > 0 && heads > 0 && ld % 8 == 0 && ldo % 4 == 0, "attn_fwd: bad sizes");
@@ -2565,20 +2615,24 @@
   a.out = (bf16_t*)out; a.ldo = ldo; a.lse = lse; a.lse_ld = lse_ld > 0 ? lse_ld : S;
   a.B = (int)B; a.S = (int)S; a.Spad = (int)Spad; a.heads = (int)heads; a.scale = scale;
   dim3 grid(ceil_div(S, BQ), (unsigned)heads, (unsigned)B);
-  const int slot = op_prof_begin(1, 4.0 * (double)B * (double)heads * (double)S * (double)S * HD, stream);
   hipStream_t s = (hipStream_t)stream;
   const bool inv_exact = (float)(bf16_t)(1.0f / scale) * scale == 1.0f;
   const bf16_t* fr = (const bf16_t*)bias_frag;
-  if (!(tune & FWD_STREAMING) && !(tune & FWD_NO_PERS) && S > 192 && S <= 257 && (!bias || (bias_frag && inv_exact))) {
+  const bool pers = !(tune & FWD_STREAMING) && !(tune & FWD_NO_PERS) && S > 192 && S <= 257 && (!bias || (bias_frag && inv_exact));
+  if (kept && !(pers && a.bias_bs == 0)) return OP_ENOTSUP;
+  const int slot = op_prof_begin(1, 4.0 * (double)B * (double)heads * (double)S * (double)S * HD, stream);
+  if (pers) {
     const int rows_pad = ceil_div(S, 32) * 32;
     const size_t sh = (size_t)4 * rows_pad * 128 + 2 * PERS_NW * PERS_SCR * 4;
     const int nitems = (int)(B * heads);
     const int nwg = min(nitems, op_num_cus());
     return attn_launched(with_bias_pad(bias, key_pad, [&](auto hb, auto hp) {
-      constexpr auto kern = attn_fwd_pers_kernel<decltype(hb)::value, decltype(hp)::value>;
-      OP_ENSURE_LDS(kern, 4 * PERS_MAX_ROWS * 128 + 2 * PERS_NW * PERS_SCR * 4, "attn_fwd");
-      hipLaunchKernelGGL(kern, dim3(nwg), dim3(PERS_NW * 64), sh, s, a, fr, rows_pad, nitems);
-      return OP_OK;
+      return op_with_bool(kept != nullptr, [&](auto kp) {
+        constexpr auto kern = attn_fwd_pers_kernel<decltype(hb)::value, decltype(hp)::value, decltype(kp)::value>;
+        OP_ENSURE_LDS(kern, 4 * PERS_MAX_ROWS * 128 + 2 * PERS_NW * PERS_SCR * 4, "attn_fwd");
+        hipLaunchKernelGGL(kern, dim3(nwg), dim3(PERS_NW * 64), sh, s, a, fr, rows_pad, nitems, kept, pos);
+        return OP_OK;
+      });
     }), slot, stream);
   }
   if (!(tune & FWD_STREAMING) && S <= RES_MAX_S && (!bias || (bias_frag && inv_exact))) {
@@ -2606,6 +2660,31 @@
   }), slot, stream);
 }
 
+extern "C" {
+
+int64_t op_attn_bwd_dbias_slabs(int64_t B, int64_t S, int64_t heads, int64_t tune) {
+  if ((tune & BWD_SEPARATE_DBIAS) || ceil_div(S, BKV) > 6) return ceil_div(B, sep_bchunk(B, S, heads));
+  const int64_t n = dbias_chunks(B, S, heads, true, (tune & BWD_ROUND2_CHUNKS) != 0, (int)((tune >> BWD_CHUNKS_SHIFT) & BWD_CHUNKS_MASK));
+  if (!(tune & BWD_NO_PERS_DQ) && pers_bwd_shape(S)) return max(n, (int64_t)pers_bwd_chunks(B, S, heads));
+  return n;
+}
+
+int op_attn_fwd(const void* q, const void* k, const void* v, int64_t ld, const void* bias, int64_t bias_batch_stride,
+                const void* bias_frag, const void* key_pad, void* out, int64_t ldo, float* lse, int64_t lse_ld, int64_t B,
+                int64_t S, int64_t Spad, int64_t heads, int64_t head_dim, float scale, int64_t tune, void* stream) {
+  return attn_fwd_impl(q, k, v, ld, bias, bias_batch_stride, bias_frag, key_pad, out, ldo, lse, lse_ld, B, S, Spad, heads, head_dim, scale, tune,
+                       nullptr, nullptr, stream);
+}
+
+int op_attn_fwd_kept(const void* q, const void* k, const void* v, int64_t ld, const void* bias, int64_t bias_batch_stride,
+                     const void* bias_frag, const void* key_pad, void* out, int64_t ldo, float* lse, int64_t lse_ld, int64_t B,
+                     int64_t S, int64_t Spad, int64_t heads, int64_t head_dim, float scale, int64_t tune, const int* kept, const int* pos,
+                     void* stream) {
+  OP_CHECK_ARG((kept == nullptr) == (pos == nullptr), "attn_fwd_kept: kept and pos must be given together");
+  return attn_fwd_impl(q, k, v, ld, bias, bias_batch_stride, bias_frag, key_pad, out, ldo, lse, lse_ld, B, S, Spad, heads, head_dim, scale, tune,
+                       kept, pos, stream);
+}
+
 
 int64_t op_attn_bias_frag_elems(int64_t n_img, int64_t S) {
   return n_img * (int64_t)ceil_div(S, 16) * ceil_div(S, 32) * FRAG_BLOCK;
@@ -2635,7 +2714,13 @@
                 const void* biasT, const void* bias_frag, int64_t bias_batch_stride, const void* key_pad, const float* lse,
                 float* delta, void* dq,
                 void* dk, void* dv, int64_t ldg, float* dbias, int64_t B, int64_t S, int64_t Spad, int64_t heads,
-                int64_t head_dim, float scale, int64_t tune, void* stream) {
+                int64_t head_dim, float scale, int64_t tune, void* stream);
+}
+
+static int attn_bwd_impl(const void* q, const void* k, const void* v, int64_t ld, const void* dout, const void* out, int64_t ldo, const void* bias,
+                         const void* biasT, const void* bias_frag, int64_t bias_batch_stride, const void* key_pad, const float* lse,
+                         float* delta, void* dq, void* dk, void* dv, int64_t ldg, float* dbias, int64_t B, int64_t S, int64_t Spad,
+                         int64_t heads, int64_t head_dim, float scale, int64_t tune, const int* kept, const int* pos, void* stream) {
   const bool merge_dbias = !(tune & BWD_SEPARATE_DBIAS);
   OP_CHECK_ARG(q && k && v && dout && lse && delta && dq && dk && dv, "attn_bwd: null pointer");
   OP_CHECK_ARG(head_dim == HD, "attn_bwd: head_dim %lld unsupported (only 64)", (long long)head_dim);
@@ -2671,13 +2756,16 @@
       });
     }), sl, stream);
   };
+  const bool pers_dq = merge_dbias && !(tune & BWD_NO_PERS_DQ) && out && pers_bwd_shape(S) && a.bias_bs == 0 &&
+                       (!bias || (a.bias_frag != nullptr && (float)(bf16_t)(1.0f / scale) * scale == 1.0f));
+  const bool pers_dkdv = !((tune & BWD_NO_PERS_DKDV) || (bias && !biasT) || (S == 256 && !(tune & BWD_PERS_DKDV_256)));
+  if (kept && !(pers_dq && pers_dkdv)) return OP_ENOTSUP;
   if (!out) {
     const int rc = launch_dkdv();
     if (rc != OP_OK) return rc;
   }
   const int nt = ceil_div(S, BKV);
-  if (merge_dbias && !(tune & BWD_NO_PERS_DQ) && out && pers_bwd_shape(S) && a.bias_bs == 0 &&
-      (!bias || (a.bias_frag != nullptr && (float)(bf16_t)(1.0f / scale) * scale == 1.0f))) {
+  if (pers_dq) {
     const int nqb = ceil_div(S, 16);
     const int nqh = ceil_div(min(nqb, 2 * PERS_NW), PERS_NW);
     const int chunks = pers_bwd_chunks(B, S, heads);
@@ -2690,25 +2778,29 @@
     const int slot = op_prof_begin(2, 1.5 * fl, stream);
     int rc = attn_launched(with_bias_pad(bias, key_pad, [&](auto hb, auto hp) {
       return op_with_bool(S > 256, [&](auto lone) {
-        constexpr bool LONE = decltype(lone)::value;
-        constexpr auto kern = attn_bwd_dq_pers_kernel<decltype(hb)::value, decltype(hp)::value, LONE ? 5 : 4, LONE ? 1 : 4>;
-        OP_ENSURE_LDS(kern, 4 * PERS_MAX_ROWS * 128 + 2 * PERS_NW * 64 * 4, "attn_bwd");
-        hipLaunchKernelGGL(kern, dim3(nwg), dim3(PERS_NW * 64), sh, s, d, rows_pad, nqh);
-        return OP_OK;
+        return op_with_bool(kept != nullptr, [&](auto kp) {
+          constexpr bool LONE = decltype(lone)::value;
+          constexpr auto kern = attn_bwd_dq_pers_kernel<decltype(hb)::value, decltype(hp)::value, LONE ? 5 : 4, LONE ? 1 : 4, decltype(kp)::value>;
+          OP_ENSURE_LDS(kern, 4 * PERS_MAX_ROWS * 128 + 2 * PERS_NW * 64 * 4, "attn_bwd");
+          hipLaunchKernelGGL(kern, dim3(nwg), dim3(PERS_NW * 64), sh, s, d, rows_pad, nqh, kept, pos);
+          return OP_OK;
+        });
       });
     }), slot, stream);
     if (rc != OP_OK) return rc;
     a.bchunk = bchunk_dkdv;
-    if ((tune & BWD_NO_PERS_DKDV) || (bias && !biasT) || (S == 256 && !(tune & BWD_PERS_DKDV_256))) return launch_dkdv();
+    if (!pers_dkdv) return launch_dkdv();
     const int dk_rows = dkdv_pers_rows(S), nitems = a.B * a.heads, dk_nwg = min(nitems, op_num_cus());
     const int dk_slot = op_prof_begin(2, 2.0 * fl, stream);
     return attn_launched(with_bias_pad(bias, key_pad, [&](auto hb, auto hp) {
       return op_with_bool(S > 256, [&](auto lone) {
-        constexpr bool LONE = decltype(lone)::value;
-        constexpr auto kern = attn_bwd_dkdv_pers_kernel<decltype(hb)::value, decltype(hp)::value, LONE ? 5 : 4, LONE>;
-        OP_ENSURE_LDS(kern, (int)dkdv_pers_lds(LONE ? 257 : 256), "attn_bwd");
-        hipLaunchKernelGGL(kern, dim3(dk_nwg), dim3(PERS_NW * 64), dkdv_pers_lds(S), s, a, dk_rows, nitems);
-        return OP_OK;
+        return op_with_bool(kept != nullptr, [&](auto kp) {
+          constexpr bool LONE = decltype(lone)::value;
+          constexpr auto kern = attn_bwd_dkdv_pers_kernel<decltype(hb)::value, decltype(hp)::value, LONE ? 5 : 4, LONE, decltype(kp)::value>;
+          OP_ENSURE_LDS(kern, (int)dkdv_pers_lds(LONE ? 257 : 256), "attn_bwd");
+          hipLaunchKernelGGL(kern, dim3(dk_nwg), dim3(PERS_NW * 64), dkdv_pers_lds(S), s, a, dk_rows, nitems, kept, pos);
+          return OP_OK;
+        });
       });
     }), dk_slot, stream);
   }
@@ -2748,4 +2840,24 @@
   return OP_OK;
 }
 
-}
+extern "C" {
+
+int op_attn_bwd(const void* q, const void* k, const void* v, int64_t ld, const void* dout, const void* out, int64_t ldo, const void* bias,
+                const void* biasT, const void* bias_frag, int64_t bias_batch_stride, const void* key_pad, const float* lse,
+                float* delta, void* dq,
+                void* dk, void* dv, int64_t ldg, float* dbias, int64_t B, int64_t S, int64_t Spad, int64_t heads,
+                int64_t head_dim, float scale, int64_t tune, void* stream) {
+  return attn_bwd_impl(q, k, v, ld, dout, out, ldo, bias, biasT, bias_frag, bias_batch_stride, key_pad, lse, delta, dq, dk, dv, ldg, dbias, B, S,
+                       Spad, heads, head_dim, scale, tune, nullptr, nullptr, stream);
+}
+
+int op_attn_bwd_kept(const void* q, const void* k, const void* v, int64_t ld, const void* dout, const void* out, int64_t ldo, const void* bias,
+                     const void* biasT, const void* bias_frag, int64_t bias_batch_stride, const void* key_pad, const float* lse, float* delta,
+                     void* dq, void* dk, void* dv, int64_t ldg, float* dbias, int64_t B, int64_t S, int64_t Spad, int64_t heads,
+                     int64_t head_dim, float scale, int64_t tune, const int* kept, const int* pos, void* stream) {
+  OP_CHECK_ARG((kept == nullptr) == (pos == nullptr), "attn_bwd_kept: kept and pos must be given together");
+  return attn_bwd_impl(q, k, v, ld, dout, out, ldo, bias, biasT, bias_frag, bias_batch_stride, key_pad, lse, delta, dq, dk, dv, ldg, dbias, B, S,
+                       Spad, heads, head_dim, scale, tune, kept, pos, stream);
+}
+
+}
diff --git a/one-peace_amd/csrc/elementwise.hip b/one-peace_amd/csrc/elementwise.hip
--- a/one-peace_amd/csrc/elementwise.hip
+++ b/one-peace_amd/csrc/elementwise.hip
@@ -780,6 +780,59 @@
       for (int c = lane; c < c8; c += 64)
         *reinterpret_cast<uint4*>(base + (int64_t)r * a.out[o].ld + c * 8) =
             src ? *reinterpret_cast<const uint4*>(src + (int64_t)r * a.out[o].lds + c * 8) : make_uint4(0u, 0u, 0u, 0u);
+  }
+}
+
+constexpr int LS_MAX_SEG = 4, LS_MAX_OUT = 4;
+constexpr int LS_PIECE = 16;
+struct LiveSamplesArgs {
+  int nseg, nout, nunits, build;
+  struct { const float* ps; int* kept; int* pos; int64_t row0; int S, B, pstride, unit0; } seg[LS_MAX_SEG];
+  struct { bf16_t* ptr; int64_t ld; int cols; } out[LS_MAX_OUT];
+};
+
+__device__ __forceinline__ bool ls_kept(const float* ps, int64_t i) { return (__float_as_uint(ps[i]) & 0x7fffffffu) != 0u; }
+
+__global__ __launch_bounds__(256) void live_samples_kernel(const LiveSamplesArgs a) {
+  __shared__ int wave_n[4];
+  const int tid = threadIdx.x, lane = tid & 63, wid = tid >> 6;
+  if ((int)blockIdx.x >= a.nunits) {
+    if (blockIdx.y != 0) return;
+    const int i = (int)blockIdx.x - a.nunits;
+    int base = 0;
+    for (int c = 0; c < a.seg[i].B; c += 256) {
+      const int u = c + tid;
+      const bool live = u < a.seg[i].B && ls_kept(a.seg[i].ps, (int64_t)u * a.seg[i].pstride);
+      const unsigned long long m = __ballot(live);
+      if (lane == 0) wave_n[wid] = __popcll(m);
+      __syncthreads();
+      int before = base;
+#pragma unroll
+      for (int w = 0; w < 4; ++w) {
+        if (w < wid) before += wave_n[w];
+        base += wave_n[w];
+      }
+      before += __popcll(m & ((1ull << lane) - 1ull));
+      if (u < a.seg[i].B) a.seg[i].pos[u] = before;
+      if (live) a.seg[i].kept[before] = u;
+      __syncthreads();
+    }
+    if (tid == 0) a.seg[i].pos[a.seg[i].B] = base;
+    return;
+  }
+  int i = 0;
+#pragma unroll
+  for (int j = 1; j < LS_MAX_SEG; ++j)
+    if (j < a.nseg && (int)blockIdx.x >= a.seg[j].unit0) i = j;
+  const int u = (int)blockIdx.x - a.seg[i].unit0;
+  const int r0 = (int)blockIdx.y * LS_PIECE, r1 = min(r0 + LS_PIECE, a.seg[i].S);
+  if (r0 >= r1) return;
+  if (a.build ? ls_kept(a.seg[i].ps, (int64_t)u * a.seg[i].pstride) : a.seg[i].pos[u + 1] != a.seg[i].pos[u]) return;
+  for (int o = 0; o < a.nout; ++o) {
+    const int c8 = a.out[o].cols >> 3;
+    bf16_t* base = a.out[o].ptr + (a.seg[i].row0 + (int64_t)u * a.seg[i].S + r0) * a.out[o].ld;
+    for (int r = wid; r < r1 - r0; r += 4)
+      for (int c = lane; c < c8; c += 64) *reinterpret_cast<uint4*>(base + (int64_t)r * a.out[o].ld + c * 8) = make_uint4(0u, 0u, 0u, 0u);
   }
 }
 
@@ -1256,3 +1309,54 @@
 }
 
 }
+
+static int live_samples_impl(const char* what, int64_t nseg, const float* const* ps, const int64_t* ps_stride, const int64_t* row0, const int64_t* S,
+                             const int64_t* B, int32_t* const* kept, int32_t* const* pos, int64_t nout, void* const* out, const int64_t* out_ld,
+                             const int64_t* out_cols, const int64_t* out_rows, void* stream) {
+  OP_CHECK_ARG(nseg >= 1 && nseg <= LS_MAX_SEG && nout >= 0 && nout <= LS_MAX_OUT, "%s: %lld segments (1 ... %d), %lld outputs (0 ... %d)", what,
+               (long long)nseg, LS_MAX_SEG, (long long)nout, LS_MAX_OUT);
+  OP_CHECK_ARG(row0 && S && B && pos && (!ps || (ps_stride && kept)) && (nout == 0 || (out && out_ld && out_cols && out_rows)), "%s: null pointer", what);
+  LiveSamplesArgs a;
+  memset(&a, 0, sizeof(a));
+  a.nseg = (int)nseg; a.nout = (int)nout; a.build = ps != nullptr;
+  int64_t last_row = 0, max_s = 1;
+  int units = 0;
+  for (int i = 0; i < (int)nseg; ++i) {
+    OP_CHECK_ARG(row0[i] >= 0 && S[i] >= 1 && B[i] >= 1 && S[i] < ((int64_t)1 << 20) && B[i] < ((int64_t)1 << 20) && row0[i] < ((int64_t)1 << 40) && pos[i] &&
+                 (!ps || (ps[i] && kept[i] && ps_stride[i] >= 1 && ps_stride[i] < ((int64_t)1 << 31))), "%s: bad segment %d", what, i);
+    auto& sg = a.seg[i];
+    sg.ps = ps ? ps[i] : nullptr; sg.kept = ps ? kept[i] : nullptr; sg.pos = pos[i]; sg.row0 = row0[i]; sg.S = (int)S[i]; sg.B = (int)B[i];
+    sg.pstride = ps ? (int)ps_stride[i] : 1; sg.unit0 = units;
+    units += sg.B;
+    if (row0[i] + S[i] * B[i] > last_row) last_row = row0[i] + S[i] * B[i];
+    if (S[i] > max_s) max_s = S[i];
+  }
+  a.nunits = units;
+  for (int o = 0; o < (int)nout; ++o) {
+    OP_CHECK_ARG(out[o] && ((uintptr_t)out[o] & 15) == 0 && out_cols[o] >= 8 && out_cols[o] % 8 == 0 && out_ld[o] % 8 == 0 && out_ld[o] >= out_cols[o] &&
+                 out_rows[o] >= last_row && out_cols[o] < ((int64_t)1 << 31), "%s: output %d: null or not 16-byte aligned, cols / ld %% 8, or fewer than %lld rows",
+                 what, o, (long long)last_row);
+    a.out[o].ptr = (bf16_t*)out[o]; a.out[o].ld = out_ld[o]; a.out[o].cols = (int)out_cols[o];
+  }
+  if (!a.build && nout == 0) return OP_OK;
+  const int ny = nout > 0 ? (int)((max_s + LS_PIECE - 1) / LS_PIECE) : 1;
+  hipLaunchKernelGGL(live_samples_kernel, dim3(units + (a.build ? (int)nseg : 0), ny), dim3(256), 0, (hipStream_t)stream, a);
+  OP_LAUNCH_CHECK();
+  return OP_OK;
+}
+
+extern "C" {
+
+int op_live_samples(int64_t nseg, const float* const* ps, const int64_t* ps_stride, const int64_t* row0, const int64_t* S, const int64_t* B,
+                    int32_t* const* kept, int32_t* const* pos, int64_t nout, void* const* out, const int64_t* out_ld, const int64_t* out_cols,
+                    const int64_t* out_rows, void* stream) {
+  OP_CHECK_ARG(ps && ps_stride && kept, "live_samples: null pointer");
+  return live_samples_impl("live_samples", nseg, ps, ps_stride, row0, S, B, kept, pos, nout, out, out_ld, out_cols, out_rows, stream);
+}
+
+int op_live_samples_fill(int64_t nseg, const int64_t* row0, const int64_t* S, const int64_t* B, int32_t* const* pos, int64_t nout, void* const* out,
+                         const int64_t* out_ld, const int64_t* out_cols, const int64_t* out_rows, void* stream) {
+  return live_samples_impl("live_samples_fill", nseg, nullptr, nullptr, row0, S, B, nullptr, pos, nout, out, out_ld, out_cols, out_rows, stream);
+}
+
+}
diff --git a/one-peace_amd/hip.py b/one-peace_amd/hip.py
--- a/one-peace_amd/hip.py
+++ b/one-peace_amd/hip.py
@@ -81,6 +81,11 @@
     "op_attn_bias_pack": (c_int, [P, P, I64, I64, I64, P]),
     "op_attn_bwd_delta": (c_int, [P, P, I64, P, I64, I64, I64, I64, P]),
     "op_attn_bwd": (c_int, [P, P, P, I64, P, P, I64, P, P, P, I64, P, P, P, P, P, P, I64, P, I64, I64, I64, I64, I64, c_float, I64, P]),
+    "op_live_samples": (c_int, [I64, P, P, P, P, P, P, P, I64, P, P, P, P, P]),
+    "op_live_samples_fill": (c_int, [I64, P, P, P, P, I64, P, P, P, P, P]),
+    "op_attn_fwd_kept": (c_int, [P, P, P, I64, P, I64, P, P, P, I64, P, I64, I64, I64, I64, I64, I64, c_float, I64, P, P, P]),
+    "op_attn_bwd_kept": (c_int, [P, P, P, I64, P, P, I64, P, P, P, I64, P, P, P, P, P, P, I64, P, I64, I64, I64, I64, I64, c_float, I64, P, P,
+                                 P]),
     "op_quant_fp8_rows": (c_int, [P, I64, P, I64, P, I64, I64, P]),
     "op_layernorm_fwd_q8": (c_int, [P, P, P, P, P, P, P, P, I64, I64, c_float, P]),
     "op_ln_geglu_fwd_q8": (c_int, [P, P, I64, P, P, P, P, P, P, P, I64, I64, c_float, P]),
@@ -996,20 +1001,88 @@
     return out
 
 
-def attn_fwd(q, k, v, ld, B, S, heads, scale, bias=None, key_pad=None, Spad=0, out=None, want_lse=True, bias_frag=None):
+def live_samples(segs, outs):
+    ns, no = len(segs), len(outs)
+    segs = [tuple(q) + (1,) * (5 - len(q)) for q in segs]
+    dev = segs[0][0].device
+    buf = torch.empty(sum(2 * q[3] + 1 for q in segs), dtype=torch.int32, device=dev)
+    res, off = [], 0
+    for q in segs:
+        res.append((buf[off:off + q[3]], buf[off + q[3]:off + 2 * q[3] + 1]))
+        off += 2 * q[3] + 1
+    i64 = lambda vals: (c_int64 * len(vals))(*[int(v) for v in vals])
+    for ps, _, _, B, st in segs:
+        assert ps.dtype == torch.float32 and ps.is_contiguous() and ps.numel() > (B - 1) * st and ps.device == dev
+    for o in outs:
+        assert o.dtype == torch.bfloat16 and o.dim() == 2 and o.stride(1) == 1 and o.device == dev
+    _check(lib().op_live_samples(ns, _ptr_array([q[0] for q in segs], ns), i64([q[4] for q in segs]), i64([q[1] for q in segs]),
+                                 i64([q[2] for q in segs]), i64([q[3] for q in segs]), _ptr_array([r[0] for r in res], ns),
+                                 _ptr_array([r[1] for r in res], ns), no, _ptr_array(outs, max(no, 1)), i64([o.stride(0) for o in outs] or [0]),
+                                 i64([o.shape[1] for o in outs] or [0]), i64([o.shape[0] for o in outs] or [0]), stream()), "op_live_samples")
+    return res
+
+
+def live_samples_fill(segs, outs):
+    ns, no = len(segs), len(outs)
+    i64 = lambda vals: (c_int64 * len(vals))(*[int(v) for v in vals])
+    for pos, _, _, B in segs:
+        assert pos.dtype == torch.int32 and pos.is_contiguous() and pos.numel() == B + 1
+    for o in outs:
+        assert o.dtype == torch.bfloat16 and o.dim() == 2 and o.stride(1) == 1 and o.device == segs[0][0].device
+    _check(lib().op_live_samples_fill(ns, i64([q[1] for q in segs]), i64([q[2] for q in segs]), i64([q[3] for q in segs]),
+                                      _ptr_array([q[0] for q in segs], ns), no, _ptr_array(outs, max(no, 1)), i64([o.stride(0) for o in outs] or [0]),
+                                      i64([o.shape[1] for o in outs] or [0]), i64([o.shape[0] for o in outs] or [0]), stream()),
+           "op_live_samples_fill")
+
+
+_inv_exact = {}
+
+
+def _inv_scale_exact(scale):
+    if scale not in _inv_exact:
+        sc = torch.tensor(scale, dtype=torch.float32)
+        _inv_exact[scale] = bool((1.0 / sc).to(torch.bfloat16).float() * sc == 1.0)
+    return _inv_exact[scale]
+
+
+def attn_kept_route(S, scale, bias=None, bias_frag=None, backward=False, out_given=True):
+    if not 192 < S <= 257 or (bias is not None and (bias.dim() == 4 or bias_frag is None)):
+        return False
+    if bias is not None and not _inv_scale_exact(float(scale)):
+        return False
+    if backward:
+        return bool(out_given and S != 256 and not TUNE.attn_bwd() & (1 | 1 << 10 | 1 << 12))
+    return not TUNE.attn_fwd() & (1 | 1 << 7)
+
+
+def _kept_lists(kept, pos, B):
+    assert (kept is None) == (pos is None)
+    if kept is not None:
+        assert kept.dtype == torch.int32 and pos.dtype == torch.int32 and kept.is_contiguous() and pos.is_contiguous()
+        assert kept.numel() >= B and pos.numel() == B + 1
+
+
+def attn_fwd(q, k, v, ld, B, S, heads, scale, bias=None, key_pad=None, Spad=0, out=None, want_lse=True, bias_frag=None, kept=None, pos=None):
     dev = q.device
     H = heads * 64
     Spad = Spad or attn_spad(S)
     if out is None:
         out = torch.empty(B * S, H, dtype=torch.bfloat16, device=dev)
     lse = torch.empty(B, heads, Spad, dtype=torch.float32, device=dev) if want_lse else None
+    _kept_lists(kept, pos, B)
+    if kept is not None:
+        rc = lib().op_attn_fwd_kept(ptr(q), ptr(k), ptr(v), ld, ptr(bias), _bias_bstride(bias), ptr(bias_frag), ptr(key_pad), ptr(out),
+                                    out.stride(0), ptr(lse), Spad, B, S, Spad, heads, 64, scale, TUNE.attn_fwd(), ptr(kept), ptr(pos), stream())
+        if rc != -95:
+            _check(rc, "op_attn_fwd_kept")
+            return out, lse
     _check(lib().op_attn_fwd(ptr(q), ptr(k), ptr(v), ld, ptr(bias), _bias_bstride(bias), ptr(bias_frag), ptr(key_pad), ptr(out), out.stride(0),
                              ptr(lse), Spad, B, S, Spad, heads, 64, scale, TUNE.attn_fwd(), stream()), "op_attn_fwd")
     return out, lse
 
 
 def attn_bwd(q, k, v, ld, dout, out, lse, B, S, heads, scale, bias=None, biasT=None, key_pad=None, Spad=0, dqkv=None,
-             want_dbias=False, bias_frag=None):
+             want_dbias=False, bias_frag=None, kept=None, pos=None):
     dev = q.device
     H = heads * 64
     Spad = Spad or attn_spad(S)
@@ -1021,18 +1094,27 @@
     dbias = attn_dbias_buffer(B, S, heads, Spad, dev, per_sample) if want_dbias else None
     dq, dk, dv = dqkv[:, :H], dqkv[:, H:2 * H], dqkv[:, 2 * H:]
     attn_bwd_launch(q, k, v, ld, dout, bias, biasT, key_pad, lse, delta, dq, dk, dv, dqkv.stride(0), dbias, B, S, Spad, heads, scale,
-                    bias_frag, out=out)
+                    bias_frag, out=out, kept=kept, pos=pos)
     if dbias is None:
         return dqkv, None
     return dqkv, (dbias if per_sample else dbias.sum(0))
 
 
 def attn_bwd_launch(q, k, v, ld, dout, bias, biasT, key_pad, lse, delta, dq, dk, dv, ldg, dbias, B, S, Spad, heads, scale,
-                    bias_frag=None, out=None):
+                    bias_frag=None, out=None, kept=None, pos=None):
+    _kept_lists(kept, pos, B)
+    if kept is not None:
+        rc = lib().op_attn_bwd_kept(ptr(q), ptr(k), ptr(v), ld, ptr(dout), ptr(out), dout.stride(0), ptr(bias), ptr(biasT), ptr(bias_frag),
+                                    _bias_bstride(bias), ptr(key_pad), ptr(lse), ptr(delta), ptr(dq), ptr(dk), ptr(dv), ldg, ptr(dbias), B, S,
+                                    Spad, heads, 64, scale, TUNE.attn_bwd(), ptr(kept), ptr(pos), stream())
+        if rc != -95:
+            _check(rc, "op_attn_bwd_kept")
+            return True
     _check(lib().op_attn_bwd(ptr(q), ptr(k), ptr(v), ld, ptr(dout), ptr(out), dout.stride(0), ptr(bias), ptr(biasT), ptr(bias_frag),
                              _bias_bstride(bias),
                              ptr(key_pad), ptr(lse), ptr(delta), ptr(dq), ptr(dk), ptr(dv), ldg, ptr(dbias), B, S, Spad, heads,
                              64, scale, TUNE.attn_bwd(), stream()), "op_attn_bwd")
+    return False
 
 
 def attn_dbias_buffer(B, S, heads, Spad, device, per_sample=False):
diff --git a/one-peace_amd/ops.py b/one-peace_amd/ops.py
--- a/one-peace_amd/ops.py
+++ b/one-peace_amd/ops.py
@@ -294,6 +294,17 @@
     return True
 
 
+SKIP_ZERO_ATTN = os.environ.get("ONEPEACE_SKIP_ZERO_ATTN", "1") != "0"
+
+
+def _attn_kept_ok(S, scale, bias, bias_frag, listed, backward=False):
+    if not (SKIP_ZERO_ATTN and listed) or SEPARATE_DELTA:
+        return False
+    if backward:
+        return hip.attn_kept_route(S, scale, bias, bias_frag, backward=True)
+    return hip.attn_kept_route(S, scale, bias, bias_frag) and hip.attn_kept_route(S, scale, bias, bias_frag, backward=True)
+
+
 class _WgradQueue:
 
     def __init__(self):
@@ -830,11 +841,18 @@
             hip.gemm_nt(xln1, [w], [b] if b is not None else None, out=qkv[:, i * H:(i + 1) * H], ldc=3 * H)
     attn = torch.empty_like(xln1)
     lses = []
-    for sg in segs:
+    klists = [(None, None)] * len(segs)
+    if win is not None:
+        qual = [i for i, sg in enumerate(segs) if _attn_kept_ok(sg.S, scale, sg.bias.image if sg.bias is not None else None,
+                                                                sg.frag(hip.ATTN_RESIDENT_MAX_S), True)]
+        if qual:
+            for i, kl in zip(qual, hip.live_samples([wsegs[i] for i in qual], [])):
+                klists[i] = kl
+    for sg, (kl, kpos) in zip(segs, klists):
         r = slice(sg.row0, sg.end)
         _, lse = hip.attn_fwd(qkv[r, :H], qkv[r, H:2 * H], qkv[r, 2 * H:], 3 * H, sg.B, sg.S, heads, scale,
                               sg.bias.image.detach() if sg.bias is not None else None, sg.key_pad, hip.attn_spad(sg.S), out=attn[r],
-                              want_lse=keep, bias_frag=sg.frag(hip.ATTN_RESIDENT_MAX_S))
+                              want_lse=keep, bias_frag=sg.frag(hip.ATTN_RESIDENT_MAX_S), kept=kl, pos=kpos)
         lses.append(lse)
         if sg.pad:
             attn[sg.end - sg.pad:sg.end].zero_()
@@ -852,6 +870,7 @@
     acts = dict(xln1=xln1, mean1=mean1, rstd1=rstd1, qkv=qkv, attn=attn, aln=aln, mean_a=mean_a, rstd_a=rstd_a, y1=y1)
     for i, lse in enumerate(lses):
         acts["lse%d" % i] = lse
+        acts["akept%d" % i], acts["apos%d" % i] = klists[i]
     return x_mid, acts
 
 
@@ -1110,7 +1129,7 @@
                 _attn_backward(qkv[r], dattn[r], A["attn"][r], A["lse%d" % i], sg.B, sg.S, heads, scale,
                                sg.bias.image.detach() if sg.bias is not None else None, sg.bias.imageT if sg.bias is not None else None,
                                sg.key_pad, sg.bias.grad_accumulator(sg.B) if want_dbias[i] else None, sg.frag(384),
-                               dparts["wq"], dparts["wk"], dparts["wv"])
+                               dparts["wq"], dparts["wk"], dparts["wv"], kept=A.get("akept%d" % i), pos=A.get("apos%d" % i))
             bias_of = {"wq": "bq", "wv": "bv"}
             bnames = tuple(bias_of[n] for n in cols if n in bias_of and needs[bias_of[n]])
             if bnames:
@@ -1469,7 +1488,7 @@
     return out, vec
 
 
-def _attn_backward(qkv, dattn, attn, lse, B, S, heads, scale, bias_img, biasT, key_pad, dbias_acc, bias_frag, dq, dk, dv):
+def _attn_backward(qkv, dattn, attn, lse, B, S, heads, scale, bias_img, biasT, key_pad, dbias_acc, bias_frag, dq, dk, dv, kept=None, pos=None):
     H = heads * 64
     dev = qkv.device
     Spad = hip.attn_spad(S)
@@ -1478,8 +1497,10 @@
         hip._check(hip.lib().op_attn_bwd_delta(hip.ptr(dattn), hip.ptr(attn), dattn.stride(0), hip.ptr(delta), B, S, Spad, heads,
                                                hip.stream()), "op_attn_bwd_delta")
         attn = None
-    hip.attn_bwd_launch(qkv[:, :H], qkv[:, H:2 * H], qkv[:, 2 * H:], 3 * H, dattn, bias_img, biasT, key_pad, lse, delta, dq, dk,
-                        dv, dq.stride(0), dbias_acc, B, S, Spad, heads, scale, bias_frag, out=attn)
+    ran = hip.attn_bwd_launch(qkv[:, :H], qkv[:, H:2 * H], qkv[:, 2 * H:], 3 * H, dattn, bias_img, biasT, key_pad, lse, delta, dq, dk,
+                              dv, dq.stride(0), dbias_acc, B, S, Spad, heads, scale, bias_frag, out=attn, kept=kept, pos=pos)
+    if kept is not None and not ran:
+        raise RuntimeError("attention backward: the forward left the dropped samples' lse out, and this call cannot take their lists")
 
 
 def attn_branch(x, bias, key_pad, ps, heads, params, save_acts=False):
```

Result: no change. 206.1 (median of 2 runs) (+0.2%).
